# google-research/sparf

Measured on NVIDIA H100. Metric: rays/sec (fwd+bwd, 128 samples/ray), higher is better.
Workload: dtype fp32 in / out; GEMMs on Hopper wgmma with a 3-pass error-compensated split (fp16 halves forward, bf16 halves backward), fp32 accumulation; fp32 CUDA cores for encoding / activations / compositing

## Files before the change

### include/sparf_b200.h

```cpp
#ifndef SPARF_B200_H_
#define SPARF_B200_H_

#include <stddef.h>
#include <stdint.h>

#ifdef __cplusplus
extern "C" {
#endif

#define SPARF_B200_VERSION 100
#define SPARF_MAX_TRUNK 12
#define SPARF_MAX_L 16

enum {
  SPARF_OK = 0,
  SPARF_ERR_INVALID = 1,
  SPARF_ERR_CUDA = 2,
  SPARF_ERR_WORKSPACE = 3,
  SPARF_ERR_UNSUPPORTED = 4
};

enum {
  SPARF_ENGINE_AUTO = 0,
  SPARF_ENGINE_SIMT_FP32 = 1,
// ... 71 lines not shown
                                const float* origins, const float* dirs, const float* t, const float* noise, float* sigma,
                                float* rgb, void* tape, size_t tape_bytes, void* workspace, size_t workspace_bytes,
                                sparf_stream_t stream);
int sparf_mlp_backward_tape_rows(const SparfMLP* mlp, int32_t engine, int32_t R, int32_t S, const int64_t* rows,
                                 const float* origins, const float* dirs, const float* t, const float* sigma,
                                 const float* rgb, const float* d_sigma, const float* d_rgb, const SparfMLPGrad* grad,
                                 float* d_origins, float* d_dirs, void* tape, size_t tape_bytes, void* workspace,
                                 size_t workspace_bytes, sparf_stream_t stream);
int sparf_compact_scatter(int64_t C, const int64_t* K, const int64_t* sample_idx, int32_t width, const float* src,
                          float* dst, sparf_stream_t stream);
int sparf_compact_gather(int64_t C, const int64_t* K, const int64_t* sample_idx, int32_t width, const float* src,
                         float* dst, sparf_stream_t stream);
int sparf_compact_ray_sum(int64_t R, int32_t S, int64_t C, const int64_t* K, const int64_t* sample_idx, int32_t width,
                          const float* src, float* dst, sparf_stream_t stream);

int sparf_mlp_forward_tape_span(const SparfMLP* mlp, int32_t engine, int32_t C, int32_t cap, const int64_t* begin,
                                const int64_t* end, const float* origins, const float* dirs, const float* t,
                                const float* noise, float* sigma, float* rgb, void* tape, size_t tape_bytes,
                                void* workspace, size_t workspace_bytes, sparf_stream_t stream);
int sparf_compact_scatter_span(int64_t C, const int64_t* ends, int32_t w, const int64_t* sample_idx, int32_t width,
                               const float* src, float* dst, sparf_stream_t stream);
int sparf_compact_gather_span(int64_t C, const int64_t* ends, int32_t w, const int64_t* sample_idx, int32_t width,
                              const float* src, float* dst, sparf_stream_t stream);
int sparf_compact_ray_sum_segments(int64_t R, int32_t S, int32_t W, const int64_t* ends, const int64_t* sample_idx,
                                   int32_t width, const float* src, float* dst, sparf_stream_t stream);

size_t sparf_density_workspace_bytes(const SparfMLP* mlp, int64_t M, int32_t backward, int32_t engine);
int sparf_density_forward(const SparfMLP* mlp, int32_t engine, int64_t M, const float* points, float* raw, float* feat,
                          void* workspace, size_t workspace_bytes, sparf_stream_t stream);
int sparf_density_backward(const SparfMLP* mlp, int32_t engine, int64_t M, const float* points, const float* d_raw,
                           const float* d_feat, const SparfMLPGrad* grad, float* d_points, void* workspace,
                           size_t workspace_bytes, sparf_stream_t stream);
int sparf_density_gradient(const SparfMLP* mlp, int32_t engine, int64_t M, const float* points, float* grad_points,
                           void* workspace, size_t workspace_bytes, sparf_stream_t stream);

#define SPARF_MCUBES_MAX_TRIS 5
size_t sparf_mcubes_workspace_bytes(int64_t nx, int64_t ny, int64_t nz);
int sparf_mcubes_count(const float* vol, int64_t nx, int64_t ny, int64_t nz, float iso, int64_t* totals, void* workspace,
                       size_t workspace_bytes, sparf_stream_t stream);
int sparf_mcubes_emit(const float* vol, int64_t nx, int64_t ny, int64_t nz, float iso, float* verts, int64_t* faces,
                      void* workspace, size_t workspace_bytes, sparf_stream_t stream);
int sparf_mcubes_table(int8_t* table);

#define SPARF_MCUBES_BLOCK 8
size_t sparf_mcubes_sparse_workspace_bytes(int32_t res, int64_t n_active, int64_t max_verts);
int sparf_mcubes_sparse_classify(const float* coarse, int32_t res, float iso, int32_t* slots, int64_t* n_active,
                                 void* workspace, size_t workspace_bytes, sparf_stream_t stream);
int sparf_mcubes_sparse_blocks(const int32_t* slots, int32_t res, int64_t* block_ids, sparf_stream_t stream);
int sparf_mcubes_sparse_points(const float* axis, int32_t res, const int64_t* block_ids, int64_t b0, int64_t n_blocks,
                               float* points, sparf_stream_t stream);
int sparf_mcubes_sparse_count(const float* sigma_blocks, int32_t res, const int32_t* slots, const int64_t* block_ids,
                              int64_t n_active, float iso, int64_t* totals, void* workspace, size_t workspace_bytes,
                              sparf_stream_t stream);
int sparf_mcubes_sparse_emit(const float* sigma_blocks, int32_t res, const int32_t* slots, const int64_t* block_ids,
                             int64_t n_active, float iso, int64_t max_verts, int64_t max_faces, float* verts,
                             int64_t* faces, void* workspace, size_t workspace_bytes, sparf_stream_t stream);

int sparf_occupancy_build(const float* sigma, int32_t res, float thres, uint32_t* bits, sparf_stream_t stream);
size_t sparf_occupancy_workspace_bytes(int64_t R, int32_t S);
int sparf_occupancy_count(int64_t R, int32_t S, const float* origins, const float* dirs, const float* t,
                          const uint32_t* bits, int32_t res, float r0, float r1, int64_t* K, void* workspace,
                          size_t workspace_bytes, sparf_stream_t stream);
int sparf_occupancy_emit(int64_t R, int32_t S, const float* origins, const float* dirs, const float* t,
                         const uint32_t* bits, int32_t res, float r0, float r1, int64_t* sample_idx, float* origins_k,
                         float* dirs_k, float* t_k, void* workspace, size_t workspace_bytes, sparf_stream_t stream);

size_t sparf_termination_workspace_bytes(int64_t R, int32_t window);
int sparf_termination_count(int64_t R, int32_t S, int32_t k0, int32_t k1, const float* origins, const float* dirs,
                            const float* t, const uint8_t* alive, const uint32_t* bits, int32_t res, float r0, float r1,
                            int64_t* K, void* workspace, size_t workspace_bytes, sparf_stream_t stream);
int sparf_termination_emit(int64_t R, int32_t S, int32_t k0, int32_t k1, const float* origins, const float* dirs,
                           const float* t, const uint8_t* alive, const uint32_t* bits, int32_t res, float r0, float r1,
                           int64_t* sample_idx, float* origins_k, float* dirs_k, float* t_k, void* workspace,
                           size_t workspace_bytes, sparf_stream_t stream);
int sparf_termination_update(int64_t R, int32_t S, int32_t k0, int32_t k1, const float* sigma, const float* t,
                             const float* dirs, float tau_max, float* tau, uint8_t* alive, sparf_stream_t stream);
int sparf_termination_append(int64_t R, int32_t S, int32_t k0, int32_t k1, const float* origins, const float* dirs,
                             const float* t, const uint8_t* alive, const uint32_t* bits, int32_t res, float r0, float r1,
                             int64_t* ends, int32_t w, int64_t* sample_idx, float* origins_k, float* dirs_k, float* t_k,
                             void* workspace, size_t workspace_bytes, sparf_stream_t stream);

int sparf_contracted_count(int64_t R, int32_t S, int32_t k0, int32_t k1, const float* origins, const float* dirs,
                           const float* t, const uint8_t* alive, const uint32_t* bits, int32_t res, const float* center,
                           float radius, int64_t* K, void* workspace, size_t workspace_bytes, sparf_stream_t stream);
int sparf_contracted_emit(int64_t R, int32_t S, int32_t k0, int32_t k1, const float* origins, const float* dirs,
                          const float* t, const uint8_t* alive, const uint32_t* bits, int32_t res, const float* center,
                          float radius, int64_t* sample_idx, float* origins_k, float* dirs_k, float* t_k,
                          void* workspace, size_t workspace_bytes, sparf_stream_t stream);
int sparf_contracted_append(int64_t R, int32_t S, int32_t k0, int32_t k1, const float* origins, const float* dirs,
                            const float* t, const uint8_t* alive, const uint32_t* bits, int32_t res, const float* center,
                            float radius, int64_t* ends, int32_t w, int64_t* sample_idx, float* origins_k, float* dirs_k,
                            float* t_k, void* workspace, size_t workspace_bytes, sparf_stream_t stream);

size_t sparf_occupancy_sample_workspace_bytes(int32_t res);
int sparf_occupancy_sample(int32_t res, const uint32_t* bits, float r0, float r1, const float* center, float radius,
                           int64_t n_uniform, int64_t n_occupied, const float* u_cell, const float* u_jit, int64_t* cells,
                           float* points, void* workspace, size_t workspace_bytes, sparf_stream_t stream);
int sparf_occupancy_ema(int32_t res, int32_t contracted, int64_t n, const int64_t* cells, const float* sigma, float decay,
                        float thres, float* density, uint32_t* bits, void* workspace, size_t workspace_bytes,
                        sparf_stream_t stream);

int sparf_composite_forward(int32_t R, int32_t S, const float* sigma, const float* rgb, const float* t,
                            const float* dirs, int32_t white_bg, float* rgb_map, float* depth,
                            float* opacity, float* depth_var, float* rgb_var, float* weights,
                            float* all_cumulated, sparf_stream_t stream);
int sparf_composite_backward(int32_t R, int32_t S, const float* sigma, const float* rgb, const float* t,
                             const float* dirs, int32_t white_bg, const float* g_rgb_map,
                             const float* g_depth, const float* g_opacity, const float* g_weights,
                             float* d_sigma, float* d_rgb, float* d_dirs, sparf_stream_t stream);

int sparf_huber2_fwd_bwd(int64_t n, const float* pred, const float* target, float scale, float* loss,
                         float* d_pred, sparf_stream_t stream);

int sparf_posenc_forward(int64_t n, int32_t channels, int32_t L, const float* x, int32_t use_c2f, float c2f_start,
                         float c2f_range, const float* progress, float* out, sparf_stream_t stream);
int sparf_posenc_backward(int64_t n, int32_t channels, int32_t L, const float* x, int32_t use_c2f, float c2f_start,
                          float c2f_range, const float* progress, const float* d_out, float* d_x, sparf_stream_t stream);

int sparf_distortion_fwd_bwd(int32_t R, int32_t S, const float* t, const float* w, float scale, float* loss,
                             float* d_w, float* d_t, sparf_stream_t stream);

int sparf_adam_step(int64_t n, float* param, float* grad, float* exp_avg, float* exp_avg_sq, int64_t* step,
                    double* scratch, double lr0, double gamma, double warmup_steps, double beta1, double beta2,
                    double eps, double max_norm, sparf_stream_t stream);

int sparf_tc_selftest(const float* A, const float* B, int32_t K, void* packed, float* D, sparf_stream_t stream);
int sparf_tc_selftest_tn(const float* G, const float* X, int32_t rows, float* D, sparf_stream_t stream);
int sparf_tc_selftest_images(const float* X, const float* W1, const float* E, const float* W2, int32_t M, float* Y, float* Z,
                             float* db, sparf_stream_t stream);
int sparf_tc_selftest_persistent(const float* X, const float* W1, const float* E, const float* W2, int32_t M, float* Y,
                                 float* Z, float* db, int32_t max_ctas, sparf_stream_t stream);
int sparf_tc_selftest_head(const float* d_rgb, const float* rgb, const float* d_sigma, const float* raw, const float* hid,
                           const float* W9, int32_t M, int32_t HW, int32_t row_passes, int32_t tr_passes, uint16_t* img,
                           float* graw, sparf_stream_t stream);
int sparf_tc_selftest_featgrad(const float* d_raw, const float* d_feat, const float* feat, int32_t M, int32_t W,
                               int32_t row_passes, int32_t tr_passes, uint16_t* img, float* sums, sparf_stream_t stream);
int sparf_tc_selftest_wgrad(const float* G, const float* X, int32_t M, int32_t N, int32_t K, int32_t Kv, int32_t ldx,
                            int32_t div, int32_t passes, int32_t max_ctas, float* dW, uint32_t* bits, sparf_stream_t stream);
int sparf_tc_selftest_wgrad_rows(const float* G, const float* X, int32_t M, int32_t N, int32_t K, int32_t Kv, int32_t ldx,
                                 int32_t div, int32_t passes, int32_t max_ctas, const int64_t* rows, float* dW,
                                 uint32_t* bits, sparf_stream_t stream);
int sparf_tc_selftest_mask_bits(const float* G, const float* W, const float* X, int32_t M, int32_t N, int32_t K,
                                int32_t max_ctas, uint16_t* img, sparf_stream_t stream);
int sparf_tc_selftest_chain(const float* enc, int32_t M, int32_t E3, int32_t nt, int32_t skip, const float* W,
                            const float* bias, int32_t passes, int32_t f16, int32_t max_ctas, int32_t chain,
                            uint32_t outputs, const int64_t* rows, float* H, uint16_t* last, sparf_stream_t stream);
int sparf_tc_selftest_chain_bits(const float* enc, int32_t M, int32_t E3, int32_t nt, int32_t skip, const float* W,
                                 const float* bias, int32_t passes, int32_t f16, int32_t max_ctas, const int64_t* rows,
                                 float* H, uint32_t* bits, sparf_stream_t stream);
int sparf_tc_selftest_dgrad_chain(const float* G, int32_t M, int32_t E3, int32_t nt, int32_t skip, const float* W,
                                  const uint32_t* bits, int32_t dg_passes, int32_t wg_passes, int32_t max_ctas,
                                  int32_t chain, const int64_t* rows, uint16_t* tr, uint16_t* row, float* db,
                                  sparf_stream_t stream);

#ifdef __cplusplus
}
#endif
#endif
```

### sparf_b200/_lib.py

```python
from __future__ import annotations

import ctypes
import os
from ctypes import POINTER, c_char_p, c_float, c_int32, c_int64, c_size_t, c_void_p

from . import build as _build

MAX_TRUNK = 12
MCUBES_MAX_TRIS = 5
MCUBES_BLOCK = 8

ENGINE_AUTO, ENGINE_SIMT_FP32, ENGINE_TC_3X, ENGINE_TC_1X, ENGINE_TC_3X_W1 = 0, 1, 2, 3, 4
ENGINES = {"auto": 0, "simt_fp32": 1, "tc_3x": 2, "tc_1x": 3, "tc_3x_w1": 4}


class SparfMLP(ctypes.Structure):
    _fields_ = [
        ("n_trunk", c_int32), ("width", c_int32), ("head_width", c_int32), ("skip_layer", c_int32),
        ("L_xyz", c_int32), ("L_view", c_int32), ("use_c2f", c_int32),
        ("c2f_start", c_float), ("c2f_range", c_float),
        ("progress", c_void_p),
        ("trunk_w", c_void_p * MAX_TRUNK), ("trunk_b", c_void_p * MAX_TRUNK),
        ("head_w", c_void_p * 2), ("head_b", c_void_p * 2),
    ]


class SparfMLPGrad(ctypes.Structure):
    _fields_ = [
        ("trunk_w", c_void_p * MAX_TRUNK), ("trunk_b", c_void_p * MAX_TRUNK),
        ("head_w", c_void_p * 2), ("head_b", c_void_p * 2),
    ]


_P = c_void_p
_SIGNATURES = {
    "sparf_version": (c_int32, []),
    "sparf_last_error": (c_char_p, []),
    "sparf_launch_count": (ctypes.c_uint64, []),
    "sparf_engine_available": (c_int32, [c_int32]),
    "sparf_raygen_forward": (c_int32, [c_int32, c_int32, c_int32, _P, _P, _P, _P, c_int32, _P, _P, _P]),
    "sparf_raygen_backward": (c_int32, [c_int32, c_int32, c_int32, _P, _P, _P, _P, c_int32, _P, _P, _P, _P, _P]),
    "sparf_sample_depth": (c_int32, [c_int32, c_int32, c_float, c_float, c_int32, _P, _P, _P, _P]),
    "sparf_sample_pdf_merge": (c_int32, [c_int32, c_int32, c_int32, c_float, c_float, _P, _P, _P, _P, _P, _P]),
    "sparf_mlp_workspace_bytes": (c_size_t, [POINTER(SparfMLP), c_int32, c_int32, c_int32, c_int32]),
    "sparf_mlp_forward": (c_int32, [POINTER(SparfMLP), c_int32, c_int32, c_int32, _P, _P, _P, _P, _P, _P, _P, c_size_t, _P]),
    "sparf_mlp_backward": (c_int32, [POINTER(SparfMLP), c_int32, c_int32, c_int32, _P, _P, _P, _P, _P, _P,
                                     POINTER(SparfMLPGrad), _P, _P, _P, c_size_t, _P]),
    "sparf_mlp_tape_bytes": (c_size_t, [POINTER(SparfMLP), c_int32, c_int32, c_int32]),
    "sparf_mlp_forward_tape": (c_int32, [POINTER(SparfMLP), c_int32, c_int32, c_int32, _P, _P, _P, _P, _P, _P, _P, c_size_t,
                                         _P, c_size_t, _P]),
    "sparf_mlp_backward_tape": (c_int32, [POINTER(SparfMLP), c_int32, c_int32, c_int32, _P, _P, _P, _P, _P, _P, _P,
                                          POINTER(SparfMLPGrad), _P, _P, _P, c_size_t, _P, c_size_t, _P]),
    "sparf_mlp_forward_tape_rows": (c_int32, [POINTER(SparfMLP), c_int32, c_int32, c_int32, _P, _P, _P, _P, _P, _P, _P, _P,
                                              c_size_t, _P, c_size_t, _P]),
    "sparf_mlp_backward_tape_rows": (c_int32, [POINTER(SparfMLP), c_int32, c_int32, c_int32, _P, _P, _P, _P, _P, _P, _P, _P,
                                               POINTER(SparfMLPGrad), _P, _P, _P, c_size_t, _P, c_size_t, _P]),
    "sparf_compact_scatter": (c_int32, [c_int64, _P, _P, c_int32, _P, _P, _P]),
    "sparf_compact_gather": (c_int32, [c_int64, _P, _P, c_int32, _P, _P, _P]),
    "sparf_compact_ray_sum": (c_int32, [c_int64, c_int32, c_int64, _P, _P, c_int32, _P, _P, _P]),
    "sparf_mlp_forward_tape_span": (c_int32, [POINTER(SparfMLP), c_int32, c_int32, c_int32, _P, _P, _P, _P, _P, _P, _P, _P,
                                              _P, c_size_t, _P, c_size_t, _P]),
    "sparf_compact_scatter_span": (c_int32, [c_int64, _P, c_int32, _P, c_int32, _P, _P, _P]),
    "sparf_compact_gather_span": (c_int32, [c_int64, _P, c_int32, _P, c_int32, _P, _P, _P]),
    "sparf_compact_ray_sum_segments": (c_int32, [c_int64, c_int32, c_int32, _P, _P, c_int32, _P, _P, _P]),
    "sparf_density_workspace_bytes": (c_size_t, [POINTER(SparfMLP), c_int64, c_int32, c_int32]),
    "sparf_density_forward": (c_int32, [POINTER(SparfMLP), c_int32, c_int64, _P, _P, _P, _P, c_size_t, _P]),
    "sparf_density_backward": (c_int32, [POINTER(SparfMLP), c_int32, c_int64, _P, _P, _P, POINTER(SparfMLPGrad), _P, _P,
                                         c_size_t, _P]),
    "sparf_density_gradient": (c_int32, [POINTER(SparfMLP), c_int32, c_int64, _P, _P, _P, c_size_t, _P]),
    "sparf_mcubes_workspace_bytes": (c_size_t, [c_int64, c_int64, c_int64]),
    "sparf_mcubes_count": (c_int32, [_P, c_int64, c_int64, c_int64, c_float, _P, _P, c_size_t, _P]),
    "sparf_mcubes_emit": (c_int32, [_P, c_int64, c_int64, c_int64, c_float, _P, _P, _P, c_size_t, _P]),
    "sparf_mcubes_table": (c_int32, [_P]),
    "sparf_mcubes_sparse_workspace_bytes": (c_size_t, [c_int32, c_int64, c_int64]),
    "sparf_mcubes_sparse_classify": (c_int32, [_P, c_int32, c_float, _P, _P, _P, c_size_t, _P]),
    "sparf_mcubes_sparse_blocks": (c_int32, [_P, c_int32, _P, _P]),
    "sparf_mcubes_sparse_points": (c_int32, [_P, c_int32, _P, c_int64, c_int64, _P, _P]),
    "sparf_mcubes_sparse_count": (c_int32, [_P, c_int32, _P, _P, c_int64, c_float, _P, _P, c_size_t, _P]),
    "sparf_mcubes_sparse_emit": (c_int32, [_P, c_int32, _P, _P, c_int64, c_float, c_int64, c_int64, _P, _P, _P, c_size_t,
                                           _P]),
    "sparf_occupancy_build": (c_int32, [_P, c_int32, c_float, _P, _P]),
    "sparf_occupancy_workspace_bytes": (c_size_t, [c_int64, c_int32]),
    "sparf_occupancy_count": (c_int32, [c_int64, c_int32, _P, _P, _P, _P, c_int32, c_float, c_float, _P, _P, c_size_t, _P]),
    "sparf_occupancy_emit": (c_int32, [c_int64, c_int32, _P, _P, _P, _P, c_int32, c_float, c_float, _P, _P, _P, _P, _P,
                                       c_size_t, _P]),
    "sparf_termination_workspace_bytes": (c_size_t, [c_int64, c_int32]),
    "sparf_termination_count": (c_int32, [c_int64, c_int32, c_int32, c_int32, _P, _P, _P, _P, _P, c_int32, c_float, c_float,
                                          _P, _P, c_size_t, _P]),
    "sparf_termination_emit": (c_int32, [c_int64, c_int32, c_int32, c_int32, _P, _P, _P, _P, _P, c_int32, c_float, c_float,
                                         _P, _P, _P, _P, _P, c_size_t, _P]),
    "sparf_termination_update": (c_int32, [c_int64, c_int32, c_int32, c_int32, _P, _P, _P, c_float, _P, _P, _P]),
    "sparf_termination_append": (c_int32, [c_int64, c_int32, c_int32, c_int32, _P, _P, _P, _P, _P, c_int32, c_float, c_float,
                                           _P, c_int32, _P, _P, _P, _P, _P, c_size_t, _P]),
    "sparf_contracted_append": (c_int32, [c_int64, c_int32, c_int32, c_int32, _P, _P, _P, _P, _P, c_int32, POINTER(c_float),
                                          c_float, _P, c_int32, _P, _P, _P, _P, _P, c_size_t, _P]),
    "sparf_contracted_count": (c_int32, [c_int64, c_int32, c_int32, c_int32, _P, _P, _P, _P, _P, c_int32, POINTER(c_float),
                                         c_float, _P, _P, c_size_t, _P]),
    "sparf_contracted_emit": (c_int32, [c_int64, c_int32, c_int32, c_int32, _P, _P, _P, _P, _P, c_int32, POINTER(c_float),
                                        c_float, _P, _P, _P, _P, _P, c_size_t, _P]),
    "sparf_occupancy_sample_workspace_bytes": (c_size_t, [c_int32]),
    "sparf_occupancy_sample": (c_int32, [c_int32, _P, c_float, c_float, POINTER(c_float), c_float, c_int64, c_int64, _P, _P,
                                         _P, _P, _P, c_size_t, _P]),
    "sparf_occupancy_ema": (c_int32, [c_int32, c_int32, c_int64, _P, _P, c_float, c_float, _P, _P, _P, c_size_t, _P]),
    "sparf_composite_forward":(c_int32, [c_int32, c_int32, _P, _P, _P, _P, c_int32, _P, _P, _P, _P, _P, _P, _P, _P]),
    "sparf_composite_backward": (c_int32, [c_int32, c_int32, _P, _P, _P, _P, c_int32, _P, _P, _P, _P, _P, _P, _P, _P]),
    "sparf_huber2_fwd_bwd": (c_int32, [c_int64, _P, _P, c_float, _P, _P, _P]),
    "sparf_posenc_forward": (c_int32, [c_int64, c_int32, c_int32, _P, c_int32, c_float, c_float, _P, _P, _P]),
    "sparf_posenc_backward": (c_int32, [c_int64, c_int32, c_int32, _P, c_int32, c_float, c_float, _P, _P, _P, _P]),
    "sparf_distortion_fwd_bwd": (c_int32, [c_int32, c_int32, _P, _P, c_float, _P, _P, _P, _P]),
    "sparf_adam_step": (c_int32, [c_int64, _P, _P, _P, _P, _P, _P] + [ctypes.c_double] * 7 + [_P]),
    "sparf_tc_selftest": (c_int32, [_P, _P, c_int32, _P, _P, _P]),
    "sparf_tc_selftest_tn": (c_int32, [_P, _P, c_int32, _P, _P]),
    "sparf_tc_selftest_images": (c_int32, [_P, _P, _P, _P, c_int32, _P, _P, _P, _P]),
    "sparf_tc_selftest_persistent": (c_int32, [_P, _P, _P, _P, c_int32, _P, _P, _P, c_int32, _P]),
    "sparf_tc_selftest_head": (c_int32, [_P, _P, _P, _P, _P, _P, c_int32, c_int32, c_int32, c_int32, _P, _P, _P]),
    "sparf_tc_selftest_featgrad": (c_int32, [_P, _P, _P, c_int32, c_int32, c_int32, c_int32, _P, _P, _P]),
    "sparf_tc_selftest_wgrad": (c_int32, [_P, _P, c_int32, c_int32, c_int32, c_int32, c_int32, c_int32, c_int32, c_int32,
                                          _P, _P, _P]),
    "sparf_tc_selftest_wgrad_rows": (c_int32, [_P, _P, c_int32, c_int32, c_int32, c_int32, c_int32, c_int32, c_int32,
                                               c_int32, _P, _P, _P, _P]),
    "sparf_tc_selftest_mask_bits": (c_int32, [_P, _P, _P, c_int32, c_int32, c_int32, c_int32, _P, _P]),
    "sparf_tc_selftest_chain": (c_int32, [_P, c_int32, c_int32, c_int32, c_int32, _P, _P, c_int32, c_int32, c_int32, c_int32,
                                          ctypes.c_uint32, _P, _P, _P, _P]),
    "sparf_tc_selftest_chain_bits": (c_int32, [_P, c_int32, c_int32, c_int32, c_int32, _P, _P, c_int32, c_int32, c_int32,
                                               _P, _P, _P, _P]),
    "sparf_tc_selftest_dgrad_chain": (c_int32, [_P, c_int32, c_int32, c_int32, c_int32, _P, _P, c_int32, c_int32, c_int32,
                                                c_int32, _P, _P, _P, _P, _P]),
}

_lib = None


def exported_symbols():
    return list(_SIGNATURES)


def lib():
    global _lib
    if _lib is not None:
        return _lib
    path = _build.LIB_PATH
    override = os.environ.get("SPARF_B200_LIB")
    if override:
        if not os.path.exists(override):
            raise RuntimeError("SPARF_B200_LIB=%s does not exist" % override)
        path = override
    elif not os.path.exists(path) or _build._stale():
        try:
            path = _build.build()
        except Exception as e:
            if not os.path.exists(path):
                raise RuntimeError(
                    "sparf_b200: native library %s is missing and could not be built (%s). "
                    "There is no fallback path." % (path, e))
    L = ctypes.CDLL(path)
    for name, (res, args) in _SIGNATURES.items():
        fn = getattr(L, name)
        fn.restype = res
        fn.argtypes = args
    _lib = L
    return L


def check(rc: int, what: str = ""):
    if rc != 0:
        msg = lib().sparf_last_error()
        raise RuntimeError("sparf_b200 %s failed (code %d): %s" % (what, rc, msg.decode() if msg else "?"))
```

### sparf_b200/csrc/gemm_wgmma.cu

```cuda
#include <cuda_bf16.h>
#include <cudaTypedefs.h>
#include <cuda_fp16.h>

#include <algorithm>
#include <type_traits>

#include "gemm_wgmma.cuh"

namespace sparf {
namespace {

constexpr int TM = 128, TN = 128, TK = 32;
constexpr int TILE_ELEMS = TM * TK;

struct __align__(128) WgSmem {
  uint16_t a[2][TILE_ELEMS];
  uint16_t b[2][TILE_ELEMS];
};

__device__ __forceinline__ int sw_off(int r, int k) { return (((r >> 3) * (TK / 8) + (k >> 3)) << 6) + ((r & 7) << 3) + (k & 7); }

__device__ __forceinline__ uint64_t smem_desc(const void* p) {
  uint32_t a = static_cast<uint32_t>(__cvta_generic_to_shared(p));
  uint64_t d = (uint64_t)((a & 0x3FFFF) >> 4);
// ... 645 lines not shown
      float* d = e.out + (size_t)m * e.ldo + e.col_off + n;
      if (n < e.Kv) atomicAdd(d, acc[i]);
      if (two && n + 1 < e.Kv) atomicAdd(d + 1, acc[i + 1]);
    }
    if (!two) acc[i + 1] = 0.f;
  }
}

template <bool F16, bool F32, int ROWP, int TRP>
__device__ __forceinline__ void epilogue(float (&acc)[64], int bx, int by, const Epi e) {
  const int m0 = by * TM, n0 = bx * TN;
  if (e.pairs) epilogue_values<F32, true>(acc, m0, n0, e);
  else epilogue_values<F32, false>(acc, m0, n0, e);
  const int lane = threadIdx.x & 31, w = threadIdx.x >> 5;
  if (e.colsum) {
    float part[32];
#pragma unroll
    for (int j = 0; j < 16; ++j)
#pragma unroll
      for (int c = 0; c < 2; ++c) part[2 * j + c] = acc[4 * j + c] + acc[4 * j + 2 + c];
    tile_colsum(part, n0, e.N, e.colsum);
  }
  if constexpr (ROWP > 0) {
#pragma unroll
    for (int j = 0; j < 16; ++j) {
      const int kt = (n0 >> 5) + (j >> 2);
      if (kt >= e.row_ks) break;
      uint16_t* t = e.row + ((size_t)by * e.row_ks + kt) * 2 * TILE_ELEMS;
#pragma unroll
      for (int h = 0; h < 2; ++h) {
        uint32_t hi, lo;
        split2<F16>(acc[4 * j + 2 * h], acc[4 * j + 2 * h + 1], hi, lo);
        const int core = (2 * w + h) * (TK / 8) + (j & 3);
        reinterpret_cast<uint32_t*>(t + core * 64)[lane] = hi;
        if (ROWP == 3) reinterpret_cast<uint32_t*>(t + TILE_ELEMS + core * 64)[lane] = lo;
      }
    }
  }
  if constexpr (TRP > 0) {
    const int kt = (m0 >> 5) + (w >> 1);
    if (kt < e.tr_ks) {
      uint16_t* t = e.tr + ((size_t)bx * e.tr_ks + kt) * 2 * TILE_ELEMS;
#pragma unroll
      for (int j = 0; j < 16; ++j)
#pragma unroll
        for (int h = 0; h < 2; ++h) {
          uint32_t hi, lo;
          split2<F16>(acc[4 * j + 2 * h], acc[4 * j + 2 * h + 1], hi, lo);
          const int core = j * (TK / 8) + 2 * (w & 1) + h;
          reinterpret_cast<uint32_t*>(t + core * 64)[lane] = movmatrix_trans(hi);
          if (TRP == 3) reinterpret_cast<uint32_t*>(t + TILE_ELEMS + core * 64)[lane] = movmatrix_trans(lo);
        }
    }
  }
}

template <bool F16, int PASSES, bool F32, int ROWP, int TRP, bool DYN = false, bool SPAN = false>
__global__ void __launch_bounds__(GEMM_THREADS, 1) wg_gemm_kernel(Opnd a, Opnd b, Units w, Epi e, RowCount rc) {
  extern __shared__ __align__(1024) uint8_t smem[];
  if constexpr (DYN) {
    e.M = (int)live_rows<true, SPAN>(e.M, rc);
    if (e.M == 0) return;
    w.tiles = (e.M + TM - 1) / TM * w.rtb;
    if constexpr (SPAN) e.out += row_start<true>(rc) * e.ldo;
  }
  uint64_t* full = reinterpret_cast<uint64_t*>(smem + STAGES * STAGE_BYTES + RED_BYTES);
  uint64_t* empty = full + STAGES;
  if (threadIdx.x == 0) {
    for (int i = 0; i < STAGES; ++i) {
      mbar_init(&full[i], 1);
      mbar_init(&empty[i], CONSUMERS / 32);
    }
    asm volatile("fence.mbarrier_init.release.cluster;\n" ::: "memory");
  }
  __syncthreads();
  if (threadIdx.x >= CONSUMERS) {
    asm volatile("setmaxnreg.dec.sync.aligned.u32 40;\n" ::: "memory");
    if (threadIdx.x == CONSUMERS) produce<PASSES>(a, b, w, full, empty);
    return;
  }
  asm volatile("setmaxnreg.inc.sync.aligned.u32 232;\n" ::: "memory");
  int it = 0;
  for (int u = blockIdx.x; u < w.tiles * w.nsplit; u += gridDim.x) {
    int bx, by, kt0, nk;
    w.get(u, bx, by, kt0, nk);
    float acc[64];
    mma_unit<F16, PASSES>(acc, nk, it, full, empty);
    epilogue<F16, F32, ROWP, TRP>(acc, bx, by, e);
  }
}

struct Staged {
  const float* X;
  int ldx, div, M, K;
  uint32_t* bits;
  int kw;
};

constexpr int STAGED_THREADS = CONSUMERS + 256;
constexpr int STAGED_STAGES = 5;
constexpr int PART_BYTES = TM * TN * 4;
constexpr int STAGED_SMEM = STAGED_STAGES * STAGE_BYTES + PART_BYTES + 3 * STAGED_STAGES * 8;

__device__ __forceinline__ void split8_mul(const float (&v)[8], uint4& hi, uint4& lo) {
  uint16_t h[8], l[8];
#pragma unroll
  for (int e = 0; e < 8; ++e) {
    const __nv_bfloat16 b = __float2bfloat16_rn(v[e]);
    h[e] = __bfloat16_as_ushort(b);
    l[e] = __bfloat16_as_ushort(__float2bfloat16_rn((v[e] - __bfloat162float(b)) * (float)(1 << LO_SHIFT)));
  }
  hi = make_uint4(h[0] | (uint32_t)h[1] << 16, h[2] | (uint32_t)h[3] << 16, h[4] | (uint32_t)h[5] << 16, h[6] | (uint32_t)h[7] << 16);
  lo = make_uint4(l[0] | (uint32_t)l[1] << 16, l[2] | (uint32_t)l[3] << 16, l[4] | (uint32_t)l[5] << 16, l[6] | (uint32_t)l[7] << 16);
}

__device__ __forceinline__ void converter_sync() { asm volatile("bar.sync 2, 128;\n" ::: "memory"); }
__device__ __forceinline__ void fence_proxy_async() { asm volatile("fence.proxy.async.shared::cta;\n" ::: "memory"); }

template <int PASSES, int NST = STAGES>
__device__ __forceinline__ void produce_staged(const Opnd& a, const Staged& x, const CUtensorMap* xmap, const Units& w,
                                               uint64_t* full, uint64_t* empty) {
  extern __shared__ __align__(1024) uint8_t smem[];
  const int lane = threadIdx.x & 31;
  const uint32_t abytes = PASSES == 3 ? 2 * TILE_BYTES : TILE_BYTES;
  int it = 0;
  for (int u = blockIdx.x; u < w.tiles * w.nsplit; u += gridDim.x) {
    int bx, by, kt0, nk;
    w.get(u, bx, by, kt0, nk);
    const int k0 = bx * TM;
    const uint32_t rbytes = 4 * min(TM, x.K - k0);
    for (int j = 0; j < nk; ++j, ++it) {
      const int s = it % NST, m0 = (kt0 + j) * TK;
      mbar_wait(&empty[s], ((it / NST) & 1) ^ 1);
      uint8_t* st = smem + s * STAGE_BYTES;
      if (x.div == 1) {
        if (lane == 0) {
          mbar_expect_tx(&full[s], abytes + TK * TM * 4);
          bulk_g2s(st, a.tile(by, kt0 + j), abytes, &full[s]);
          tensor_g2s(st + 2 * TILE_BYTES, xmap, k0, m0, &full[s]);
        }
        continue;
      }
      if (lane == 0) {
        mbar_expect_tx(&full[s], abytes + min(TK, x.M - m0) * rbytes);
        bulk_g2s(st, a.tile(by, kt0 + j), abytes, &full[s]);
      }
      __syncwarp();
      const int m = m0 + lane;
      if (m < x.M) bulk_g2s(st + 2 * TILE_BYTES + lane * (TM * 4), x.X + (size_t)(m / x.div) * x.ldx + k0, rbytes, &full[s]);
    }
  }
}

template <int PASSES, int NST = STAGES>
__device__ __forceinline__ void convert_staged(const Staged& x, const Units& w, uint64_t* full, uint64_t* conv) {
  extern __shared__ __align__(1024) uint8_t smem[];
  const int t = threadIdx.x - CONSUMERS, lane = t & 31;
  int it = 0;
  for (int u = blockIdx.x; u < w.tiles * w.nsplit; u += gridDim.x) {
    int bx, by, kt0, nk;
    w.get(u, bx, by, kt0, nk);
    const bool kin = bx * TM + t < x.K, bits = x.bits && by == 0;
    const int bword = bx * (TM / 32) + (t >> 5);
    for (int j = 0; j < nk; ++j, ++it) {
      const int s = it % NST, m0 = (kt0 + j) * TK;
      mbar_wait(&full[s], (it / NST) & 1);
      uint8_t* st = smem + s * STAGE_BYTES + 2 * TILE_BYTES;
      const float* src = reinterpret_cast<const float*>(st);
      float v[TK];
      if (kin && m0 + TK <= x.M) {
#pragma unroll
        for (int r = 0; r < TK; ++r) v[r] = src[r * TM + t];
      } else {
#pragma unroll
        for (int r = 0; r < TK; ++r) v[r] = kin && m0 + r < x.M ? src[r * TM + t] : 0.f;
      }
      if (bits) {
        uint32_t word = 0;
#pragma unroll
        for (int r = 0; r < TK; ++r) {
          const uint32_t b = __ballot_sync(0xffffffffu, v[r] > 0.f);
          if (lane == r) word = b;
        }
        if (m0 + lane < x.M && bword < x.kw) x.bits[(size_t)(m0 + lane) * x.kw + bword] = word;
      }
      converter_sync();
      uint16_t* img = reinterpret_cast<uint16_t*>(st);
#pragma unroll
      for (int o = 0; o < TK / 8; ++o) {
        float e8[8];
#pragma unroll
        for (int e = 0; e < 8; ++e) e8[e] = v[8 * o + e];
        uint4 hi, lo;
        split8_mul(e8, hi, lo);
        const int off = sw_off(t, 8 * o);
        *reinterpret_cast<uint4*>(img + off) = hi;
        if (PASSES == 3) *reinterpret_cast<uint4*>(img + TILE_ELEMS + off) = lo;
      }
      fence_proxy_async();
      __syncwarp();
      if (lane == 0) mbar_arrive(&conv[s]);
    }
  }
}

__device__ __forceinline__ int part_off(int r, int c) { return r * TN + (((c >> 3) ^ (r & 7)) << 3) + (c & 7); }

__device__ __forceinline__ void presum_epilogue(const float (&acc)[64], float* part, bool first, bool flush, int bx, int by,
                                                const Epi& e) {
  const int lane = threadIdx.x & 31, w = threadIdx.x >> 5;
#pragma unroll
  for (int i = 0; i < 64; i += 2) {
    float2* p = reinterpret_cast<float2*>(part + part_off(frag_row(i), frag_col(i)));
    if (first) {
      *p = make_float2(acc[i], acc[i + 1]);
    } else {
      const float2 o = *p;
      *p = make_float2(o.x + acc[i], o.y + acc[i + 1]);
    }
  }
  if (!flush) return;
  __syncwarp();
  const int m0 = by * TM, n0 = bx * TN;
  float* out = e.out + e.col_off + n0;
  for (int i = 0; i < 16; ++i) {
    const int r = 16 * w + i, m = m0 + r;
    if (m >= e.M) continue;
#pragma unroll
    for (int q = 0; q < TN / 32; ++q) {
      const int c = 32 * q + lane, n = n0 + c;
      if (n < e.N && n < e.Kv) atomicAdd(out + (size_t)m * e.ldo + c, part[part_off(r, c)]);
    }
  }
  __syncwarp();
}

template <int PASSES, bool DYN = false>
__global__ void __launch_bounds__(STAGED_THREADS, 1) wg_gemm_staged_kernel(Opnd a, Staged x, Units w, Epi e, RowCount rc,
                                                                           int ctas, const __grid_constant__ CUtensorMap xmap) {
  extern __shared__ __align__(1024) uint8_t smem[];
  if constexpr (DYN) {
    x.M = (int)live_rows<true, false>(x.M, rc);
    if (x.M == 0) return;
    w.nk = (x.M + TK - 1) / TK;
    w.nsplit = max(1, min(w.nk, (ctas + w.tiles - 1) / w.tiles * ((w.nk + 1023) / 1024)));
  }
  float* part = reinterpret_cast<float*>(smem + STAGED_STAGES * STAGE_BYTES);
  uint64_t* full = reinterpret_cast<uint64_t*>(smem + STAGED_STAGES * STAGE_BYTES + PART_BYTES);
  uint64_t* empty = full + STAGED_STAGES;
  uint64_t* conv = empty + STAGED_STAGES;
  if (threadIdx.x == 0) {
    for (int i = 0; i < STAGED_STAGES; ++i) {
      mbar_init(&full[i], 1);
      mbar_init(&empty[i], CONSUMERS / 32);
      mbar_init(&conv[i], 4);
    }
    asm volatile("fence.mbarrier_init.release.cluster;\n" ::: "memory");
  }
  __syncthreads();
  if (threadIdx.x >= CONSUMERS + 128) {
    asm volatile("setmaxnreg.dec.sync.aligned.u32 40;\n" ::: "memory");
    if (threadIdx.x < CONSUMERS + 128 + 32) produce_staged<PASSES, STAGED_STAGES>(a, x, &xmap, w, full, empty);
    return;
  }
  if (threadIdx.x >= CONSUMERS) {
    asm volatile("setmaxnreg.dec.sync.aligned.u32 64;\n" ::: "memory");
    convert_staged<PASSES, STAGED_STAGES>(x, w, full, conv);
    return;
  }
  asm volatile("setmaxnreg.inc.sync.aligned.u32 200;\n" ::: "memory");
  const int units = w.tiles * w.nsplit, grid = gridDim.x;
  int it = 0;
  for (int u = blockIdx.x; u < units; u += grid) {
    int bx, by, kt0, nk;
    w.get(u, bx, by, kt0, nk);
    float acc[64];
    mma_unit<false, PASSES, true, STAGED_STAGES>(acc, nk, it, full, empty, conv);
    const int t = u % w.tiles;
    const bool first = u < grid || (u - grid) % w.tiles != t;
    const bool flush = u + grid >= units || (u + grid) % w.tiles != t;
    presum_epilogue(acc, part, first, flush, bx, by, e);
  }
}

constexpr int CH_W = 256;
constexpr int CH_M = 64;
constexpr int CH_KS = CH_W / TK;
constexpr int CH_ENC_KS = 2;
constexpr int CH_HALF = CH_M * TK * 2;
constexpr int CH_STAGES = 4;
constexpr int CH_ENC = CH_KS * 2 * CH_HALF;
constexpr int CH_RING = CH_ENC + CH_ENC_KS * 2 * CH_HALF;
constexpr int CH_BAR = CH_RING + CH_STAGES * STAGE_BYTES;
constexpr int CH_SMEM = CH_BAR + (2 * CH_STAGES + 2) * 8;

struct Chain {
  int M, nl, skip, enc_ks;
  const uint16_t* enc;
  const uint16_t* w[SPARF_MAX_TRUNK];
  const float* bias[SPARF_MAX_TRUNK];
  float* H[SPARF_MAX_TRUNK];
  uint16_t* last;
  uint32_t* bits[SPARF_MAX_TRUNK];
};

__host__ __device__ __forceinline__ int chain_ks(int l, int skip, int enc_ks) {
  return l == 0 ? enc_ks : CH_KS + (l == skip ? enc_ks : 0);
}

template <int PASSES>
__device__ __forceinline__ void chain_produce(const Chain& c, int M, int tiles, uint64_t* full, uint64_t* empty, uint64_t* enc_full,
                                              uint64_t* enc_empty) {
  extern __shared__ __align__(1024) uint8_t smem[];
  constexpr int HB = PASSES == 3 ? 2 : 1;
  int it = 0, n = 0;
  for (int t = blockIdx.x; t < tiles; t += gridDim.x) {
    if (t * CH_M >= M) continue;
    mbar_wait(enc_empty, (n & 1) ^ 1);
    ++n;
    mbar_expect_tx(enc_full, c.enc_ks * HB * CH_HALF);
    for (int kt = 0; kt < c.enc_ks; ++kt)
      for (int h = 0; h < HB; ++h)
        bulk_g2s(smem + CH_ENC + (kt * 2 + h) * CH_HALF,
                 c.enc + (((size_t)(t >> 1) * c.enc_ks + kt) * 2 + h) * TILE_ELEMS + (t & 1) * (CH_M * TK), CH_HALF, enc_full);
    for (int l = 0; l < c.nl; ++l) {
      const int nk = chain_ks(l, c.skip, c.enc_ks);
      for (int kt = 0; kt < nk; ++kt, ++it) {
        const int s = it % CH_STAGES;
        mbar_wait(&empty[s], ((it / CH_STAGES) & 1) ^ 1);
        uint8_t* st = smem + CH_RING + s * STAGE_BYTES;
        mbar_expect_tx(&full[s], 2 * HB * TILE_BYTES);
        for (int g = 0; g < 2; ++g)
          bulk_g2s(st + g * 2 * TILE_BYTES, c.w[l] + ((size_t)g * nk + kt) * 2 * TILE_ELEMS, HB * TILE_BYTES, &full[s]);
      }
    }
  }
}

template <bool F16, int PASSES>
__device__ __forceinline__ void chain_mma(float (&acc)[64], int nk, int na, int& it, uint64_t* full, uint64_t* empty) {
  extern __shared__ __align__(1024) uint8_t smem[];
  const int wg = threadIdx.x >> 7, lane = threadIdx.x & 31;
  float acc_lo[PASSES == 3 ? 64 : 1];
#pragma unroll
  for (int i = 0; i < 64; ++i) acc[i] = 0.f;
#pragma unroll
  for (int i = 0; i < (PASSES == 3 ? 64 : 1); ++i) acc_lo[i] = 0.f;
  for (int j = 0; j < nk; ++j, ++it) {
    const int s = it % CH_STAGES;
    mbar_wait(&full[s], (it / CH_STAGES) & 1);
    const uint8_t* a = j < na ? smem + j * 2 * CH_HALF : smem + CH_ENC + (j - na) * 2 * CH_HALF;
    const uint8_t* b = smem + CH_RING + s * STAGE_BYTES + wg * 2 * TILE_BYTES;
    wgmma_fence();
#pragma unroll
    for (int ks = 0; ks < TK / 16; ++ks) {
      const uint64_t ahi = smem_desc(a + ks * 256), bhi = smem_desc(b + ks * 256);
      if constexpr (PASSES == 3) {
        wgmma_m64n128k16<F16>(acc_lo, smem_desc(a + CH_HALF + ks * 256), bhi);
        wgmma_m64n128k16<F16>(acc_lo, ahi, smem_desc(b + TILE_BYTES + ks * 256));
      }
      wgmma_m64n128k16<F16>(acc, ahi, bhi);
    }
    wgmma_commit();
    wgmma_wait_1();
    if (j > 0 && lane == 0) mbar_arrive(&empty[(it + CH_STAGES - 1) % CH_STAGES]);
  }
  wgmma_wait_all();
  if (lane == 0) mbar_arrive(&empty[(it + CH_STAGES - 1) % CH_STAGES]);
  if constexpr (PASSES == 3) {
#pragma unroll
    for (int i = 0; i < 64; ++i) acc[i] += ldexpf(acc_lo[i], -LO_SHIFT);
  }
}

template <bool F16, int PASSES>
__device__ __forceinline__ void chain_epilogue(float (&acc)[64], const Chain& c, int M, int l, int t) {
  extern __shared__ __align__(1024) uint8_t smem[];
  const int wg = threadIdx.x >> 7, wq = (threadIdx.x >> 5) & 3, lane = threadIdx.x & 31;
  const float* bias = c.bias[l];
#pragma unroll
  for (int i = 0; i < 64; i += 2) {
    const int m = t * CH_M + wq * 16 + (lane >> 2) + ((i >> 1) & 1) * 8, n = wg * TN + (i >> 2) * 8 + (lane & 3) * 2;
    if (m >= M) {
      acc[i] = acc[i + 1] = 0.f;
      continue;
    }
    acc[i] = fmaxf(acc[i] + bias[n], 0.f);
    acc[i + 1] = fmaxf(acc[i + 1] + bias[n + 1], 0.f);
  }
  const bool last = l == c.nl - 1;
  if (last && !c.last) return;
  uint16_t* img = last ? c.last + (size_t)(t >> 1) * CH_KS * 2 * TILE_ELEMS + (t & 1) * (CH_M * TK)
                       : reinterpret_cast<uint16_t*>(smem);
  const int kstride = last ? 2 * TILE_ELEMS : CH_HALF, lo_off = last ? TILE_ELEMS : CH_HALF / 2;
#pragma unroll
  for (int j = 0; j < 16; ++j) {
    uint16_t* kt = img + (size_t)(4 * wg + (j >> 2)) * kstride;
#pragma unroll
    for (int h = 0; h < 2; ++h) {
      uint32_t hi, lo;
      split2<F16>(acc[4 * j + 2 * h], acc[4 * j + 2 * h + 1], hi, lo);
      const int core = (2 * wq + h) * (TK / 8) + (j & 3);
      reinterpret_cast<uint32_t*>(kt + core * 64)[lane] = hi;
      if (PASSES == 3) reinterpret_cast<uint32_t*>(kt + lo_off + core * 64)[lane] = lo;
    }
  }
}

__device__ __forceinline__ void chain_store(const float (&acc)[64], float* H, int M, int t) {
  const int wg = threadIdx.x >> 7, wq = (threadIdx.x >> 5) & 3, lane = threadIdx.x & 31;
#pragma unroll
  for (int i = 0; i < 64; i += 2) {
    const int m = t * CH_M + wq * 16 + (lane >> 2) + ((i >> 1) & 1) * 8, n = wg * TN + (i >> 2) * 8 + (lane & 3) * 2;
    if (m < M) *reinterpret_cast<float2*>(H + (size_t)m * CH_W + n) = make_float2(acc[i], acc[i + 1]);
  }
}

__device__ __forceinline__ void chain_store_bits(const float (&acc)[64], uint32_t* bits, int M, int t) {
  const int wg = threadIdx.x >> 7, wq = (threadIdx.x >> 5) & 3, lane = threadIdx.x & 31;
#pragma unroll
  for (int h = 0; h < 2; ++h) {
    uint32_t mine = 0;
#pragma unroll
    for (int q = 0; q < 4; ++q) {
      uint32_t w = 0;
#pragma unroll
      for (int jj = 0; jj < 4; ++jj) {
        const int i = 4 * (4 * q + jj) + 2 * h, b = 8 * jj + 2 * (lane & 3);
        w |= (uint32_t)(acc[i] > 0.f) << b | (uint32_t)(acc[i + 1] > 0.f) << (b + 1);
      }
      w |= __shfl_xor_sync(0xffffffffu, w, 1);
      w |= __shfl_xor_sync(0xffffffffu, w, 2);
      if ((lane & 3) == q) mine = w;
    }
    const int m = t * CH_M + wq * 16 + (lane >> 2) + 8 * h;
    if (m < M) bits[(size_t)m * (CH_W / 32) + wg * 4 + (lane & 3)] = mine;
  }
}

template <bool F16, int PASSES, bool DYN = false, bool BITS = false, bool SPAN = false>
__global__ void __launch_bounds__(GEMM_THREADS, 1) trunk_chain_kernel(const Chain c, RowCount rc) {
  extern __shared__ __align__(1024) uint8_t smem[];
  const int M = (int)live_rows<DYN, SPAN>(c.M, rc);
  if (DYN && M == 0) return;
  const int tiles = (M + TM - 1) / TM * 2;
  uint64_t* full = reinterpret_cast<uint64_t*>(smem + CH_BAR);
  uint64_t* empty = full + CH_STAGES;
  uint64_t* enc_full = empty + CH_STAGES;
  uint64_t* enc_empty = enc_full + 1;
  if (threadIdx.x == 0) {
    for (int i = 0; i < CH_STAGES; ++i) {
      mbar_init(&full[i], 1);
      mbar_init(&empty[i], CONSUMERS / 32);
    }
    mbar_init(enc_full, 1);
    mbar_init(enc_empty, CONSUMERS / 32);
    asm volatile("fence.mbarrier_init.release.cluster;\n" ::: "memory");
  }
  __syncthreads();
  if (threadIdx.x >= CONSUMERS) {
    asm volatile("setmaxnreg.dec.sync.aligned.u32 40;\n" ::: "memory");
    if (threadIdx.x == CONSUMERS) chain_produce<PASSES>(c, M, tiles, full, empty, enc_full, enc_empty);
    return;
  }
  asm volatile("setmaxnreg.inc.sync.aligned.u32 232;\n" ::: "memory");
  const int enc_last = c.skip > 0 && c.skip < c.nl ? c.skip : 0;
  const long long s0 = row_start<SPAN>(rc);
  int it = 0, n = 0;
  for (int t = blockIdx.x; t < tiles; t += gridDim.x) {
    if (t * CH_M >= M) {
      if (c.last)
        for (int i = 0; i < CH_KS * (PASSES == 3 ? 2 : 1); ++i)
          reinterpret_cast<uint4*>(c.last + ((size_t)(t >> 1) * CH_KS * 2 + (PASSES == 3 ? i : 2 * i)) * TILE_ELEMS +
                                   (t & 1) * (CH_M * TK))[threadIdx.x] = make_uint4(0, 0, 0, 0);
      continue;
    }
    mbar_wait(enc_full, n & 1);
    ++n;
    for (int l = 0; l < c.nl; ++l) {
      float acc[64];
      chain_mma<F16, PASSES>(acc, chain_ks(l, c.skip, c.enc_ks), l == 0 ? 0 : CH_KS, it, full, empty);
      if (l == enc_last && (threadIdx.x & 31) == 0) mbar_arrive(enc_empty);
      consumer_sync();
      chain_epilogue<F16, PASSES>(acc, c, M, l, t);
      if (l + 1 < c.nl) {
        fence_proxy_async();
        consumer_sync();
      }
      if (c.H[l]) chain_store(acc, c.H[l] + s0 * CH_W, M, t);
      if (BITS && c.bits[l]) chain_store_bits(acc, c.bits[l] + s0 * (CH_W / 32), M, t);
    }
  }
}

template <bool F16, int PASSES>
static int launch_chain(const Chain& c, int ctas, RowCount rc, cudaStream_t st) {
  bool bits = false;
  for (int l = 0; l < c.nl; ++l) bits |= c.bits[l] != nullptr;
  auto kernel = bits ? (rc.rows ? trunk_chain_kernel<F16, PASSES, true, true> : trunk_chain_kernel<F16, PASSES, false, true>)
                     : (rc.rows ? trunk_chain_kernel<F16, PASSES, true> : trunk_chain_kernel<F16, PASSES>);
  if (rc.start) {
    if (!bits) {
      set_error("trunk_chain: a row start needs the mask bits (taped forward)");
      return SPARF_ERR_UNSUPPORTED;
    }
    kernel = trunk_chain_kernel<F16, PASSES, true, true, true>;
  }
  SPARF_CHECK_CUDA(cudaFuncSetAttribute(kernel, cudaFuncAttributeMaxDynamicSharedMemorySize, CH_SMEM));
  kernel<<<std::min(2 * ceil_div(c.M, TM), ctas), GEMM_THREADS, CH_SMEM, st>>>(c, rc);
  SPARF_CHECK_LAUNCH("trunk_chain_kernel");
  return SPARF_OK;
}

struct DgChain {
  int M, top, tr_ks;
  const uint16_t* in;
  const uint16_t* w[SPARF_MAX_TRUNK];
  const uint32_t* bits[SPARF_MAX_TRUNK];
  float* db[SPARF_MAX_TRUNK];
  uint16_t* tr[SPARF_MAX_TRUNK];
  uint16_t* row[SPARF_MAX_TRUNK];
};

template <int DP>
__device__ __forceinline__ void dg_produce(const DgChain& c, int M, int tiles, uint64_t* full, uint64_t* empty, uint64_t* act_full,
                                           uint64_t* act_empty) {
  extern __shared__ __align__(1024) uint8_t smem[];
  constexpr int HB = DP == 3 ? 2 : 1;
  int it = 0, n = 0;
  for (int t = blockIdx.x; t < tiles; t += gridDim.x) {
    if (t * CH_M >= M) continue;
    mbar_wait(act_empty, (n & 1) ^ 1);
    ++n;
    mbar_expect_tx(act_full, CH_KS * HB * CH_HALF);
    for (int kt = 0; kt < CH_KS; ++kt)
      for (int h = 0; h < HB; ++h)
        bulk_g2s(smem + (kt * 2 + h) * CH_HALF,
                 c.in + (((size_t)(t >> 1) * CH_KS + kt) * 2 + h) * TILE_ELEMS + (t & 1) * (CH_M * TK), CH_HALF, act_full);
    for (int l = c.top; l >= 1; --l)
      for (int kt = 0; kt < CH_KS; ++kt, ++it) {
        const int s = it % CH_STAGES;
        mbar_wait(&empty[s], ((it / CH_STAGES) & 1) ^ 1);
        uint8_t* st = smem + CH_RING + s * STAGE_BYTES;
        mbar_expect_tx(&full[s], 2 * HB * TILE_BYTES);
        for (int g = 0; g < 2; ++g)
          bulk_g2s(st + g * 2 * TILE_BYTES, c.w[l] + ((size_t)g * CH_KS + kt) * 2 * TILE_ELEMS, HB * TILE_BYTES, &full[s]);
      }
  }
}

__device__ __forceinline__ void dg_mask_words(uint4 (&wd)[2], const uint32_t* bits, int M, int t) {
  const int wg = threadIdx.x >> 7, wq = (threadIdx.x >> 5) & 3, lane = threadIdx.x & 31;
#pragma unroll
  for (int h = 0; h < 2; ++h) {
    const int m = t * CH_M + wq * 16 + (lane >> 2) + 8 * h;
    wd[h] = m < M ? *reinterpret_cast<const uint4*>(bits + (size_t)m * (CH_W / 32) + wg * 4) : make_uint4(0, 0, 0, 0);
  }
}

template <int PASSES>
__device__ __forceinline__ void dg_split(const float (&acc)[64], uint16_t* img, int kstride, int lo_off) {
  const int wg = threadIdx.x >> 7, wq = (threadIdx.x >> 5) & 3, lane = threadIdx.x & 31;
#pragma unroll
  for (int j = 0; j < 16; ++j) {
    uint16_t* kt = img + (size_t)(4 * wg + (j >> 2)) * kstride;
#pragma unroll
    for (int h = 0; h < 2; ++h) {
      uint32_t hi, lo;
      split2<false>(acc[4 * j + 2 * h], acc[4 * j + 2 * h + 1], hi, lo);
      const int core = (2 * wq + h) * (TK / 8) + (j & 3);
      reinterpret_cast<uint32_t*>(kt + core * 64)[lane] = hi;
      if (PASSES == 3) reinterpret_cast<uint32_t*>(kt + lo_off + core * 64)[lane] = lo;
    }
  }
}

template <int DP, int TP>
__device__ __forceinline__ void dg_zero_tile(const DgChain& c, int t) {
  const uint4 z = make_uint4(0, 0, 0, 0);
  for (int l = c.top; l >= 1; --l) {
    if (c.row[l])
      for (int i = 0; i < CH_KS * (DP == 3 ? 2 : 1); ++i)
        reinterpret_cast<uint4*>(c.row[l] + ((size_t)(t >> 1) * CH_KS * 2 + (DP == 3 ? i : 2 * i)) * TILE_ELEMS +
                                 (t & 1) * (CH_M * TK))[threadIdx.x] = z;
    for (int g = 0; g < 2; ++g)
      for (int kt = 2 * t; kt < 2 * t + 2 && kt < c.tr_ks; ++kt)
        for (int h = 0; h < (TP == 3 ? 2 : 1); ++h)
          for (int i = threadIdx.x; i < TILE_ELEMS / 8; i += CONSUMERS)
            reinterpret_cast<uint4*>(c.tr[l] + (((size_t)g * c.tr_ks + kt) * 2 + h) * TILE_ELEMS)[i] = z;
  }
}

template <int DP, int TP, bool DYN = false>
__global__ void __launch_bounds__(GEMM_THREADS, 1) dgrad_chain_kernel(const DgChain c, RowCount rc) {
  extern __shared__ __align__(1024) uint8_t smem[];
  const int M = (int)live_rows<DYN, false>(c.M, rc);
  if (DYN && M == 0) return;
  const int tiles = (M + TM - 1) / TM * 2;
  uint64_t* full = reinterpret_cast<uint64_t*>(smem + CH_BAR);
  uint64_t* empty = full + CH_STAGES;
  uint64_t* act_full = empty + CH_STAGES;
  uint64_t* act_empty = act_full + 1;
  float* red = reinterpret_cast<float*>(smem + CH_ENC);
  if (threadIdx.x == 0) {
    for (int i = 0; i < CH_STAGES; ++i) {
      mbar_init(&full[i], 1);
      mbar_init(&empty[i], CONSUMERS / 32);
    }
    mbar_init(act_full, 1);
    mbar_init(act_empty, CONSUMERS / 32);
    asm volatile("fence.mbarrier_init.release.cluster;\n" ::: "memory");
  }
  __syncthreads();
  if (threadIdx.x >= CONSUMERS) {
    asm volatile("setmaxnreg.dec.sync.aligned.u32 40;\n" ::: "memory");
    if (threadIdx.x == CONSUMERS) dg_produce<DP>(c, M, tiles, full, empty, act_full, act_empty);
    return;
  }
  asm volatile("setmaxnreg.inc.sync.aligned.u32 232;\n" ::: "memory");
  const int wg = threadIdx.x >> 7, wq = (threadIdx.x >> 5) & 3, w = threadIdx.x >> 5, lane = threadIdx.x & 31;
  int it = 0, n = 0;
  for (int t = blockIdx.x; t < tiles; t += gridDim.x) {
    if (t * CH_M >= M) {
      dg_zero_tile<DP, TP>(c, t);
      continue;
    }
    mbar_wait(act_full, n & 1);
    ++n;
    for (int l = c.top; l >= 1; --l) {
      uint4 wd[2];
      dg_mask_words(wd, c.bits[l], M, t);
      float acc[64];
      chain_mma<false, DP>(acc, CH_KS, CH_KS, it, full, empty);
      if (l == 1 && lane == 0) mbar_arrive(act_empty);
      consumer_sync();
      const uint32_t wds[2][4] = {{wd[0].x, wd[0].y, wd[0].z, wd[0].w}, {wd[1].x, wd[1].y, wd[1].z, wd[1].w}};
#pragma unroll
      for (int i = 0; i < 64; i += 2) {
        const int j = i >> 2;
        const uint32_t k = wds[(i >> 1) & 1][j >> 2] >> (8 * (j & 3) + 2 * (lane & 3));
        if (!(k & 1)) acc[i] = 0.f;
        if (!(k & 2)) acc[i + 1] = 0.f;
      }
#pragma unroll
      for (int j = 0; j < 16; ++j)
#pragma unroll
        for (int cc = 0; cc < 2; ++cc) {
          float s = acc[4 * j + cc] + acc[4 * j + 2 + cc];
#pragma unroll
          for (int o = 4; o < 32; o <<= 1) s += __shfl_xor_sync(0xffffffffu, s, o);
          if (lane < 4) red[w * TN + 8 * j + 2 * lane + cc] = s;
        }
      if (l > 1) {
        dg_split<DP>(acc, reinterpret_cast<uint16_t*>(smem), CH_HALF, CH_HALF / 2);
        fence_proxy_async();
      }
      consumer_sync();
      {
        float s = 0.f;
#pragma unroll
        for (int i = 0; i < 4; ++i) s += red[(4 * wg + i) * TN + (threadIdx.x & (TN - 1))];
        atomicAdd(c.db[l] + threadIdx.x, s);
      }
      const int kt = 2 * t + (wq >> 1);
      if (kt < c.tr_ks) {
        uint16_t* tp = c.tr[l] + ((size_t)wg * c.tr_ks + kt) * 2 * TILE_ELEMS;
#pragma unroll
        for (int j = 0; j < 16; ++j)
#pragma unroll
          for (int h = 0; h < 2; ++h) {
            uint32_t hi, lo;
            split2<false>(acc[4 * j + 2 * h], acc[4 * j + 2 * h + 1], hi, lo);
            const int core = j * (TK / 8) + 2 * (wq & 1) + h;
            reinterpret_cast<uint32_t*>(tp + core * 64)[lane] = movmatrix_trans(hi);
            if (TP == 3) reinterpret_cast<uint32_t*>(tp + TILE_ELEMS + core * 64)[lane] = movmatrix_trans(lo);
          }
      }
      if (c.row[l])
        dg_split<DP>(acc, c.row[l] + (size_t)(t >> 1) * CH_KS * 2 * TILE_ELEMS + (t & 1) * (CH_M * TK), 2 * TILE_ELEMS, TILE_ELEMS);
    }
  }
}

template <int DP, int TP>
static int launch_dgrad_chain(const DgChain& c, int ctas, RowCount rc, cudaStream_t st) {
  auto kernel = rc.rows ? dgrad_chain_kernel<DP, TP, true> : dgrad_chain_kernel<DP, TP>;
  SPARF_CHECK_CUDA(cudaFuncSetAttribute(kernel, cudaFuncAttributeMaxDynamicSharedMemorySize, CH_SMEM));
  kernel<<<std::min(2 * ceil_div(c.M, TM), ctas), GEMM_THREADS, CH_SMEM, st>>>(c, rc);
  SPARF_CHECK_LAUNCH("dgrad_chain_kernel");
  return SPARF_OK;
}

template <bool F16, int PASSES, bool KFAST, class F, bool DYN = false>
static int launch_pack(F f, int rtiles, int ksteps, uint16_t* img, cudaStream_t st, RowCount rc = {nullptr, 0}) {
  pack_kernel<F16, PASSES, KFAST, F, DYN><<<dim3(ksteps, rtiles), 256, 0, st>>>(f, ksteps, img, rc);
  SPARF_CHECK_LAUNCH("pack_kernel");
  return SPARF_OK;
}

template <bool F16, int PASSES, bool F32, int ROWP, int TRP>
static int launch_gemm(const Opnd& a, const Opnd& b, const Units& w, int ctas, const Epi& e, RowCount rc, cudaStream_t st) {
  auto kernel = rc.rows ? wg_gemm_kernel<F16, PASSES, F32, ROWP, TRP, true> : wg_gemm_kernel<F16, PASSES, F32, ROWP, TRP>;
  if (rc.start) {
    if constexpr (F32) {
      kernel = wg_gemm_kernel<F16, PASSES, F32, ROWP, TRP, true, true>;
    } else {
      set_error("a GEMM without an fp32 output takes no row start");
      return SPARF_ERR_UNSUPPORTED;
    }
  }
  SPARF_CHECK_CUDA(cudaFuncSetAttribute(kernel, cudaFuncAttributeMaxDynamicSharedMemorySize, GEMM_SMEM));
  kernel<<<std::min(w.tiles * w.nsplit, ctas), GEMM_THREADS, GEMM_SMEM, st>>>(a, b, w, e, rc);
  SPARF_CHECK_LAUNCH("wg_gemm_kernel");
  return SPARF_OK;
}

static int gemm_ctas(const TcPrec& p) { return p.max_ctas > 0 ? std::min(p.max_ctas, num_sms()) : num_sms(); }

static Units gemm_units(int rta, int rtb, int ksteps, bool split_k, int ctas) {
  Units w{rtb, rta * rtb, 1, ksteps};
  if (split_k) w.nsplit = std::max(1, std::min(ksteps, ceil_div(ctas, w.tiles) * ceil_div(ksteps, 1024)));
  return w;
}

template <bool F16, int PASSES, bool BK, class FB>
static int run(const TcPrec& p, const Opnd& a, int a_rows, FB fb, int b_rows, int ksteps, bool split_k, const Epi& e,
               int row_passes, int tr_passes, cudaStream_t st) {
  const int rta = ceil_div(a_rows, TM), rtb = ceil_div(b_rows, TM);
  SPARF_REQUIRE(p.pack_b && (size_t)rtb * ksteps * 2 * TILE_ELEMS <= p.pack_elems,
                "tc gemm: B operand image needs %zu 16-bit elements, have %zu", (size_t)rtb * ksteps * 2 * TILE_ELEMS,
                p.pack_elems);
  SPARF_TRY((launch_pack<F16, PASSES, BK>(fb, rtb, ksteps, p.pack_b, st)));
  const Opnd b{p.pack_b, nullptr, ksteps, 0};
  const int ctas = gemm_ctas(p);
  const Units w = gemm_units(rta, rtb, ksteps, split_k, ctas);
  const bool f32 = e.out != nullptr;
  const RowCount rc = p.rows;
  SPARF_REQUIRE(!rc.rows || !split_k, "tc gemm: a device row count needs the staged weight-gradient GEMM");
  if (f32 && !row_passes && !tr_passes) return launch_gemm<F16, PASSES, true, 0, 0>(a, b, w, ctas, e, rc, st);
  if (f32 && row_passes == PASSES && !tr_passes) return launch_gemm<F16, PASSES, true, PASSES, 0>(a, b, w, ctas, e, rc, st);
  if (!f32 && row_passes == PASSES && tr_passes == 3) return launch_gemm<F16, PASSES, false, PASSES, 3>(a, b, w, ctas, e, rc, st);
  if (!f32 && row_passes == PASSES && tr_passes == 1) return launch_gemm<F16, PASSES, false, PASSES, 1>(a, b, w, ctas, e, rc, st);
  SPARF_REQUIRE(false, "tc gemm: no kernel for fp32 output %d, row image %d passes, transposed image %d passes", (int)f32,
                row_passes, tr_passes);
}

static int staged_tensor_map(const Staged& x, CUtensorMap* map) {
  static PFN_cuTensorMapEncodeTiled_v12000 encode = nullptr;
  if (!encode) {
    void* fn = nullptr;
    cudaDriverEntryPointQueryResult q;
    SPARF_CHECK_CUDA(cudaGetDriverEntryPoint("cuTensorMapEncodeTiled", &fn, cudaEnableDefault, &q));
    SPARF_REQUIRE(fn && q == cudaDriverEntryPointSuccess, "tc_gemm_tn: the driver has no cuTensorMapEncodeTiled");
    encode = reinterpret_cast<PFN_cuTensorMapEncodeTiled_v12000>(fn);
  }
  const cuuint64_t dims[2] = {(cuuint64_t)x.K, (cuuint64_t)x.M}, pitch[1] = {(cuuint64_t)x.ldx * 4};
  const cuuint32_t box[2] = {TM, TK}, step[2] = {1, 1};
  const CUresult r = encode(map, CU_TENSOR_MAP_DATA_TYPE_FLOAT32, 2, const_cast<float*>(x.X), dims, pitch, box, step,
                            CU_TENSOR_MAP_INTERLEAVE_NONE, CU_TENSOR_MAP_SWIZZLE_NONE, CU_TENSOR_MAP_L2_PROMOTION_L2_256B,
                            CU_TENSOR_MAP_FLOAT_OOB_FILL_NONE);
  SPARF_REQUIRE(r == CUDA_SUCCESS, "tc_gemm_tn: cuTensorMapEncodeTiled failed (%d)", (int)r);
  return SPARF_OK;
}

template <int PASSES>
static int run_staged(const TcPrec& p, const Opnd& gt, int N, const Staged& x, int ksteps, const Epi& e, cudaStream_t st) {
  CUtensorMap xmap{};
  if (x.div == 1 && x.M > 0) SPARF_TRY(staged_tensor_map(x, &xmap));
  const int ctas = gemm_ctas(p);
  const Units w = gemm_units(ceil_div(N, TM), ceil_div(x.K, TM), ksteps, true, ctas);
  auto kernel = p.rows.rows ? wg_gemm_staged_kernel<PASSES, true> : wg_gemm_staged_kernel<PASSES>;
  SPARF_CHECK_CUDA(cudaFuncSetAttribute(kernel, cudaFuncAttributeMaxDynamicSharedMemorySize, STAGED_SMEM));
  kernel<<<std::min(w.tiles * w.nsplit, ctas), STAGED_THREADS, STAGED_SMEM, st>>>(gt, x, w, e, p.rows, ctas, xmap);
  SPARF_CHECK_LAUNCH("wg_gemm_staged_kernel");
  return SPARF_OK;
}

static Opnd opnd(const TcImage& x, const TcImage& y = TcImage{}) { return Opnd{x.p, y.p, x.ks, y.ks}; }

static int set_images(Epi& e, const TcOut& o, int M, int N) {
  SPARF_REQUIRE(!e.accumulate || (!o.row_passes && !o.tr_passes), "tc gemm: images of an accumulated output");
  SPARF_REQUIRE(!o.row_passes || (o.row.p && o.row.ks == ceil_div(N, TK)), "tc gemm: row image needs %d k-steps",
                ceil_div(N, TK));
  SPARF_REQUIRE(!o.tr_passes || (o.tr.p && o.tr.ks == ceil_div(M, TK)), "tc gemm: transposed image needs %d k-steps",
                ceil_div(M, TK));
  e.row = o.row.p; e.row_ks = o.row.ks;
  e.tr = o.tr.p; e.tr_ks = o.tr.ks;
  return SPARF_OK;
}

}

#define SPARF_WG_RUN(BK, ...)                                                                   \
  (p.f16 ? (p.passes == 3 ? run<true, 3, BK>(__VA_ARGS__) : run<true, 1, BK>(__VA_ARGS__))       \
         : (p.passes == 3 ? run<false, 3, BK>(__VA_ARGS__) : run<false, 1, BK>(__VA_ARGS__)))
#define SPARF_WG_PACK(KFAST, ...)                                                                                 \
  (p.f16 ? (p.passes == 3 ? launch_pack<true, 3, KFAST>(__VA_ARGS__) : launch_pack<true, 1, KFAST>(__VA_ARGS__)) \
         : (p.passes == 3 ? launch_pack<false, 3, KFAST>(__VA_ARGS__) : launch_pack<false, 1, KFAST>(__VA_ARGS__)))

size_t tc_image_elems(int rows, int cols) { return (size_t)ceil_div(rows, TM) * ceil_div(cols, TK) * 2 * TILE_ELEMS; }

size_t tc_pack_elems(int rows, int ksteps_rows, int cols) {
  return (size_t)ceil_div(std::max(rows, cols), TM) * ksteps_rows * 2 * TILE_ELEMS;
}

int tc_pack_rows(TcPrec p, int M, int K, const float* X, int ldx, int div, TcImage img, cudaStream_t st) {
  SPARF_REQUIRE((p.passes == 1 || p.passes == 3) && img.p && img.ks == ceil_div(K, TK), "tc_pack_rows: passes=%d ks=%d K=%d",
                p.passes, img.ks, K);
  if (p.rows.rows) {
    const Rows f{X, ldx, K, div, M};
    return p.f16 ? (p.passes == 3 ? launch_pack<true, 3, true, Rows, true>(f, ceil_div(M, TM), img.ks, img.p, st, p.rows)
                                  : launch_pack<true, 1, true, Rows, true>(f, ceil_div(M, TM), img.ks, img.p, st, p.rows))
                 : (p.passes == 3 ? launch_pack<false, 3, true, Rows, true>(f, ceil_div(M, TM), img.ks, img.p, st, p.rows)
                                  : launch_pack<false, 1, true, Rows, true>(f, ceil_div(M, TM), img.ks, img.p, st, p.rows));
  }
  return SPARF_WG_PACK(true, Rows{X, ldx, K, div, M}, ceil_div(M, TM), img.ks, img.p, st);
}

int tc_pack_cols(TcPrec p, int M, int N, const float* X, int ldx, TcImage img, cudaStream_t st) {
  SPARF_REQUIRE((p.passes == 1 || p.passes == 3) && img.p && img.ks == ceil_div(M, TK), "tc_pack_cols: passes=%d ks=%d M=%d",
                p.passes, img.ks, M);
  return SPARF_WG_PACK(false, Cols{X, ldx, M, N}, ceil_div(N, TM), img.ks, img.p, st);
}

int tc_gemm_nt(TcPrec p, int act, int M, int N, TcImage a1, int K1v, TcImage a2, int K2v, const float* W, int ldw, int wcol2,
               const float* bias, float* Y, int ldy, const TcOut& out, cudaStream_t st) {
  SPARF_REQUIRE((p.passes == 1 || p.passes == 3) && (act == 0 || act == 1) && Y, "tc_gemm_nt: passes=%d act=%d", p.passes, act);
  const int ks = a1.ks + (a2.p ? a2.ks : 0);
  Epi e{};
  e.kind = 0; e.M = M; e.N = N; e.act = act; e.bias = bias; e.out = Y; e.ldo = ldy;
  e.pairs = N % 2 == 0 && pair_aligned(Y, ldy);
  SPARF_TRY(set_images(e, out, M, N));
  return SPARF_WG_RUN(true, p, opnd(a1, a2.p ? a2 : TcImage{}), M, NtB{W, ldw, wcol2, K1v, K2v, N, a1.ks}, N, ks, false, e,
                      out.row_passes, out.tr_passes, st);
}

bool tc_chain_supported(int W, int E3p, int nt, int skip) {
  return W == CH_W && E3p <= CH_ENC_KS * TK && nt >= 3 && nt <= SPARF_MAX_TRUNK && skip != 0 && skip < nt;
}

int tc_chain_ksteps(int l, int skip, int E3p) { return chain_ks(l, skip, ceil_div(E3p, TK)); }

int tc_pack_nt(TcPrec p, int N, int ks1, int K1v, int ks2, int K2v, const float* W, int ldw, int wcol2, TcImage img,
               cudaStream_t st) {
  SPARF_REQUIRE((p.passes == 1 || p.passes == 3) && img.p && img.ks == ks1 + ks2, "tc_pack_nt: passes=%d ks=%d, %d + %d k-steps",
                p.passes, img.ks, ks1, ks2);
  return SPARF_WG_PACK(true, NtB{W, ldw, wcol2, K1v, K2v, N, ks1}, ceil_div(N, TM), img.ks, img.p, st);
}

int tc_pack_nn(TcPrec p, int Kout, int N, int Kv, const float* W, int ldw, int wcol, TcImage img, cudaStream_t st) {
  SPARF_REQUIRE((p.passes == 1 || p.passes == 3) && img.p && img.ks == ceil_div(N, TK), "tc_pack_nn: passes=%d ks=%d N=%d",
                p.passes, img.ks, N);
  return SPARF_WG_PACK(false, NnB{W, ldw, wcol, Kv, N}, ceil_div(Kout, TM), img.ks, img.p, st);
}

int tc_dgrad_chain(TcPrec dg, TcPrec wg, int M, int W, int top, TcImage in, const TcImage* wimg, const uint32_t* const* bits,
                   float* const* db, const TcImage* tr, const TcImage* row, cudaStream_t st) {
  SPARF_REQUIRE(!dg.f16 && !wg.f16 && M >= 1 && W == CH_W && top >= 1 && top < SPARF_MAX_TRUNK && in.p && in.ks == CH_KS,
                "tc_dgrad_chain: bf16 images, M=%d W=%d top=%d, input row image of %d k-steps", M, W, top, CH_KS);
  DgChain c{};
  c.M = M; c.top = top; c.tr_ks = ceil_div(M, TK); c.in = in.p;
  for (int l = 1; l <= top; ++l) {
    SPARF_REQUIRE(wimg[l].p && wimg[l].ks == CH_KS && bits[l] && !(reinterpret_cast<uintptr_t>(bits[l]) & 15) && db[l] &&
                      tr[l].p && tr[l].ks == c.tr_ks && (!row[l].p || row[l].ks == CH_KS),
                  "tc_dgrad_chain: layer %d: weight image of %d k-steps, 16-byte aligned mask bits, column sums, transposed "
                  "image of %d k-steps, row image of %d",
                  l, CH_KS, c.tr_ks, CH_KS);
    c.w[l] = wimg[l].p; c.bits[l] = bits[l]; c.db[l] = db[l]; c.tr[l] = tr[l].p; c.row[l] = row[l].p;
  }
  const int ctas = gemm_ctas(dg);
  if (dg.passes == 3 && wg.passes == 3) return launch_dgrad_chain<3, 3>(c, ctas, dg.rows, st);
  if (dg.passes == 3 && wg.passes == 1) return launch_dgrad_chain<3, 1>(c, ctas, dg.rows, st);
  if (dg.passes == 1 && wg.passes == 1) return launch_dgrad_chain<1, 1>(c, ctas, dg.rows, st);
  SPARF_REQUIRE(false, "tc_dgrad_chain: no kernel for %d-pass row and %d-pass transposed images", dg.passes, wg.passes);
}

int tc_trunk_chain(TcPrec p, int M, int W, int nt, int skip, TcImage enc, const TcImage* wimg, const float* const* bias,
                   float* const* H, uint32_t* const* bits, const TcOut& last, cudaStream_t st) {
  SPARF_REQUIRE((p.passes == 1 || p.passes == 3) && M >= 1 && enc.p && tc_chain_supported(W, enc.ks * TK, nt, skip),
                "tc_trunk_chain: passes=%d M=%d W=%d nt=%d skip=%d encoding k-steps %d", p.passes, M, W, nt, skip, enc.ks);
  Chain c{};
  c.M = M; c.skip = skip; c.enc_ks = enc.ks; c.enc = enc.p;
  c.nl = H[nt - 1] ? nt : nt - 1;
  SPARF_REQUIRE(H[c.nl - 1], "tc_trunk_chain: no output asked for");
  for (int l = 0; l < c.nl; ++l) {
    SPARF_REQUIRE(wimg[l].p && wimg[l].ks == chain_ks(l, skip, enc.ks) && bias[l] && !(reinterpret_cast<uintptr_t>(H[l]) & 7),
                  "tc_trunk_chain: layer %d: weight image of %d k-steps, bias, 8-byte aligned output", l,
                  chain_ks(l, skip, enc.ks));
    c.w[l] = wimg[l].p; c.bias[l] = bias[l]; c.H[l] = H[l];
    c.bits[l] = bits ? bits[l] : nullptr;
  }
  if (last.row_passes) {
    SPARF_REQUIRE(c.nl == nt && last.row_passes == p.passes && !last.tr_passes && last.row.p && last.row.ks == CH_KS,
                  "tc_trunk_chain: the last layer's row image takes the chain's passes and %d k-steps", CH_KS);
    c.last = last.row.p;
  }
  const int ctas = gemm_ctas(p);
  return p.f16 ? (p.passes == 3 ? launch_chain<true, 3>(c, ctas, p.rows, st) : launch_chain<true, 1>(c, ctas, p.rows, st))
               : (p.passes == 3 ? launch_chain<false, 3>(c, ctas, p.rows, st) : launch_chain<false, 1>(c, ctas, p.rows, st));
}

int tc_gemm_nn(TcPrec p, int M, int N, int Kout, int Kv, TcImage g, const float* W, int ldw, int wcol, const float* mask_src,
               int ldmask, const uint32_t* mask_bits, const float* r1_vec, const float* r1_row, float* D, int ldd,
               int accumulate, const TcOut& out, float* db, float* r1_wgrad, cudaStream_t st) {
  SPARF_REQUIRE((p.passes == 1 || p.passes == 3) && g.ks == ceil_div(N, TK), "tc_gemm_nn: passes=%d ks=%d N=%d", p.passes,
                g.ks, N);
  SPARF_REQUIRE(!r1_wgrad || (mask_src && r1_vec && !D), "tc_gemm_nn: r1_wgrad needs the mask source, r1_vec, no fp32 D");
  SPARF_REQUIRE(!mask_src || !mask_bits, "tc_gemm_nn: an fp32 mask or a bit mask, not both");
  SPARF_REQUIRE(!mask_bits || !D, "tc_gemm_nn: a bit mask needs image outputs only (no fp32 D)");
  Epi e{};
  e.kind = 1; e.M = M; e.N = Kout; e.out = D; e.ldo = ldd; e.Kv = Kv; e.mask = mask_src; e.ldmask = ldmask;
  if (mask_bits) {
    e.mask_bits = mask_bits;
    e.ldbits = ceil_div(Kout, 32);
  }
  e.r1_vec = r1_vec; e.r1_row = r1_row; e.accumulate = accumulate; e.colsum = db; e.r1_wgrad = r1_wgrad;
  e.pairs = Kout % 2 == 0 && pair_aligned(D, ldd) && pair_aligned(mask_src, ldmask);
  SPARF_REQUIRE(!db || !accumulate, "tc_gemm_nn: column sums of an accumulated output");
  SPARF_TRY(set_images(e, out, M, Kout));
  return SPARF_WG_RUN(false, p, opnd(g), M, NnB{W, ldw, wcol, Kv, N}, Kout, g.ks, false, e, out.row_passes, out.tr_passes, st);
}

int tc_gemm_tn(TcPrec p, int M, int N, int K, int Kv, TcImage gt, const float* X, int ldx, int div, float* dW, int ldw,
               int wcol, uint32_t* bits, cudaStream_t st) {
  SPARF_REQUIRE((p.passes == 1 || p.passes == 3) && gt.ks == ceil_div(M, TK), "tc_gemm_tn: passes=%d ks=%d", p.passes, gt.ks);
  Epi e{};
  e.kind = 2; e.M = N; e.N = K; e.out = dW; e.ldo = ldw; e.col_off = wcol; e.Kv = Kv;
  if (!(reinterpret_cast<uintptr_t>(X) & 15) && ldx % 4 == 0 && K % 4 == 0) {
    SPARF_REQUIRE(!p.f16, "tc_gemm_tn: bf16 halves only");
    const Staged x{X, ldx, div, M, K, bits, ceil_div(K, 32)};
    return p.passes == 3 ? run_staged<3>(p, opnd(gt), N, x, gt.ks, e, st) : run_staged<1>(p, opnd(gt), N, x, gt.ks, e, st);
  }
  SPARF_REQUIRE(!p.rows.rows, "tc_gemm_tn: a device row count needs X 16-byte aligned with ldx and K multiples of 4");
  return SPARF_WG_RUN(false, p, opnd(gt), N, TnB{X, ldx, div, M, K, bits, ceil_div(K, 32)}, K, gt.ks, true, e, 0, 0, st);
}

template <int ROWP, int TRP>
static int launch_head_bwd(const HeadBwd& h, RowCount rc, cudaStream_t st) {
  auto kernel = rc.rows ? head_bwd_kernel<ROWP, TRP, true> : head_bwd_kernel<ROWP, TRP>;
  SPARF_CHECK_CUDA(cudaFuncSetAttribute(kernel, cudaFuncAttributeMaxDynamicSharedMemorySize, HEAD_SMEM));
  kernel<<<ceil_div(h.M, TM), 256, HEAD_SMEM, st>>>(h, rc);
  SPARF_CHECK_LAUNCH("head_bwd_kernel");
  return SPARF_OK;
}

int tc_head_backward(TcPrec dg, TcPrec wg, int M, int HW, const float* d_rgb, const float* rgb, const float* d_sigma,
                     const float* raw, const float* hid, const float* W9, float* graw, TcImage row, TcImage tr, float* dW9,
                     float* db9, float* db_hid, float* db_raw, cudaStream_t st) {
  SPARF_REQUIRE(!dg.f16 && !wg.f16 && (dg.passes == 1 || dg.passes == 3) && (wg.passes == 1 || wg.passes == 3),
                "tc_head_backward: bf16 1- or 3-pass images only");
  SPARF_REQUIRE(M >= 1 && HW % 4 == 0 && !(reinterpret_cast<uintptr_t>(hid) & 15), "tc_head_backward: M=%d HW=%d", M, HW);
  SPARF_REQUIRE(row.p && row.ks == ceil_div(HW, TK) && tr.p && tr.ks == ceil_div(M, TK),
                "tc_head_backward: images need %d and %d k-steps", ceil_div(HW, TK), ceil_div(M, TK));
  const HeadBwd h{M, HW, d_rgb, rgb, d_sigma, raw, hid, W9, graw, row.p, tr.p, row.ks, tr.ks, dW9, db9, db_hid, db_raw};
  if (dg.passes == 3 && wg.passes == 3) return launch_head_bwd<3, 3>(h, dg.rows, st);
  if (dg.passes == 3 && wg.passes == 1) return launch_head_bwd<3, 1>(h, dg.rows, st);
  if (dg.passes == 1 && wg.passes == 1) return launch_head_bwd<1, 1>(h, dg.rows, st);
  SPARF_REQUIRE(false, "tc_head_backward: no kernel for %d-pass row and %d-pass transposed images", dg.passes, wg.passes);
}

template <int ROWP, int TRP>
static int launch_feat_bwd(const FeatBwd& f, cudaStream_t st) {
  auto kernel = feat_bwd_kernel<ROWP, TRP>;
  SPARF_CHECK_CUDA(cudaFuncSetAttribute(kernel, cudaFuncAttributeMaxDynamicSharedMemorySize, FEAT_SMEM));
  kernel<<<ceil_div(f.M, TM), 256, FEAT_SMEM, st>>>(f);
  SPARF_CHECK_LAUNCH("feat_bwd_kernel");
  return SPARF_OK;
}

int tc_feat_backward(TcPrec dg, TcPrec wg, int M, int W, const float* d_raw, const float* d_feat, const float* feat,
                     TcImage row, TcImage tr, float* db_raw, float* db_feat, cudaStream_t st) {
  SPARF_REQUIRE(!dg.f16 && !wg.f16 && (dg.passes == 1 || dg.passes == 3) && (wg.passes == 1 || wg.passes == 3),
                "tc_feat_backward: bf16 1- or 3-pass images only");
  SPARF_REQUIRE(M >= 1 && W % 4 == 0 && (!d_feat || (feat && !(reinterpret_cast<uintptr_t>(feat) & 15))),
                "tc_feat_backward: M=%d W=%d", M, W);
  SPARF_REQUIRE(row.p && row.ks == ceil_div(W, TK) && tr.p && tr.ks == ceil_div(M, TK),
                "tc_feat_backward: images need %d and %d k-steps", ceil_div(W, TK), ceil_div(M, TK));
  const FeatBwd f{M, W, d_raw, d_feat, feat, row.p, tr.p, row.ks, tr.ks, db_raw, db_feat,
                  !(reinterpret_cast<uintptr_t>(d_feat) & 15)};
  if (dg.passes == 3 && wg.passes == 3) return launch_feat_bwd<3, 3>(f, st);
  if (dg.passes == 3 && wg.passes == 1) return launch_feat_bwd<3, 1>(f, st);
  if (dg.passes == 1 && wg.passes == 1) return launch_feat_bwd<1, 1>(f, st);
  SPARF_REQUIRE(false, "tc_feat_backward: no kernel for %d-pass row and %d-pass transposed images", dg.passes, wg.passes);
}

}

using namespace sparf;

static int alloc_images(size_t elems, cudaStream_t st, TcPrec& p) {
  SPARF_CHECK_CUDA(cudaMallocAsync(reinterpret_cast<void**>(&p.pack_a), elems * 2, st));
  SPARF_CHECK_CUDA(cudaMallocAsync(reinterpret_cast<void**>(&p.pack_b), elems * 2, st));
  p.pack_elems = elems;
  return SPARF_OK;
}

static void free_images(TcPrec& p, cudaStream_t st) {
  cudaFreeAsync(p.pack_a, st);
  cudaFreeAsync(p.pack_b, st);
}

extern "C" int sparf_tc_selftest(const float* A, const float* B, int32_t K, void* packed, float* D, sparf_stream_t stream) {
  (void)packed;
  SPARF_REQUIRE(K % 64 == 0 && K >= 64 && K <= 256, "tc_selftest: K=%d", K);
  cudaStream_t st = (cudaStream_t)stream;
  TcPrec p{false, 1};
  SPARF_TRY(alloc_images(tc_pack_elems(128, K / 32, 128), st, p));
  const TcImage a{p.pack_a, K / 32};
  int rc = tc_pack_rows(p, 128, K, A, K, 1, a, st);
  if (!rc) rc = tc_gemm_nt(p, 0, 128, 128, a, K, TcImage{}, 0, B, K, 0, nullptr, D, 128, TcOut{}, st);
  free_images(p, st);
  return rc;
}

extern "C" int sparf_tc_selftest_tn(const float* G, const float* X, int32_t rows, float* D, sparf_stream_t stream) {
  SPARF_REQUIRE(rows == 64 || rows == 128, "tc_selftest_tn: rows=%d", rows);
  cudaStream_t st = (cudaStream_t)stream;
  SPARF_CHECK_CUDA(cudaMemsetAsync(D, 0, 128 * 128 * sizeof(float), st));
  TcPrec p{false, 1};
  SPARF_TRY(alloc_images(tc_pack_elems(128, rows / 32, 128), st, p));
  const TcImage gt{p.pack_a, rows / 32};
  int rc = tc_pack_cols(p, rows, 128, G, 128, gt, st);
  if (!rc) rc = tc_gemm_tn(p, rows, 128, 128, 128, gt, X, 128, 1, D, 128, 0, nullptr, st);
  free_images(p, st);
  return rc;
}

static int selftest_images(const float* X, const float* W1, const float* E, const float* W2, int M, float* Y, float* Z,
                           float* db, int max_ctas, cudaStream_t st) {
  SPARF_REQUIRE(M >= 1 && M <= 1024, "tc_selftest_images: M=%d", M);
  const int N = 128, K = 96, KE = 40;
  TcPrec q{false, 3};
  q.max_ctas = max_ctas;
  const TcImage x{nullptr, N / TK}, d{nullptr, K / TK}, e{nullptr, ceil_div(KE, TK)}, dt{nullptr, ceil_div(M, TK)};
  const size_t nx = tc_image_elems(M, N), nd = tc_image_elems(M, K), ne = tc_image_elems(M, KE), ndt = tc_image_elems(K, M);
  SPARF_TRY(alloc_images(nx + nd + ne + ndt + tc_pack_elems(std::max(M, N), ceil_div(K + KE, TK), 0), st, q));
  TcImage xi = x, di = d, ei = e, dti = dt;
  xi.p = q.pack_a; di.p = xi.p + nx; ei.p = di.p + nd; dti.p = ei.p + ne;
  SPARF_CHECK_CUDA(cudaMemsetAsync(q.pack_a, 0xFF, (nx + nd + ne + ndt) * 2, st));
  SPARF_CHECK_CUDA(cudaMemsetAsync(db, 0, K * sizeof(float), st));
  SPARF_CHECK_CUDA(cudaMemsetAsync(Z, 0, K * N * sizeof(float), st));
  TcOut o;
  o.row = di; o.row_passes = 3;
  o.tr = dti; o.tr_passes = 3;
  int rc = tc_pack_rows(q, M, N, X, N, 1, xi, st);
  if (!rc)
    rc = tc_gemm_nn(q, M, N, K, K, xi, W1, K, 0, nullptr, 0, nullptr, nullptr, nullptr, nullptr, 0, 0, o, db, nullptr, st);
  if (!rc) rc = tc_pack_rows(q, M, KE, E, KE, 1, ei, st);
  if (!rc) rc = tc_gemm_nt(q, 0, M, 128, di, K, ei, KE, W2, K + KE, K, nullptr, Y, 128, TcOut{}, st);
  if (!rc) rc = tc_gemm_tn(q, M, K, N, N, dti, X, N, 1, Z, N, 0, nullptr, st);
  free_images(q, st);
  return rc;
}

extern "C" int sparf_tc_selftest_images(const float* X, const float* W1, const float* E, const float* W2, int32_t M, float* Y,
                                        float* Z, float* db, sparf_stream_t stream) {
  return selftest_images(X, W1, E, W2, M, Y, Z, db, 0, (cudaStream_t)stream);
}

static int selftest_wgrad(const float* G, const float* X, int M, int N, int K, int Kv, int ldx, int div, int passes,
                          int max_ctas, const int64_t* rows, float* dW, uint32_t* bits, cudaStream_t st) {
  SPARF_REQUIRE(M >= 1 && M <= (1 << 20) && N >= 1 && N <= 512 && K >= 1 && K <= 512 && Kv >= 0 && Kv <= K && ldx >= K &&
                    div >= 1 && (passes == 1 || passes == 3),
                "tc_selftest_wgrad: M=%d N=%d K=%d Kv=%d ldx=%d div=%d passes=%d", M, N, K, Kv, ldx, div, passes);
  SPARF_REQUIRE(G && X && dW, "tc_selftest_wgrad: NULL tensor");
  SPARF_CHECK_CUDA(cudaMemsetAsync(dW, 0, (size_t)N * K * sizeof(float), st));
  TcPrec p{false, passes};
  p.max_ctas = max_ctas;
  SPARF_TRY(alloc_images(std::max(tc_image_elems(N, M), tc_pack_elems(K, ceil_div(M, TK), 0)), st, p));
  const TcImage gt{p.pack_a, ceil_div(M, TK)};
  int rc = tc_pack_cols(p, M, N, G, N, gt, st);
  p.rows = RowCount{rows, 0};
  if (!rc) rc = tc_gemm_tn(p, M, N, K, Kv, gt, X, ldx, div, dW, K, 0, bits, st);
  free_images(p, st);
  return rc;
}

extern "C" int sparf_tc_selftest_wgrad(const float* G, const float* X, int32_t M, int32_t N, int32_t K, int32_t Kv, int32_t ldx,
                                       int32_t div, int32_t passes, int32_t max_ctas, float* dW, uint32_t* bits,
                                       sparf_stream_t stream) {
  return selftest_wgrad(G, X, M, N, K, Kv, ldx, div, passes, max_ctas, nullptr, dW, bits, (cudaStream_t)stream);
}

extern "C" int sparf_tc_selftest_wgrad_rows(const float* G, const float* X, int32_t M, int32_t N, int32_t K, int32_t Kv,
                                            int32_t ldx, int32_t div, int32_t passes, int32_t max_ctas, const int64_t* rows,
                                            float* dW, uint32_t* bits, sparf_stream_t stream) {
  SPARF_REQUIRE(rows, "tc_selftest_wgrad_rows: NULL row count");
  return selftest_wgrad(G, X, M, N, K, Kv, ldx, div, passes, max_ctas, rows, dW, bits, (cudaStream_t)stream);
}

extern "C" int sparf_tc_selftest_mask_bits(const float* G, const float* W, const float* X, int32_t M, int32_t N, int32_t K,
                                           int32_t max_ctas, uint16_t* img, sparf_stream_t stream) {
  SPARF_REQUIRE(M >= 1 && M <= (1 << 20) && N >= 1 && N <= 512 && K >= 2 && K <= 512 && K % 2 == 0,
                "tc_selftest_mask_bits: M=%d N=%d K=%d", M, N, K);
  SPARF_REQUIRE(G && W && X && img, "tc_selftest_mask_bits: NULL tensor");
  cudaStream_t st = (cudaStream_t)stream;
  TcPrec p{false, 3};
  p.max_ctas = max_ctas;
  const size_t ng = tc_image_elems(M, N), ngt = tc_image_elems(N, M);
  const size_t nrow = tc_image_elems(M, K), ntr = tc_image_elems(K, M);
  SPARF_TRY(alloc_images(ng + ngt + tc_pack_elems(K, ceil_div(M, TK) + ceil_div(N, TK), 0), st, p));
  uint32_t* bits = nullptr;
  float* dW = nullptr;
  const size_t nbits = (size_t)M * ceil_div(K, 32);
  SPARF_CHECK_CUDA(cudaMallocAsync(reinterpret_cast<void**>(&bits), nbits * 4 + (size_t)N * K * sizeof(float), st));
  dW = reinterpret_cast<float*>(bits + nbits);
  SPARF_CHECK_CUDA(cudaMemsetAsync(dW, 0, (size_t)N * K * sizeof(float), st));
  SPARF_CHECK_CUDA(cudaMemsetAsync(img, 0xFF, 2 * (nrow + ntr) * sizeof(uint16_t), st));
  const TcImage g{p.pack_a, ceil_div(N, TK)}, gt{p.pack_a + ng, ceil_div(M, TK)};
  TcOut o[2];
  for (int i = 0; i < 2; ++i) {
    o[i].row = TcImage{img + i * (nrow + ntr), ceil_div(K, TK)};
    o[i].tr = TcImage{img + i * (nrow + ntr) + nrow, ceil_div(M, TK)};
    o[i].row_passes = o[i].tr_passes = 3;
  }
  int rc = tc_pack_rows(p, M, N, G, N, 1, g, st);
  if (!rc) rc = tc_pack_cols(p, M, N, G, N, gt, st);
  if (!rc) rc = tc_gemm_tn(p, M, N, K, K, gt, X, K, 1, dW, K, 0, bits, st);
  if (!rc)
    rc = tc_gemm_nn(p, M, N, K, K, g, W, K, 0, X, K, nullptr, nullptr, nullptr, nullptr, 0, 0, o[0], nullptr, nullptr, st);
  if (!rc)
    rc = tc_gemm_nn(p, M, N, K, K, g, W, K, 0, nullptr, 0, bits, nullptr, nullptr, nullptr, 0, 0, o[1], nullptr, nullptr, st);
  cudaFreeAsync(bits, st);
  free_images(p, st);
  return rc;
}

extern "C" int sparf_tc_selftest_persistent(const float* X, const float* W1, const float* E, const float* W2, int32_t M,
                                            float* Y, float* Z, float* db, int32_t max_ctas, sparf_stream_t stream) {
  return selftest_images(X, W1, E, W2, M, Y, Z, db, max_ctas, (cudaStream_t)stream);
}

static int selftest_chain(const float* enc, int M, int E3, int nt, int skip, const float* W, const float* bias, int passes,
                          int f16, int max_ctas, int chain, uint32_t outputs, const int64_t* rows, float* H, uint16_t* last,
                          uint32_t* bits, cudaStream_t st) {
  SPARF_REQUIRE(enc && W && bias && H && M >= 1 && M <= (1 << 20) && E3 >= 1 && (passes == 1 || passes == 3),
                "tc_selftest_chain: M=%d E3=%d passes=%d", M, E3, passes);
  const int E3p = ceil_div(E3, TK) * TK, eks = E3p / TK;
  SPARF_REQUIRE(tc_chain_supported(CH_W, E3p, nt, skip) && (outputs >> (nt - 2) & 1), "tc_selftest_chain: nt=%d skip=%d", nt, skip);
  SPARF_REQUIRE(!bits || chain, "tc_selftest_chain: mask bits come from the chain only");
  TcPrec p{f16 != 0, passes};
  p.max_ctas = max_ctas;
  p.rows = RowCount{rows, 0};
  const bool feat = outputs >> (nt - 1) & 1;
  size_t wel = 0;
  for (int l = 0; l < nt; ++l) wel += tc_image_elems(CH_W, chain_ks(l, skip, eks) * TK);
  const size_t ne = tc_image_elems(M, E3p), nh = tc_image_elems(M, CH_W);
  SPARF_TRY(alloc_images(std::max(ne + 2 * nh, wel), st, p));
  float* scratch = nullptr;
  SPARF_CHECK_CUDA(cudaMallocAsync(reinterpret_cast<void**>(&scratch), (size_t)M * CH_W * sizeof(float), st));
  const TcImage ei{p.pack_a, eks}, himg[2] = {{p.pack_a + ne, CH_KS}, {p.pack_a + ne + nh, CH_KS}};
  TcOut lo;
  if (feat && last) {
    lo.row = TcImage{last, CH_KS};
    lo.row_passes = passes;
  }
  int rc = tc_pack_rows(p, M, E3p, enc, E3p, 1, ei, st);
  const float* Wl[SPARF_MAX_TRUNK];
  const float* bl[SPARF_MAX_TRUNK];
  float* Hl[SPARF_MAX_TRUNK];
  uint32_t* bl_bits[SPARF_MAX_TRUNK] = {};
  TcImage wimg[SPARF_MAX_TRUNK];
  size_t wo = 0, io = 0;
  for (int l = 0; l < nt; ++l) {
    Wl[l] = W + wo;
    bl[l] = bias + (size_t)l * CH_W;
    Hl[l] = outputs >> l & 1 ? H + (size_t)l * M * CH_W : nullptr;
    if (bits && l < nt - 2) bl_bits[l] = bits + (size_t)l * M * (CH_W / 32);
    wimg[l] = TcImage{p.pack_b + io, chain_ks(l, skip, eks)};
    wo += (size_t)CH_W * ((l == 0 ? E3 : CH_W) + (l == skip ? E3 : 0));
    io += tc_image_elems(CH_W, wimg[l].ks * TK);
  }
  if (chain) {
    for (int l = 0; l < nt && !rc; ++l)
      rc = tc_pack_nt(p, CH_W, l == 0 ? eks : CH_KS, l == 0 ? E3 : CH_W, l == skip ? eks : 0, E3, Wl[l],
                      (l == 0 ? E3 : CH_W) + (l == skip ? E3 : 0), CH_W, wimg[l], st);
    if (!rc) rc = tc_trunk_chain(p, M, CH_W, nt, skip, ei, wimg, bl, Hl, bl_bits, lo, st);
  } else {
    for (int l = 0; l < (feat ? nt : nt - 1) && !rc; ++l) {
      TcOut o;
      if (l < nt - 1) {
        o.row = himg[l & 1];
        o.row_passes = passes;
      } else {
        o = lo;
      }
      rc = tc_gemm_nt(p, 1, M, CH_W, l == 0 ? ei : himg[(l - 1) & 1], l == 0 ? E3 : CH_W, l == skip ? ei : TcImage{}, E3, Wl[l],
                      (l == 0 ? E3 : CH_W) + (l == skip ? E3 : 0), CH_W, bl[l], Hl[l] ? Hl[l] : scratch, CH_W, o, st);
    }
  }
  cudaFreeAsync(scratch, st);
  free_images(p, st);
  return rc;
}

extern "C" int sparf_tc_selftest_chain(const float* enc, int32_t M, int32_t E3, int32_t nt, int32_t skip, const float* W,
                                       const float* bias, int32_t passes, int32_t f16, int32_t max_ctas, int32_t chain,
                                       uint32_t outputs, const int64_t* rows, float* H, uint16_t* last,
                                       sparf_stream_t stream) {
  return selftest_chain(enc, M, E3, nt, skip, W, bias, passes, f16, max_ctas, chain, outputs, rows, H, last, nullptr,
                        (cudaStream_t)stream);
}

extern "C" int sparf_tc_selftest_chain_bits(const float* enc, int32_t M, int32_t E3, int32_t nt, int32_t skip, const float* W,
                                            const float* bias, int32_t passes, int32_t f16, int32_t max_ctas,
                                            const int64_t* rows, float* H, uint32_t* bits, sparf_stream_t stream) {
  SPARF_REQUIRE(bits && nt >= 3 && nt <= SPARF_MAX_TRUNK, "tc_selftest_chain_bits: nt=%d, bits", nt);
  return selftest_chain(enc, M, E3, nt, skip, W, bias, passes, f16, max_ctas, 1, (1u << nt) - 1, rows, H, nullptr, bits,
                        (cudaStream_t)stream);
}

extern "C" int sparf_tc_selftest_dgrad_chain(const float* G, int32_t M, int32_t E3, int32_t nt, int32_t skip, const float* W,
                                             const uint32_t* bits, int32_t dg_passes, int32_t wg_passes, int32_t max_ctas,
                                             int32_t chain, const int64_t* rows, uint16_t* tr, uint16_t* row, float* db,
                                             sparf_stream_t stream) {
  SPARF_REQUIRE(G && W && bits && tr && db && M >= 1 && M <= (1 << 20) && E3 >= 1 && nt >= 3 && nt <= SPARF_MAX_TRUNK &&
                    skip > 0 && skip < nt && (!row || skip <= nt - 3),
                "tc_selftest_dgrad_chain: M=%d E3=%d nt=%d skip=%d", M, E3, nt, skip);
  cudaStream_t st = (cudaStream_t)stream;
  TcPrec dg{false, dg_passes}, wg{false, wg_passes};
  dg.max_ctas = wg.max_ctas = max_ctas;
  dg.rows = wg.rows = RowCount{rows, 0};
  const int top = nt - 2;
  const size_t nh = tc_image_elems(M, CH_W), ntr = tc_image_elems(CH_W, M), nw = tc_image_elems(CH_W, CH_W);
  SPARF_TRY(alloc_images(std::max(3 * nh, (top + 1) * nw), st, dg));
  SPARF_CHECK_CUDA(cudaMemsetAsync(db, 0, (size_t)top * CH_W * sizeof(float), st));
  const TcImage gin{dg.pack_a, CH_KS}, scratch[2] = {{dg.pack_a + nh, CH_KS}, {dg.pack_a + 2 * nh, CH_KS}};
  const float* Wl[SPARF_MAX_TRUNK];
  int ldw[SPARF_MAX_TRUNK];
  size_t wo = 0;
  for (int l = 0; l < nt; ++l) {
    Wl[l] = W + wo;
    ldw[l] = (l == 0 ? E3 : CH_W) + (l == skip ? E3 : 0);
    wo += (size_t)CH_W * ldw[l];
  }
  TcImage trl[SPARF_MAX_TRUNK], rowl[SPARF_MAX_TRUNK], wimg[SPARF_MAX_TRUNK];
  const uint32_t* bl[SPARF_MAX_TRUNK] = {};
  float* dbl[SPARF_MAX_TRUNK] = {};
  for (int l = 1; l <= top; ++l) {
    trl[l] = TcImage{tr + (size_t)(l - 1) * ntr, ceil_div(M, TK)};
    if (row && (l == 1 || l - 1 == skip)) rowl[l] = TcImage{row + (l == 1 ? 0 : nh), CH_KS};
    bl[l] = bits + (size_t)(l - 1) * M * (CH_W / 32);
    dbl[l] = db + (size_t)(l - 1) * CH_W;
    wimg[l] = TcImage{dg.pack_b + (size_t)l * nw, CH_KS};
  }
  int rc = tc_pack_rows(dg, M, CH_W, G, CH_W, 1, gin, st);
  if (chain) {
    for (int l = 1; l <= top && !rc; ++l) rc = tc_pack_nn(dg, CH_W, CH_W, CH_W, Wl[l], ldw[l], 0, wimg[l], st);
    if (!rc) rc = tc_dgrad_chain(dg, wg, M, CH_W, top, gin, wimg, bl, dbl, trl, rowl, st);
  } else {
    TcImage g = gin;
    for (int l = top; l >= 1 && !rc; --l) {
      TcOut o;
      o.row = rowl[l].p ? rowl[l] : scratch[l & 1];
      o.tr = trl[l];
      o.row_passes = dg_passes;
      o.tr_passes = wg_passes;
      rc = tc_gemm_nn(dg, M, CH_W, CH_W, CH_W, g, Wl[l], ldw[l], 0, nullptr, 0, bl[l], nullptr, nullptr, nullptr, 0, 0, o,
                      dbl[l], nullptr, st);
      g = o.row;
    }
  }
  free_images(dg, st);
  return rc;
}
```

### sparf_b200/csrc/gemm_wgmma.cuh

```cuda
#pragma once
#include "common.cuh"

namespace sparf {

struct TcPrec {
  bool f16;
  int passes;
  uint16_t* pack_a = nullptr;
  uint16_t* pack_b = nullptr;
  size_t pack_elems = 0;
  int max_ctas = 0;
  RowCount rows{nullptr, 0};
};

struct TcImage {
  uint16_t* p = nullptr;
  int ks = 0;
};

struct TcOut {
  TcImage row, tr;
  int row_passes = 0, tr_passes = 0;
};

size_t tc_image_elems(int rows, int cols);
size_t tc_pack_elems(int rows, int ksteps, int cols);

int tc_pack_rows(TcPrec p, int M, int K, const float* X, int ldx, int div, TcImage img, cudaStream_t st);
int tc_pack_cols(TcPrec p, int M, int N, const float* X, int ldx, TcImage img, cudaStream_t st);

int tc_gemm_nt(TcPrec p, int act, int M, int N, TcImage a1, int K1v, TcImage a2, int K2v, const float* W, int ldw, int wcol2,
               const float* bias, float* Y, int ldy, const TcOut& out, cudaStream_t st);
bool tc_chain_supported(int W, int E3p, int nt, int skip);
int tc_chain_ksteps(int l, int skip, int E3p);
int tc_pack_nt(TcPrec p, int N, int ks1, int K1v, int ks2, int K2v, const float* W, int ldw, int wcol2, TcImage img,
               cudaStream_t st);
int tc_trunk_chain(TcPrec p, int M, int W, int nt, int skip, TcImage enc, const TcImage* wimg, const float* const* bias,
                   float* const* H, uint32_t* const* bits, const TcOut& last, cudaStream_t st);
int tc_pack_nn(TcPrec p, int Kout, int N, int Kv, const float* W, int ldw, int wcol, TcImage img, cudaStream_t st);
int tc_dgrad_chain(TcPrec dg, TcPrec wg, int M, int W, int top, TcImage in, const TcImage* wimg, const uint32_t* const* bits,
                   float* const* db, const TcImage* tr, const TcImage* row, cudaStream_t st);
int tc_gemm_nn(TcPrec p, int M, int N, int Kout, int Kv, TcImage g, const float* W, int ldw, int wcol, const float* mask_src,
               int ldmask, const uint32_t* mask_bits, const float* r1_vec, const float* r1_row, float* D, int ldd,
               int accumulate, const TcOut& out, float* db, float* r1_wgrad, cudaStream_t st);
int tc_gemm_tn(TcPrec p, int M, int N, int K, int Kv, TcImage gt, const float* X, int ldx, int div, float* dW, int ldw,
               int wcol, uint32_t* bits, cudaStream_t st);

int tc_head_backward(TcPrec dg, TcPrec wg, int M, int HW, const float* d_rgb, const float* rgb, const float* d_sigma,
                     const float* raw, const float* hid, const float* W9, float* graw, TcImage row, TcImage tr, float* dW9,
                     float* db9, float* db_hid, float* db_raw, cudaStream_t st);

int tc_feat_backward(TcPrec dg, TcPrec wg, int M, int W, const float* d_raw, const float* d_feat, const float* feat,
                     TcImage row, TcImage tr, float* db_raw, float* db_feat, cudaStream_t st);

}
```

### sparf_b200/csrc/mlp.cu

```cuda
#include <algorithm>

#include "common.cuh"
#include "gemm_wgmma.cuh"

namespace sparf {

__global__ void c2f_weights_kernel(C2F c, int L_xyz, int L_view, float* __restrict__ wts ) {
  int j = threadIdx.x;
  if (j < 16) wts[j] = j < L_xyz ? band_weight(c, L_xyz, j) : 0.f;
  else if (j < 32) wts[j] = (j - 16) < L_view ? band_weight(c, L_view, j - 16) : 0.f;
}

template <bool DYN = false>
__global__ void encode_xyz_kernel(long long total, int S, int L, int E3p, const float* __restrict__ origins,
                                  const float* __restrict__ dirs, const float* __restrict__ t,
                                  const float* __restrict__ wts, float* __restrict__ enc, RowCount rc) {
  long long idx = (long long)blockIdx.x * blockDim.x + threadIdx.x;
  if (idx >= (DYN ? live_rows<DYN>(total / E3p, rc) * E3p : total)) return;
  if constexpr (DYN) {
    const long long s0 = row_start<true>(rc);
    origins += s0 * 3;
    if (dirs) dirs += s0 * 3;
    t += s0;
    enc += s0 * E3p;
// ... 372 lines not shown
__global__ void ray_reduce_kernel(int nrays, int S, int C, const float* __restrict__ in, float* __restrict__ out,
                                  RowCount rc) {
  int idx = blockIdx.x * blockDim.x + threadIdx.x;
  if (idx >= (int)live_rows<DYN, false>(nrays, rc) * C) return;
  int c = idx % C, r = idx / C;
  float acc = 0.f;
  for (int k = 0; k < S; ++k) acc += in[((size_t)r * S + k) * C + c];
  out[idx] = acc;
}

template <bool DYN = false>
__global__ void posenc_bwd_kernel(int nrays, int S, int L, int E3p, const float* __restrict__ enc,
                                  const float* __restrict__ Genc, const float* __restrict__ t,
                                  float* __restrict__ d_o, float* __restrict__ d_d, RowCount rc) {
  const int lane = threadIdx.x & 31;
  int r = blockIdx.x * (blockDim.x >> 5) + (threadIdx.x >> 5);
  if (r >= (int)live_rows<DYN, false>(nrays, rc)) return;
  float so[3] = {0.f, 0.f, 0.f}, sd[3] = {0.f, 0.f, 0.f};
  for (int k = lane; k < S; k += 32) {
    size_t m = (size_t)r * S + k;
    const float* e = enc + m * E3p;
    const float* g = Genc + m * E3p;
    float tk = t ? t[m] : 0.f;
#pragma unroll
    for (int c = 0; c < 3; ++c) {
      float gx = g[c];
      for (int j = 0; j < L; ++j) {
        float f = band_freq(j);
        int is = 3 + c * 2 * L + j, ic = is + L;
        gx += f * (g[is] * e[ic] - g[ic] * e[is]);
      }
      so[c] += gx;
      sd[c] += tk * gx;
    }
  }
#pragma unroll
  for (int c = 0; c < 3; ++c) {
#pragma unroll
    for (int s = 16; s > 0; s >>= 1) {
      so[c] += __shfl_xor_sync(0xffffffffu, so[c], s);
      sd[c] += __shfl_xor_sync(0xffffffffu, sd[c], s);
    }
  }
  if (lane == 0) {
#pragma unroll
    for (int c = 0; c < 3; ++c) {
      if (d_o) d_o[r * 3 + c] += so[c];
      if (d_d) d_d[r * 3 + c] += sd[c];
    }
  }
}

template <bool DYN = false>
__global__ void direnc_bwd_kernel(int nrays, int L, int Evp, const float* __restrict__ denc,
                                  const float* __restrict__ Gdenc, const float* __restrict__ dirs,
                                  float* __restrict__ d_d, RowCount rc) {
  int r = blockIdx.x * blockDim.x + threadIdx.x;
  if (r >= (int)live_rows<DYN, false>(nrays, rc)) return;
  const float* e = denc + (size_t)r * Evp;
  const float* g = Gdenc + (size_t)r * Evp;
  float gu[3];
#pragma unroll
  for (int c = 0; c < 3; ++c) {
    float gx = g[c];
    for (int j = 0; j < L; ++j) {
      float f = band_freq(j);
      int is = 3 + c * 2 * L + j, ic = is + L;
      gx += f * (g[is] * e[ic] - g[ic] * e[is]);
    }
    gu[c] = gx;
  }
  float dx = dirs[r * 3], dy = dirs[r * 3 + 1], dz = dirs[r * 3 + 2];
  float len = fmaxf(sqrtf(dx * dx + dy * dy + dz * dz), 1e-12f);
  float ux = dx / len, uy = dy / len, uz = dz / len;
  float dot = gu[0] * ux + gu[1] * uy + gu[2] * uz;
  d_d[r * 3] += (gu[0] - ux * dot) / len;
  d_d[r * 3 + 1] += (gu[1] - uy * dot) / len;
  d_d[r * 3 + 2] += (gu[2] - uz * dot) / len;
}

static inline int pad8(int x) { return (x + 7) / 8 * 8; }

struct MlpDims {
  int E3, E3p, Ev, Evp, W, HW, nt, skip;
};

static MlpDims mlp_dims(const SparfMLP* mlp) {
  MlpDims d;
  d.E3 = 3 + 6 * mlp->L_xyz;
  d.Ev = 3 + 6 * mlp->L_view;
  d.E3p = pad8(d.E3);
  d.Evp = pad8(d.Ev);
  d.W = mlp->width;
  d.HW = mlp->head_width;
  d.nt = mlp->n_trunk;
  d.skip = mlp->skip_layer;
  return d;
}

static int validate_trunk(const SparfMLP* mlp) {
  SPARF_REQUIRE(mlp != nullptr, "mlp is NULL");
  SPARF_REQUIRE(mlp->n_trunk >= 2 && mlp->n_trunk <= SPARF_MAX_TRUNK, "n_trunk=%d unsupported", mlp->n_trunk);
  SPARF_REQUIRE(mlp->width % 8 == 0 && mlp->width >= 8, "width=%d must be a multiple of 8", mlp->width);
  SPARF_REQUIRE(mlp->L_xyz >= 1 && mlp->L_xyz <= SPARF_MAX_L && mlp->L_view >= 1 && mlp->L_view <= SPARF_MAX_L,
                "L_xyz=%d / L_view=%d unsupported", mlp->L_xyz, mlp->L_view);
  SPARF_REQUIRE(mlp->skip_layer < mlp->n_trunk && mlp->skip_layer != 0, "skip_layer=%d unsupported", mlp->skip_layer);
  SPARF_REQUIRE(!mlp->use_c2f || mlp->progress, "use_c2f needs the progress pointer");
  for (int i = 0; i < mlp->n_trunk; ++i)
    SPARF_REQUIRE(mlp->trunk_w[i] && mlp->trunk_b[i], "trunk layer %d has NULL tensors", i);
  return SPARF_OK;
}

static int validate_mlp(const SparfMLP* mlp) {
  SPARF_TRY(validate_trunk(mlp));
  SPARF_REQUIRE(mlp->head_width % 8 == 0 && mlp->head_width >= 8, "head_width=%d must be a multiple of 8", mlp->head_width);
  SPARF_REQUIRE(mlp->head_w[0] && mlp->head_b[0] && mlp->head_w[1] && mlp->head_b[1], "head has NULL tensors");
  return SPARF_OK;
}

enum class Pass { kForward, kTapedForward, kRecomputeBackward, kTapedBackward, kGradient };

static int chunk_rows(Pass pass) {
  switch (pass) {
    case Pass::kForward: return 65536;
    case Pass::kRecomputeBackward:
    case Pass::kGradient: return 32768;
    default: return 131072;
  }
}

static int chunk_rays(int S, Pass pass) { return std::max(1, chunk_rows(pass) / S); }

struct Carver {
  char* p;
  size_t used;
  float* take(size_t nfloats) {
    size_t bytes = align_up(nfloats * sizeof(float), 256);
    float* r = reinterpret_cast<float*>(p + used);
    used += bytes;
    return r;
  }
  TcImage image(int rows, int cols) {
    return TcImage{reinterpret_cast<uint16_t*>(take((tc_image_elems(rows, cols) + 1) / 2)), ceil_div(cols, 32)};
  }
};

struct Tape {
  float *enc, *denc, *hid, *raw;
  float* H[SPARF_MAX_TRUNK];
  uint32_t* bits[SPARF_MAX_TRUNK];
};

static bool trunk_chained(const MlpDims& d, bool tc) { return tc && tc_chain_supported(d.W, d.E3p, d.nt, d.skip); }

static size_t tape_layout(const MlpDims& d, bool tc, int R, int S, char* base, Tape* tp) {
  const size_t M = (size_t)R * S;
  Carver cv{base, 0};
  Tape t{};
  t.enc = cv.take(M * d.E3p);
  t.denc = cv.take((size_t)R * d.Evp);
  t.hid = cv.take(M * d.HW);
  t.raw = cv.take(M);
  for (int l = 0; l < d.nt; ++l) t.H[l] = cv.take(M * d.W);
  for (int l = 0; trunk_chained(d, tc) && l < d.nt - 2; ++l) t.bits[l] = reinterpret_cast<uint32_t*>(cv.take(M * (d.W / 32)));
  if (tp) *tp = t;
  return cv.used + 256;
}

constexpr size_t kMaxTapeBytes = (size_t)16 << 30;

static Tape tape_chunk(const Tape& t, const MlpDims& d, int r0, int S) {
  const size_t m0 = (size_t)r0 * S;
  Tape c{};
  c.enc = t.enc + m0 * d.E3p;
  c.denc = t.denc + (size_t)r0 * d.Evp;
  c.hid = t.hid + m0 * d.HW;
  c.raw = t.raw + m0;
  for (int l = 0; l < d.nt; ++l) {
    c.H[l] = t.H[l] + m0 * d.W;
    c.bits[l] = t.bits[l] ? t.bits[l] + m0 * (d.W / 32) : nullptr;
  }
  return c;
}

struct Ws {
  float *wts, *rgbv, *G0, *G1, *Genc, *Ghid, *gpre, *graw, *Gdtmp, *Gdenc;
  float *ones, *colsum_sink;
  Tape act;
  TcImage encimg, dencimg, Himg[2], Grow[2], Gtr[SPARF_MAX_TRUNK - 1], ghid_row, ghid_tr;
  TcImage wimg[SPARF_MAX_TRUNK];
  TcImage nnimg[SPARF_MAX_TRUNK];
  uint32_t* mask_bits;
  uint16_t* pack_b;
  size_t pack_elems;
};

static size_t carve(const MlpDims& d, bool tc, int nrc, int S, Pass pass, bool head, char* base, Ws* out) {
  const size_t Mc = (size_t)nrc * S;
  const bool grad_only = pass == Pass::kGradient;
  const bool fwd_here = pass == Pass::kForward || pass == Pass::kRecomputeBackward || grad_only;
  const bool bwd = pass == Pass::kRecomputeBackward || pass == Pass::kTapedBackward || grad_only;
  const bool chain = trunk_chained(d, tc);
  Carver cv{base, 0};
  Ws w{};
  w.wts = cv.take(32);
  if (fwd_here) {
    w.act.enc = cv.take(Mc * d.E3p);
    if (head) {
      w.act.denc = cv.take((size_t)nrc * d.Evp);
      w.act.hid = cv.take(Mc * d.HW);
      w.act.raw = cv.take(Mc);
      w.rgbv = cv.take(Mc * 3);
    }
    const int nH = pass == Pass::kForward ? 2 : grad_only ? d.nt - 1 : d.nt;
    if (chain && pass == Pass::kForward) {
      for (int l = d.nt - 2; l < d.nt; ++l) w.act.H[l] = cv.take(Mc * d.W);
    } else {
      for (int l = 0; l < nH; ++l) w.act.H[l] = cv.take(Mc * d.W);
      for (int l = nH; l < d.nt; ++l) w.act.H[l] = w.act.H[l & 1];
    }
    if (grad_only) w.act.H[d.nt - 1] = nullptr;
    for (int l = 0; chain && bwd && l < d.nt - 2; ++l) w.act.bits[l] = reinterpret_cast<uint32_t*>(cv.take(Mc * (d.W / 32)));
  }
  if (bwd && !tc) {
    w.G0 = cv.take(Mc * d.W);
    w.G1 = cv.take(Mc * d.W);
  }
  if (bwd) {
    w.Genc = cv.take(Mc * d.E3p);
    if (grad_only) w.ones = cv.take(Mc);
    if (!tc && head) {
      w.Ghid = cv.take(Mc * d.HW);
      w.gpre = cv.take(Mc * 4);
    }
    if (head) {
      w.graw = cv.take(Mc);
      w.Gdtmp = cv.take(Mc * d.Evp);
      w.Gdenc = cv.take((size_t)nrc * d.Evp);
    }
  }
  if (tc && pass != Pass::kTapedBackward) {
    w.encimg = cv.image((int)Mc, d.E3p);
    if (head) w.dencimg = cv.image((int)Mc, d.Evp);
    if (chain) {
      if (head) w.Himg[(d.nt - 1) & 1] = cv.image((int)Mc, d.W);
      for (int l = 0; l < d.nt; ++l) w.wimg[l] = cv.image(d.W, tc_chain_ksteps(l, d.skip, d.E3p) * 32);
    } else {
      for (TcImage& h : w.Himg) h = cv.image((int)Mc, d.W);
    }
  }
  if (tc && bwd) {
    for (TcImage& g : w.Grow) g = cv.image((int)Mc, d.W);
    const int ntr = chain ? d.nt - 1 : 2;
    for (int i = 0; i < (grad_only ? 1 : ntr); ++i) w.Gtr[i] = cv.image(d.W, (int)Mc);
    for (int i = 1; grad_only && i < ntr; ++i) w.Gtr[i] = w.Gtr[0];
    for (int l = 1; chain && l <= d.nt - 2; ++l) w.nnimg[l] = cv.image(d.W, d.W);
    if (head) {
      w.ghid_row = cv.image((int)Mc, d.HW);
      w.ghid_tr = cv.image(d.HW, (int)Mc);
    }
    if (grad_only) w.colsum_sink = cv.take(d.W);
    else w.mask_bits = reinterpret_cast<uint32_t*>(cv.take(Mc * ceil_div(d.W, 32)));
  }
  if (tc) {
    const int HW = head ? d.HW : 0, Evp = head ? d.Evp : 0;
    const int wmax = std::max(std::max(d.W, HW), std::max(d.E3p, Evp));
    w.pack_elems = tc_pack_elems(wmax, ceil_div(wmax, 32) + ceil_div(std::max(d.E3p, Evp), 32), 0);
    w.pack_b = reinterpret_cast<uint16_t*>(cv.take((w.pack_elems + 1) / 2));
  }
  if (out) *out = w;
  return cv.used + 256;
}

static size_t workspace_need(const MlpDims& d, bool tc, long long R, int S, Pass pass, bool head) {
  auto bytes = [&](Pass p) {
    return carve(d, tc, (int)std::min<long long>(R, chunk_rays(S, p)), S, p, head, nullptr, nullptr);
  };
  return head && pass == Pass::kForward ? std::max(bytes(Pass::kForward), bytes(Pass::kTapedForward)) : bytes(pass);
}

struct Call {
  MlpDims d;
  bool tc;
  int nrc;
  Ws w;
  EnginePrec ep;
  Tape tape;
  RowCount rc{nullptr, 0};

  void at(long long m0) {
    if (!rc.rows) return;
    rc.m0 = m0;
    for (TcPrec* p : {&ep.fwd, &ep.dgrad, &ep.wgrad}) p->rows = rc;
  }
};

static int begin_call(const char* who, const SparfMLP* mlp, int engine, long long R, int S, Pass pass, bool head, void* tape,
                      size_t tape_bytes, void* workspace, size_t workspace_bytes, Call* c, long long tape_R = -1) {
  const int e = resolve_engine(engine);
  if (e < 0) {
    set_error("%s: engine %d not available in this build", who, engine);
    return SPARF_ERR_UNSUPPORTED;
  }
  SPARF_TRY(head ? validate_mlp(mlp) : validate_trunk(mlp));
  c->d = mlp_dims(mlp);
  c->tc = is_tc(e);
  if (tape_R < 0) tape_R = R;
  if (tape) {
    SPARF_REQUIRE(tape_bytes >= tape_layout(c->d, c->tc, (int)tape_R, S, nullptr, nullptr), "%s: tape %zu bytes too small",
                  who, tape_bytes);
    tape_layout(c->d, c->tc, (int)tape_R, S, reinterpret_cast<char*>(align_up(reinterpret_cast<size_t>(tape), 256)),
                &c->tape);
  }
  const size_t need = workspace_need(c->d, c->tc, R, S, pass, head);
  if (workspace_bytes < need) {
    set_error("%s: workspace %zu < %zu bytes", who, workspace_bytes, need);
    return SPARF_ERR_WORKSPACE;
  }
  c->nrc = (int)std::min<long long>(R, chunk_rays(S, pass));
  carve(c->d, c->tc, c->nrc, S, pass, head, reinterpret_cast<char*>(workspace), &c->w);
  c->ep = engine_prec(e);
  for (TcPrec* p : {&c->ep.fwd, &c->ep.dgrad, &c->ep.wgrad}) {
    p->pack_b = c->w.pack_b;
    p->pack_elems = c->w.pack_elems;
  }
  return SPARF_OK;
}

static inline int trunk_in_main(const MlpDims& d, int l) { return l == 0 ? d.E3p : d.W; }
static inline int trunk_in_main_valid(const MlpDims& d, int l) { return l == 0 ? d.E3 : d.W; }
static inline int trunk_ldw(const MlpDims& d, int l) {
  return (l == 0 ? d.E3 : d.W) + (l == d.skip ? d.E3 : 0);
}

static int chunk_encode_xyz(const SparfMLP* mlp, const Call& c, long long Mc, int S, const float* origins,
                            const float* dirs, const float* t, float* enc, cudaStream_t st) {
  const MlpDims& d = c.d;
  C2F c2f{mlp->use_c2f, mlp->c2f_start, mlp->c2f_range, mlp->progress};
  c2f_weights_kernel<<<1, 32, 0, st>>>(c2f, mlp->L_xyz, mlp->L_view, c.w.wts);
  SPARF_CHECK_LAUNCH("c2f_weights_kernel");
  if (c.rc.rows)
    encode_xyz_kernel<true><<<ceil_div(Mc * d.E3p, 256), 256, 0, st>>>(Mc * d.E3p, S, mlp->L_xyz, d.E3p, origins, dirs, t,
                                                                       c.w.wts, enc, c.rc);
  else
    encode_xyz_kernel<<<ceil_div(Mc * d.E3p, 256), 256, 0, st>>>(Mc * d.E3p, S, mlp->L_xyz, d.E3p, origins, dirs, t, c.w.wts,
                                                                 enc, c.rc);
  SPARF_CHECK_LAUNCH("encode_xyz_kernel");
  if (c.tc) SPARF_TRY(tc_pack_rows(c.ep.fwd, (int)Mc, d.E3p, enc, d.E3p, 1, c.w.encimg, st));
  return SPARF_OK;
}

static int chunk_trunk(const SparfMLP* mlp, const Call& c, long long Mc, const float* enc, float* const* H,
                       uint32_t* const* bits, const float* noise, float* raw, float* sigma, bool last_image, cudaStream_t st) {
  const MlpDims& d = c.d;
  const Ws& w = c.w;
  const float* in = enc;
  const bool chained = trunk_chained(d, c.tc);
  if (chained) {
    const float* bias[SPARF_MAX_TRUNK];
    for (int l = 0; l < d.nt; ++l) {
      const bool last = l == d.nt - 1;
      bias[l] = mlp->trunk_b[l] + (last ? 1 : 0);
      if (last && !H[l]) break;
      const int ldw = trunk_ldw(d, l);
      SPARF_TRY(tc_pack_nt(c.ep.fwd, d.W, ceil_div(trunk_in_main(d, l), 32), trunk_in_main_valid(d, l),
                           l == d.skip ? w.encimg.ks : 0, d.E3, mlp->trunk_w[l] + (last ? ldw : 0), ldw, d.W, w.wimg[l], st));
    }
    TcOut o;
    if (last_image) {
      o.row = w.Himg[(d.nt - 1) & 1];
      o.row_passes = c.ep.fwd.passes;
    }
    SPARF_TRY(tc_trunk_chain(c.ep.fwd, (int)Mc, d.W, d.nt, d.skip, w.encimg, w.wimg, bias, H, bits, o, st));
  }
  for (int l = 0; l < d.nt; ++l) {
    const bool last = l == d.nt - 1;
    const int ldw = trunk_ldw(d, l);
    const float* Wl = mlp->trunk_w[l] + (last ? ldw : 0);
    const float* bl = mlp->trunk_b[l] + (last ? 1 : 0);
    const bool sk = l == d.skip;
    if (chained) {
    } else if (c.tc && H[l]) {
      TcOut o;
      if (!last || last_image) {
        o.row = w.Himg[l & 1];
        o.row_passes = c.ep.fwd.passes;
      }
      SPARF_TRY(tc_gemm_nt(c.ep.fwd, 1, (int)Mc, d.W, l == 0 ? w.encimg : w.Himg[(l - 1) & 1], trunk_in_main_valid(d, l),
                           sk ? w.encimg : TcImage{}, d.E3, Wl, ldw, d.W, bl, H[l], d.W, o, st));
    } else if (H[l]) {
      SPARF_TRY(gemm_nt((int)Mc, d.W, in, trunk_in_main(d, l), trunk_in_main(d, l), trunk_in_main_valid(d, l),
                        sk ? enc : nullptr, d.E3p, d.E3p, d.E3, 1, Wl, ldw, d.W, bl, H[l], d.W, st));
    }
    if (last && (raw || sigma)) {
      if (c.rc.rows)
        rowdot_kernel<0, true><<<ceil_div(Mc, 8), 256, 0, st>>>(Mc, d.W, in, d.W, mlp->trunk_w[l], ldw, mlp->trunk_b[l], noise,
                                                                raw, sigma, c.rc);
      else
        rowdot_kernel<0><<<ceil_div(Mc, 8), 256, 0, st>>>(Mc, d.W, in, d.W, mlp->trunk_w[l], ldw, mlp->trunk_b[l], noise, raw,
                                                         sigma, c.rc);
      SPARF_CHECK_LAUNCH("rowdot_kernel<0>");
    }
    in = H[l];
  }
  return SPARF_OK;
}

static int chunk_forward(const SparfMLP* mlp, const Call& c, int nr, int S, const float* origins, const float* dirs,
                         const float* t, const float* noise, const Tape& v, float* sigma, float* rgb, cudaStream_t st) {
  const MlpDims& d = c.d;
  const long long Mc = (long long)nr * S;
  SPARF_TRY(chunk_encode_xyz(mlp, c, Mc, S, origins, dirs, t, v.enc, st));
  if (c.rc.rows)
    encode_dir_kernel<true><<<ceil_div((long long)nr * d.Evp, 256), 256, 0, st>>>(nr * d.Evp, mlp->L_view, d.Evp, dirs,
                                                                                  c.w.wts + 16, v.denc, c.rc);
  else
    encode_dir_kernel<<<ceil_div((long long)nr * d.Evp, 256), 256, 0, st>>>(nr * d.Evp, mlp->L_view, d.Evp, dirs, c.w.wts + 16,
                                                                            v.denc, c.rc);
  SPARF_CHECK_LAUNCH("encode_dir_kernel");
  if (c.tc) SPARF_TRY(tc_pack_rows(c.ep.fwd, (int)Mc, d.Evp, v.denc, d.Evp, S, c.w.dencimg, st));
  SPARF_TRY(chunk_trunk(mlp, c, Mc, v.enc, v.H, v.bits, noise, v.raw, sigma, true, st));
  if (c.tc)
    SPARF_TRY(tc_gemm_nt(c.ep.fwd, 1, (int)Mc, d.HW, c.w.Himg[(d.nt - 1) & 1], d.W, c.w.dencimg, d.Ev, mlp->head_w[0],
                         d.W + d.Ev, d.W, mlp->head_b[0], v.hid, d.HW, TcOut{}, st));
  else
    SPARF_TRY(gemm_nt((int)Mc, d.HW, v.H[d.nt - 1], d.W, d.W, d.W, v.denc, d.Evp, d.Evp, d.Ev, S, mlp->head_w[0], d.W + d.Ev,
                      d.W, mlp->head_b[0], v.hid, d.HW, st));
  if (c.rc.rows)
    rowdot_kernel<1, true><<<ceil_div(Mc, 8), 256, 0, st>>>(Mc, d.HW, v.hid, d.HW, mlp->head_w[1], d.HW, mlp->head_b[1], nullptr,
                                                            nullptr, rgb, c.rc);
  else
    rowdot_kernel<1><<<ceil_div(Mc, 8), 256, 0, st>>>(Mc, d.HW, v.hid, d.HW, mlp->head_w[1], d.HW, mlp->head_b[1], nullptr,
                                                     nullptr, rgb, c.rc);
  SPARF_CHECK_LAUNCH("rowdot_kernel<1>");
  return SPARF_OK;
}

static int rows_call(const char* who, Call* c, int S, const int64_t* rows, const int64_t* start = nullptr) {
  if (!rows) return SPARF_OK;
  if (!c->tc) {
    set_error("%s: a device row count needs a tensor-core engine (tc_3x, tc_1x or tc_3x_w1)", who);
    return SPARF_ERR_UNSUPPORTED;
  }
  SPARF_REQUIRE(S == 1, "%s: a device row count needs S = 1 (one-sample rays), got S = %d", who, S);
  c->rc.rows = rows;
  c->rc.start = start;
  return SPARF_OK;
}

static int mlp_forward(const SparfMLP* mlp, int engine, int R, int S, const float* origins, const float* dirs, const float* t,
                       const float* noise, float* sigma, float* rgb, void* tape, size_t tape_bytes, void* workspace,
                       size_t workspace_bytes, cudaStream_t st, const int64_t* rows = nullptr,
                       const int64_t* start = nullptr, long long tape_R = -1) {
  Call c;
  const char* who = start ? "mlp_forward_tape_span" : rows ? "mlp_forward_tape_rows" : tape ? "mlp_forward_tape" : "mlp_forward";
  SPARF_TRY(begin_call(who, mlp, engine, R, S, tape ? Pass::kTapedForward : Pass::kForward, true, tape, tape_bytes, workspace,
                       workspace_bytes, &c, tape_R));
  SPARF_TRY(rows_call(who, &c, S, rows, start));
  Tape v = c.w.act;
  v.raw = nullptr;
  for (int r0 = 0; r0 < R; r0 += c.nrc) {
    const int nr = std::min(c.nrc, R - r0);
    c.at(r0);
    const size_t m0 = (size_t)r0 * S;
    SPARF_TRY(chunk_forward(mlp, c, nr, S, origins + (size_t)r0 * 3, dirs + (size_t)r0 * 3, t + m0, noise ? noise + m0 : nullptr,
                            tape ? tape_chunk(c.tape, c.d, r0, S) : v, sigma + m0, rgb + m0 * 3, st));
  }
  return SPARF_OK;
}

constexpr int kSimtSlab = 2048;

static TcImage grad_tr(const Ws& w, int i, long long Mc) { return TcImage{w.Gtr[i].p, ceil_div(Mc, 32)}; }
static TcOut grad_images(const Call& c, int i, long long Mc) {
  TcOut o;
  o.row = c.w.Grow[i];
  o.tr = grad_tr(c.w, i, Mc);
  o.row_passes = c.ep.dgrad.passes;
  o.tr_passes = c.ep.wgrad.passes;
  return o;
}

static int head_backward_simt(const SparfMLP* mlp, const Call& c, long long Mc, int S, const float* d_rgb, const float* rgbv,
                              const float* d_sigma, const Tape& v, const SparfMLPGrad* grad, bool dir_grad, cudaStream_t st) {
  const MlpDims& d = c.d;
  const Ws& w = c.w;
  const int ldw8 = d.W + d.Ev;
  const float* feat = v.H[d.nt - 1];
  head_grad_kernel<<<ceil_div(Mc, 256), 256, 0, st>>>(Mc, d_rgb, rgbv, d_sigma, v.raw, w.gpre, w.graw);
  SPARF_CHECK_LAUNCH("head_grad_kernel");
  narrow_wgrad_kernel<3><<<ceil_div(Mc, 512), 128, 0, st>>>(Mc, d.HW, 512, w.gpre, 4, v.hid, d.HW, grad->head_w[1], d.HW,
                                                             grad->head_b[1]);
  SPARF_CHECK_LAUNCH("narrow_wgrad_kernel<3>");
  narrow_dgrad_kernel<<<ceil_div(Mc * d.HW, 256), 256, 0, st>>>(Mc * d.HW, d.HW, w.gpre, mlp->head_w[1], d.HW, v.hid, w.Ghid);
  SPARF_CHECK_LAUNCH("narrow_dgrad_kernel");
  SPARF_TRY(gemm_tn((int)Mc, d.HW, d.W, d.W, kSimtSlab, w.Ghid, d.HW, feat, d.W, 1, grad->head_w[0], ldw8, 0, st));
  SPARF_TRY(gemm_tn((int)Mc, d.HW, d.Evp, d.Ev, kSimtSlab, w.Ghid, d.HW, v.denc, d.Evp, S, grad->head_w[0], ldw8, d.W, st));
  colsum_kernel<<<dim3(ceil_div(d.HW, 32), ceil_div(Mc, 1024)), 256, 0, st>>>(Mc, d.HW, 1024, w.Ghid, d.HW, grad->head_b[0]);
  SPARF_CHECK_LAUNCH("colsum_kernel(head)");
  SPARF_TRY(gemm_nn((int)Mc, d.HW, d.W, d.W, w.Ghid, d.HW, mlp->head_w[0], ldw8, 0, feat, d.W, nullptr, nullptr, w.G0, d.W, 0, st));
  if (dir_grad)
    SPARF_TRY(gemm_nn((int)Mc, d.HW, d.Evp, d.Ev, w.Ghid, d.HW, mlp->head_w[0], ldw8, d.W, nullptr, 0, nullptr, nullptr, w.Gdtmp,
                      d.Evp, 0, st));
  return SPARF_OK;
}

static int head_backward_tc(const SparfMLP* mlp, const Call& c, long long Mc, int S, const float* d_rgb, const float* rgbv,
                            const float* d_sigma, const Tape& v, const SparfMLPGrad* grad, bool dir_grad, cudaStream_t st) {
  const MlpDims& d = c.d;
  const Ws& w = c.w;
  const EnginePrec& ep = c.ep;
  const int ldw8 = d.W + d.Ev;
  const float* feat = v.H[d.nt - 1];
  const TcImage ghid_t{w.ghid_tr.p, ceil_div(Mc, 32)}, ghid = w.ghid_row;
  SPARF_TRY(tc_head_backward(ep.dgrad, ep.wgrad, (int)Mc, d.HW, d_rgb, rgbv, d_sigma, v.raw, v.hid, mlp->head_w[1], w.graw, ghid,
                             ghid_t, grad->head_w[1], grad->head_b[1], grad->head_b[0], grad->trunk_b[d.nt - 1], st));
  SPARF_TRY(tc_gemm_tn(ep.wgrad, (int)Mc, d.HW, d.W, d.W, ghid_t, feat, d.W, 1, grad->head_w[0], ldw8, 0, w.mask_bits, st));
  SPARF_TRY(tc_gemm_tn(ep.wgrad, (int)Mc, d.HW, d.Evp, d.Ev, ghid_t, v.denc, d.Evp, S, grad->head_w[0], ldw8, d.W, nullptr, st));
  SPARF_TRY(tc_gemm_nn(ep.dgrad, (int)Mc, d.HW, d.W, d.W, ghid, mlp->head_w[0], ldw8, 0, nullptr, 0, w.mask_bits, nullptr,
                       nullptr, nullptr, 0, 0, grad_images(c, 0, Mc), grad->trunk_b[d.nt - 1] + 1, nullptr, st));
  if (dir_grad)
    SPARF_TRY(tc_gemm_nn(ep.dgrad, (int)Mc, d.HW, d.Evp, d.Ev, ghid, mlp->head_w[0], ldw8, d.W, nullptr, 0, nullptr, nullptr,
                         nullptr, w.Gdtmp, d.Evp, 0, TcOut{}, nullptr, nullptr, st));
  return SPARF_OK;
}

static int trunk_backward_simt(const SparfMLP* mlp, const Call& c, long long Mc, const float* enc, float* const* H,
                               const float* graw, const SparfMLPGrad* grad, bool enc_grad, cudaStream_t st) {
  const MlpDims& d = c.d;
  float* G = c.w.G0;
  float* Gn = c.w.G1;
  bool genc_written = false;
  for (int l = d.nt - 1; l >= 0; --l) {
    const bool last = l == d.nt - 1;
    const bool r1 = last && graw;
    const int ldw = trunk_ldw(d, l);
    const float* in = l == 0 ? enc : H[l - 1];
    const int Kin = trunk_in_main(d, l), Kinv = trunk_in_main_valid(d, l);
    const int rowoff = last ? 1 : 0;
    const float* Wl = mlp->trunk_w[l] + (size_t)rowoff * ldw;
    if (grad) {
      float* dWl = grad->trunk_w[l] + (size_t)rowoff * ldw;
      SPARF_TRY(gemm_tn((int)Mc, d.W, Kin, Kinv, kSimtSlab, G, d.W, in, Kin, 1, dWl, ldw, 0, st));
      if (l == d.skip) SPARF_TRY(gemm_tn((int)Mc, d.W, d.E3p, d.E3, kSimtSlab, G, d.W, enc, d.E3p, 1, dWl, ldw, d.W, st));
      colsum_kernel<<<dim3(ceil_div(d.W, 32), ceil_div(Mc, 1024)), 256, 0, st>>>(Mc, d.W, 1024, G, d.W, grad->trunk_b[l] + rowoff);
      SPARF_CHECK_LAUNCH("colsum_kernel(trunk)");
      if (r1) {
        narrow_wgrad_kernel<1><<<ceil_div(Mc, 512), 128, 0, st>>>(Mc, d.W, 512, graw, 1, in, d.W, grad->trunk_w[l], ldw,
                                                                   grad->trunk_b[l]);
        SPARF_CHECK_LAUNCH("narrow_wgrad_kernel<1>");
      }
    }
    if (l > 0)
      SPARF_TRY(gemm_nn((int)Mc, d.W, d.W, d.W, G, d.W, Wl, ldw, 0, in, d.W, r1 ? graw : nullptr, r1 ? mlp->trunk_w[l] : nullptr,
                        Gn, d.W, 0, st));
    if (enc_grad && (l == d.skip || l == 0)) {
      SPARF_TRY(gemm_nn((int)Mc, d.W, d.E3p, d.E3, G, d.W, Wl, ldw, l == 0 ? 0 : d.W, nullptr, 0, nullptr, nullptr, c.w.Genc,
                        d.E3p, genc_written ? 1 : 0, st));
      genc_written = true;
    }
    std::swap(G, Gn);
  }
  return SPARF_OK;
}

static int grad_tr_buf(const MlpDims& d, bool chained, int l) { return chained ? (l ? d.nt - 1 - l : 0) : (d.nt - 1 - l) & 1; }
static int grad_row(const MlpDims& d, bool chained, int l) {
  return chained ? (l == 0 || l == d.nt - 1 ? 0 : 1) : (d.nt - 1 - l) & 1;
}

static int chunk_dgrad_chain(const SparfMLP* mlp, const Call& c, long long Mc, uint32_t* const* bits, const SparfMLPGrad* grad,
                             bool enc_grad, cudaStream_t st) {
  const MlpDims& d = c.d;
  const int top = d.nt - 2;
  const uint32_t* mask[SPARF_MAX_TRUNK] = {};
  float* db[SPARF_MAX_TRUNK] = {};
  TcImage tr[SPARF_MAX_TRUNK], row[SPARF_MAX_TRUNK];
  for (int l = top; l >= 1; --l) {
    SPARF_TRY(tc_pack_nn(c.ep.dgrad, d.W, d.W, d.W, mlp->trunk_w[l], trunk_ldw(d, l), 0, c.w.nnimg[l], st));
    mask[l] = bits[l - 1];
    db[l] = grad ? grad->trunk_b[l - 1] : c.w.colsum_sink;
    tr[l] = grad_tr(c.w, grad_tr_buf(d, true, l - 1), Mc);
    if (enc_grad && (l - 1 == 0 || l - 1 == d.skip)) row[l] = c.w.Grow[grad_row(d, true, l - 1)];
  }
  return tc_dgrad_chain(c.ep.dgrad, c.ep.wgrad, (int)Mc, d.W, top, c.w.Grow[grad_row(d, true, top)], c.w.nnimg, mask, db, tr,
                        row, st);
}

static int trunk_backward_tc(const SparfMLP* mlp, const Call& c, long long Mc, const float* enc, float* const* H,
                             uint32_t* const* bits, const float* graw, const SparfMLPGrad* grad, bool enc_grad, cudaStream_t st) {
  const MlpDims& d = c.d;
  const EnginePrec& ep = c.ep;
  const bool chained = trunk_chained(d, true);
  bool genc_written = false;
  for (int l = d.nt - 1; l >= 0; --l) {
    const bool last = l == d.nt - 1;
    const bool r1 = last && graw;
    const int ldw = trunk_ldw(d, l);
    const float* in = l == 0 ? enc : H[l - 1];
    const int Kin = trunk_in_main(d, l), Kinv = trunk_in_main_valid(d, l);
    const int rowoff = last ? 1 : 0;
    const float* Wl = mlp->trunk_w[l] + (size_t)rowoff * ldw;
    const int gi = (d.nt - 1 - l) & 1;
    const bool nn = l > 0 && (!chained || last);
    uint32_t* wbits = grad && nn && !r1 ? c.w.mask_bits : nullptr;
    if (grad) {
      float* dWl = grad->trunk_w[l] + (size_t)rowoff * ldw;
      const TcImage gt = grad_tr(c.w, grad_tr_buf(d, chained, l), Mc);
      SPARF_TRY(tc_gemm_tn(ep.wgrad, (int)Mc, d.W, Kin, Kinv, gt, in, Kin, 1, dWl, ldw, 0, wbits, st));
      if (l == d.skip) SPARF_TRY(tc_gemm_tn(ep.wgrad, (int)Mc, d.W, d.E3p, d.E3, gt, enc, d.E3p, 1, dWl, ldw, d.W, nullptr, st));
    }
    if (nn)
      SPARF_TRY(tc_gemm_nn(ep.dgrad, (int)Mc, d.W, d.W, d.W, c.w.Grow[gi], Wl, ldw, 0, wbits ? nullptr : in, d.W, wbits,
                           r1 ? graw : nullptr, r1 ? mlp->trunk_w[l] : nullptr, nullptr, 0, 0, grad_images(c, gi ^ 1, Mc),
                           grad ? grad->trunk_b[l - 1] : nullptr, grad && r1 ? grad->trunk_w[l] : nullptr, st));
    if (enc_grad && (l == d.skip || l == 0)) {
      SPARF_TRY(tc_gemm_nn(ep.dgrad, (int)Mc, d.W, d.E3p, d.E3, c.w.Grow[grad_row(d, chained, l)], Wl, ldw, l == 0 ? 0 : d.W,
                           nullptr, 0, nullptr, nullptr, nullptr, c.w.Genc, d.E3p, genc_written ? 1 : 0, TcOut{}, nullptr,
                           nullptr, st));
      genc_written = true;
    }
    if (chained && last) SPARF_TRY(chunk_dgrad_chain(mlp, c, Mc, bits, grad, enc_grad, st));
  }
  return SPARF_OK;
}

static int mlp_backward(const SparfMLP* mlp, int engine, int R, int S, const float* origins, const float* dirs, const float* t,
                        const float* noise, const float* rgb_fwd, void* tape, size_t tape_bytes, const float* d_sigma,
                        const float* d_rgb, const SparfMLPGrad* grad, float* d_origins, float* d_dirs, void* workspace,
                        size_t workspace_bytes, cudaStream_t st, const int64_t* rows = nullptr) {
  Call c;
  const char* who = rows ? "mlp_backward_tape_rows" : tape ? "mlp_backward_tape" : "mlp_backward";
  SPARF_TRY(begin_call(who, mlp, engine, R, S, tape ? Pass::kTapedBackward : Pass::kRecomputeBackward, true, tape, tape_bytes,
                       workspace, workspace_bytes, &c));
  SPARF_TRY(rows_call(who, &c, S, rows));
  const MlpDims& d = c.d;
  const Ws& w = c.w;
  const bool need_rays = d_origins != nullptr || d_dirs != nullptr;
  for (int r0 = 0; r0 < R; r0 += c.nrc) {
    const int nr = std::min(c.nrc, R - r0);
    c.at(r0);
    const long long Mc = (long long)nr * S;
    const size_t m0 = (size_t)r0 * S;
    const float* d_c = dirs + (size_t)r0 * 3;
    const Tape v = tape ? tape_chunk(c.tape, d, r0, S) : w.act;
    const float* rgbv = tape ? rgb_fwd + m0 * 3 : w.rgbv;
    if (!tape)
      SPARF_TRY(chunk_forward(mlp, c, nr, S, origins + (size_t)r0 * 3, d_c, t + m0, noise ? noise + m0 : nullptr, v, nullptr,
                              w.rgbv, st));
    SPARF_TRY(c.tc ? head_backward_tc(mlp, c, Mc, S, d_rgb + m0 * 3, rgbv, d_sigma + m0, v, grad, d_dirs != nullptr, st)
                   : head_backward_simt(mlp, c, Mc, S, d_rgb + m0 * 3, rgbv, d_sigma + m0, v, grad, d_dirs != nullptr, st));
    if (d_dirs) {
      if (c.rc.rows) {
        ray_reduce_kernel<true><<<ceil_div((long long)nr * d.Evp, 256), 256, 0, st>>>(nr, S, d.Evp, w.Gdtmp, w.Gdenc, c.rc);
        SPARF_CHECK_LAUNCH("ray_reduce_kernel");
        direnc_bwd_kernel<true><<<ceil_div(nr, 128), 128, 0, st>>>(nr, mlp->L_view, d.Evp, v.denc, w.Gdenc, d_c,
                                                                   d_dirs + (size_t)r0 * 3, c.rc);
      } else {
        ray_reduce_kernel<<<ceil_div((long long)nr * d.Evp, 256), 256, 0, st>>>(nr, S, d.Evp, w.Gdtmp, w.Gdenc, c.rc);
        SPARF_CHECK_LAUNCH("ray_reduce_kernel");
        direnc_bwd_kernel<<<ceil_div(nr, 128), 128, 0, st>>>(nr, mlp->L_view, d.Evp, v.denc, w.Gdenc, d_c, d_dirs + (size_t)r0 * 3,
                                                             c.rc);
      }
      SPARF_CHECK_LAUNCH("direnc_bwd_kernel");
    }
    SPARF_TRY(c.tc ? trunk_backward_tc(mlp, c, Mc, v.enc, v.H, v.bits, w.graw, grad, need_rays, st)
                   : trunk_backward_simt(mlp, c, Mc, v.enc, v.H, w.graw, grad, need_rays, st));
    if (need_rays) {
      float* d_o = d_origins ? d_origins + (size_t)r0 * 3 : nullptr;
      float* d_d = d_dirs ? d_dirs + (size_t)r0 * 3 : nullptr;
      if (c.rc.rows)
        posenc_bwd_kernel<true><<<ceil_div(nr, 4), 128, 0, st>>>(nr, S, mlp->L_xyz, d.E3p, v.enc, w.Genc, t + m0, d_o, d_d, c.rc);
      else
        posenc_bwd_kernel<<<ceil_div(nr, 4), 128, 0, st>>>(nr, S, mlp->L_xyz, d.E3p, v.enc, w.Genc, t + m0, d_o, d_d, c.rc);
      SPARF_CHECK_LAUNCH("posenc_bwd_kernel");
    }
  }
  return SPARF_OK;
}

static int selftest_featgrad(const float* d_raw, const float* d_feat, const float* feat, int M, int W, TcPrec dg, TcPrec wg,
                             uint16_t* img, float* sums, float* scratch, cudaStream_t st) {
  const size_t nrow = tc_image_elems(M, W), ntr = tc_image_elems(W, M);
  const TcImage row{img, ceil_div(W, 32)}, tr{img + nrow, ceil_div(M, 32)};
  const TcImage row_ref{img + nrow + ntr, row.ks}, tr_ref{img + 2 * nrow + ntr, tr.ks};
  float* ref = sums + W + 1;
  SPARF_CHECK_CUDA(cudaMemsetAsync(img, 0xFF, 2 * (nrow + ntr) * sizeof(uint16_t), st));
  SPARF_CHECK_CUDA(cudaMemsetAsync(sums, 0, 2 * (W + 1) * sizeof(float), st));
  SPARF_TRY(tc_feat_backward(dg, wg, M, W, d_raw, d_feat, feat, row, tr, sums, sums + 1, st));
  relu_mask_kernel<<<ceil_div((long long)M * W, 256), 256, 0, st>>>((long long)M * W, feat, d_feat, scratch);
  SPARF_CHECK_LAUNCH("relu_mask_kernel");
  colsum_kernel<<<dim3(ceil_div(W, 32), ceil_div(M, 1024)), 256, 0, st>>>(M, W, 1024, scratch, W, ref + 1);
  SPARF_CHECK_LAUNCH("colsum_kernel");
  colsum_kernel<<<dim3(1, ceil_div(M, 1024)), 256, 0, st>>>(M, 1, 1024, d_raw, 1, ref);
  SPARF_CHECK_LAUNCH("colsum_kernel");
  SPARF_TRY(tc_pack_rows(dg, M, W, scratch, W, 1, row_ref, st));
  return tc_pack_cols(wg, M, W, scratch, W, tr_ref, st);
}

static int selftest_head(const float* d_rgb, const float* rgb, const float* d_sigma, const float* raw, const float* hid,
                         const float* W9, int M, int HW, TcPrec dg, TcPrec wg, uint16_t* img, float* graw, float* scratch,
                         cudaStream_t st) {
  const size_t nrow = tc_image_elems(M, HW), ntr = tc_image_elems(HW, M);
  const TcImage row{img, ceil_div(HW, 32)}, tr{img + nrow, ceil_div(M, 32)};
  const TcImage row_ref{img + nrow + ntr, row.ks}, tr_ref{img + 2 * nrow + ntr, tr.ks};
  float *Ghid = scratch, *gpre = Ghid + (size_t)M * HW, *sums = gpre + (size_t)M * 4;
  SPARF_CHECK_CUDA(cudaMemsetAsync(img, 0xFF, 2 * (nrow + ntr) * sizeof(uint16_t), st));
  SPARF_CHECK_CUDA(cudaMemsetAsync(sums, 0, (4 * HW + 4) * sizeof(float), st));
  SPARF_TRY(tc_head_backward(dg, wg, M, HW, d_rgb, rgb, d_sigma, raw, hid, W9, graw, row, tr, sums, sums + 3 * HW,
                             sums + 3 * HW + 3, sums + 4 * HW + 3, st));
  head_grad_kernel<<<ceil_div(M, 256), 256, 0, st>>>(M, d_rgb, rgb, d_sigma, raw, gpre, graw + M);
  SPARF_CHECK_LAUNCH("head_grad_kernel");
  narrow_dgrad_kernel<<<ceil_div((long long)M * HW, 256), 256, 0, st>>>((long long)M * HW, HW, gpre, W9, HW, hid, Ghid);
  SPARF_CHECK_LAUNCH("narrow_dgrad_kernel");
  SPARF_TRY(tc_pack_rows(dg, M, HW, Ghid, HW, 1, row_ref, st));
  return tc_pack_cols(wg, M, HW, Ghid, HW, tr_ref, st);
}

}

using namespace sparf;

extern "C" size_t sparf_mlp_workspace_bytes(const SparfMLP* mlp, int32_t R, int32_t S, int32_t backward, int32_t engine) {
  if (!mlp || R <= 0 || S <= 0) return 0;
  const int e = resolve_engine(engine);
  if (e < 0 || backward < 0 || backward > 2) return 0;
  const Pass pass = backward == 0 ? Pass::kForward : backward == 1 ? Pass::kRecomputeBackward : Pass::kTapedBackward;
  return workspace_need(mlp_dims(mlp), is_tc(e), R, S, pass, true);
}

extern "C" int sparf_mlp_forward(const SparfMLP* mlp, int32_t engine, int32_t R, int32_t S, const float* origins,
                                 const float* dirs, const float* t, const float* noise, float* sigma, float* rgb,
                                 void* workspace, size_t workspace_bytes, sparf_stream_t stream) {
  SPARF_REQUIRE(mlp && R >= 0 && S > 0, "mlp_forward: bad arguments");
  SPARF_REQUIRE(origins && dirs && t && sigma && rgb, "mlp_forward: NULL tensor");
  if (R == 0) return SPARF_OK;
  return mlp_forward(mlp, engine, R, S, origins, dirs, t, noise, sigma, rgb, nullptr, 0, workspace, workspace_bytes,
                     (cudaStream_t)stream);
}

extern "C" int sparf_mlp_backward(const SparfMLP* mlp, int32_t engine, int32_t R, int32_t S, const float* origins,
                                  const float* dirs, const float* t, const float* noise, const float* d_sigma,
                                  const float* d_rgb, const SparfMLPGrad* grad, float* d_origins, float* d_dirs,
                                  void* workspace, size_t workspace_bytes, sparf_stream_t stream) {
  SPARF_REQUIRE(mlp && R >= 0 && S > 0, "mlp_backward: bad arguments");
  SPARF_REQUIRE(origins && dirs && t && d_sigma && d_rgb && grad, "mlp_backward: NULL tensor");
  if (R == 0) return SPARF_OK;
  return mlp_backward(mlp, engine, R, S, origins, dirs, t, noise, nullptr, nullptr, 0, d_sigma, d_rgb, grad, d_origins, d_dirs,
                      workspace, workspace_bytes, (cudaStream_t)stream);
}

extern "C" size_t sparf_mlp_tape_bytes(const SparfMLP* mlp, int32_t engine, int32_t R, int32_t S) {
  if (!mlp || R <= 0 || S <= 0 || resolve_engine(engine) < 0 || validate_mlp(mlp)) return 0;
  const size_t n = tape_layout(mlp_dims(mlp), is_tc(resolve_engine(engine)), R, S, nullptr, nullptr);
  return n <= kMaxTapeBytes ? n : 0;
}

extern "C" int sparf_mlp_forward_tape(const SparfMLP* mlp, int32_t engine, int32_t R, int32_t S, const float* origins,
                                      const float* dirs, const float* t, const float* noise, float* sigma, float* rgb,
                                      void* tape, size_t tape_bytes, void* workspace, size_t workspace_bytes,
                                      sparf_stream_t stream) {
  SPARF_REQUIRE(mlp && R > 0 && S > 0 && origins && dirs && t && sigma && rgb && tape, "mlp_forward_tape: bad arguments");
  return mlp_forward(mlp, engine, R, S, origins, dirs, t, noise, sigma, rgb, tape, tape_bytes, workspace, workspace_bytes,
                     (cudaStream_t)stream);
}

extern "C" int sparf_mlp_backward_tape(const SparfMLP* mlp, int32_t engine, int32_t R, int32_t S, const float* origins,
                                       const float* dirs, const float* t, const float* sigma, const float* rgb,
                                       const float* d_sigma, const float* d_rgb, const SparfMLPGrad* grad,
                                       float* d_origins, float* d_dirs, void* tape, size_t tape_bytes, void* workspace,
                                       size_t workspace_bytes, sparf_stream_t stream) {
  SPARF_REQUIRE(mlp && R > 0 && S > 0 && origins && dirs && t && sigma && rgb && d_sigma && d_rgb && grad && tape,
                "mlp_backward_tape: bad arguments");
  return mlp_backward(mlp, engine, R, S, origins, dirs, t, nullptr, rgb, tape, tape_bytes, d_sigma, d_rgb, grad, d_origins,
                      d_dirs, workspace, workspace_bytes, (cudaStream_t)stream);
}

extern "C" int sparf_mlp_forward_tape_rows(const SparfMLP* mlp, int32_t engine, int32_t R, int32_t S, const int64_t* rows,
                                           const float* origins, const float* dirs, const float* t, const float* noise,
                                           float* sigma, float* rgb, void* tape, size_t tape_bytes, void* workspace,
                                           size_t workspace_bytes, sparf_stream_t stream) {
  SPARF_REQUIRE(mlp && R > 0 && S > 0 && rows && origins && dirs && t && sigma && rgb && tape,
                "mlp_forward_tape_rows: bad arguments");
  return mlp_forward(mlp, engine, R, S, origins, dirs, t, noise, sigma, rgb, tape, tape_bytes, workspace, workspace_bytes,
                     (cudaStream_t)stream, rows);
}

extern "C" int sparf_mlp_forward_tape_span(const SparfMLP* mlp, int32_t engine, int32_t C, int32_t cap, const int64_t* begin,
                                           const int64_t* end, const float* origins, const float* dirs, const float* t,
                                           const float* noise, float* sigma, float* rgb, void* tape, size_t tape_bytes,
                                           void* workspace, size_t workspace_bytes, sparf_stream_t stream) {
  SPARF_REQUIRE(mlp && C > 0 && cap > 0 && cap <= C && begin && end && origins && dirs && t && sigma && rgb && tape,
                "mlp_forward_tape_span: bad arguments");
  return mlp_forward(mlp, engine, cap, 1, origins, dirs, t, noise, sigma, rgb, tape, tape_bytes, workspace, workspace_bytes,
                     (cudaStream_t)stream, end, begin, C);
}

extern "C" int sparf_mlp_backward_tape_rows(const SparfMLP* mlp, int32_t engine, int32_t R, int32_t S, const int64_t* rows,
                                            const float* origins, const float* dirs, const float* t, const float* sigma,
                                            const float* rgb, const float* d_sigma, const float* d_rgb,
                                            const SparfMLPGrad* grad, float* d_origins, float* d_dirs, void* tape,
                                            size_t tape_bytes, void* workspace, size_t workspace_bytes,
                                            sparf_stream_t stream) {
  SPARF_REQUIRE(mlp && R > 0 && S > 0 && rows && origins && dirs && t && sigma && rgb && d_sigma && d_rgb && grad && tape,
                "mlp_backward_tape_rows: bad arguments");
  return mlp_backward(mlp, engine, R, S, origins, dirs, t, nullptr, rgb, tape, tape_bytes, d_sigma, d_rgb, grad, d_origins,
                      d_dirs, workspace, workspace_bytes, (cudaStream_t)stream, rows);
}

extern "C" size_t sparf_density_workspace_bytes(const SparfMLP* mlp, int64_t M, int32_t backward, int32_t engine) {
  if (!mlp || M <= 0) return 0;
  const int e = resolve_engine(engine);
  if (e < 0 || backward < 0 || backward > 2) return 0;
  const Pass pass = backward == 0 ? Pass::kForward : backward == 1 ? Pass::kRecomputeBackward : Pass::kGradient;
  return workspace_need(mlp_dims(mlp), is_tc(e), M, 1, pass, false);
}

extern "C" int sparf_density_forward(const SparfMLP* mlp, int32_t engine, int64_t M, const float* points, float* raw,
                                     float* feat, void* workspace, size_t workspace_bytes, sparf_stream_t stream) {
  SPARF_REQUIRE(mlp && M >= 0, "density_forward: bad arguments");
  if (M == 0) return SPARF_OK;
  SPARF_REQUIRE(points && raw, "density_forward: NULL tensor");
  Call c;
  SPARF_TRY(begin_call("density_forward", mlp, engine, M, 1, Pass::kForward, false, nullptr, 0, workspace, workspace_bytes, &c));
  const cudaStream_t st = (cudaStream_t)stream;
  const MlpDims& d = c.d;
  Tape v = c.w.act;
  for (long long p0 = 0; p0 < M; p0 += c.nrc) {
    const int n = (int)std::min<long long>(c.nrc, M - p0);
    v.H[d.nt - 1] = feat ? feat + (size_t)p0 * d.W : nullptr;
    SPARF_TRY(chunk_encode_xyz(mlp, c, n, 1, points + (size_t)p0 * 3, nullptr, nullptr, v.enc, st));
    SPARF_TRY(chunk_trunk(mlp, c, n, v.enc, v.H, nullptr, nullptr, raw + p0, nullptr, false, st));
  }
  return SPARF_OK;
}

extern "C" int sparf_density_backward(const SparfMLP* mlp, int32_t engine, int64_t M, const float* points, const float* d_raw,
                                      const float* d_feat, const SparfMLPGrad* grad, float* d_points, void* workspace,
                                      size_t workspace_bytes, sparf_stream_t stream) {
  SPARF_REQUIRE(mlp && M >= 0, "density_backward: bad arguments");
  if (M == 0) return SPARF_OK;
  SPARF_REQUIRE(points && grad, "density_backward: NULL tensor");
  Call c;
  SPARF_TRY(begin_call("density_backward", mlp, engine, M, 1, Pass::kRecomputeBackward, false, nullptr, 0, workspace,
                       workspace_bytes, &c));
  const cudaStream_t st = (cudaStream_t)stream;
  const MlpDims& d = c.d;
  float* db = grad->trunk_b[d.nt - 1];
  Tape v = c.w.act;
  if (!d_feat) v.H[d.nt - 1] = nullptr;
  for (long long p0 = 0; p0 < M; p0 += c.nrc) {
    const int n = (int)std::min<long long>(c.nrc, M - p0);
    const float* dr = d_raw ? d_raw + p0 : nullptr;
    const float* df = d_feat ? d_feat + (size_t)p0 * d.W : nullptr;
    SPARF_TRY(chunk_encode_xyz(mlp, c, n, 1, points + (size_t)p0 * 3, nullptr, nullptr, v.enc, st));
    SPARF_TRY(chunk_trunk(mlp, c, n, v.enc, v.H, v.bits, nullptr, nullptr, nullptr, false, st));
    if (c.tc) {
      SPARF_TRY(tc_feat_backward(c.ep.dgrad, c.ep.wgrad, n, d.W, dr, df, v.H[d.nt - 1], c.w.Grow[0], grad_tr(c.w, 0, n), db,
                                 db + 1, st));
    } else if (df) {
      relu_mask_kernel<<<ceil_div((long long)n * d.W, 256), 256, 0, st>>>((long long)n * d.W, v.H[d.nt - 1], df, c.w.G0);
      SPARF_CHECK_LAUNCH("relu_mask_kernel");
    } else {
      SPARF_CHECK_CUDA(cudaMemsetAsync(c.w.G0, 0, (size_t)n * d.W * sizeof(float), st));
    }
    SPARF_TRY(c.tc ? trunk_backward_tc(mlp, c, n, v.enc, v.H, v.bits, dr, grad, d_points != nullptr, st)
                   : trunk_backward_simt(mlp, c, n, v.enc, v.H, dr, grad, d_points != nullptr, st));
    if (d_points) {
      posenc_bwd_kernel<<<ceil_div(n, 4), 128, 0, st>>>(n, 1, mlp->L_xyz, d.E3p, v.enc, c.w.Genc, nullptr,
                                                       d_points + (size_t)p0 * 3, nullptr, c.rc);
      SPARF_CHECK_LAUNCH("posenc_bwd_kernel");
    }
  }
  return SPARF_OK;
}

extern "C" int sparf_density_gradient(const SparfMLP* mlp, int32_t engine, int64_t M, const float* points, float* grad_points,
                                      void* workspace, size_t workspace_bytes, sparf_stream_t stream) {
  SPARF_REQUIRE(mlp && M >= 0, "density_gradient: bad arguments");
  if (M == 0) return SPARF_OK;
  SPARF_REQUIRE(points && grad_points, "density_gradient: NULL tensor");
  Call c;
  SPARF_TRY(begin_call("density_gradient", mlp, engine, M, 1, Pass::kGradient, false, nullptr, 0, workspace, workspace_bytes,
                       &c));
  const cudaStream_t st = (cudaStream_t)stream;
  const MlpDims& d = c.d;
  const Tape& v = c.w.act;
  fill_kernel<<<ceil_div(c.nrc, 256), 256, 0, st>>>(c.nrc, 1.f, c.w.ones);
  SPARF_CHECK_LAUNCH("fill_kernel");
  for (long long p0 = 0; p0 < M; p0 += c.nrc) {
    const int n = (int)std::min<long long>(c.nrc, M - p0);
    float* gp = grad_points + (size_t)p0 * 3;
    SPARF_CHECK_CUDA(cudaMemsetAsync(gp, 0, (size_t)n * 3 * sizeof(float), st));
    SPARF_TRY(chunk_encode_xyz(mlp, c, n, 1, points + (size_t)p0 * 3, nullptr, nullptr, v.enc, st));
    SPARF_TRY(chunk_trunk(mlp, c, n, v.enc, v.H, v.bits, nullptr, nullptr, nullptr, false, st));
    if (c.tc)
      SPARF_CHECK_CUDA(cudaMemsetAsync(c.w.Grow[0].p, 0, tc_image_elems(n, d.W) * sizeof(uint16_t), st));
    else
      SPARF_CHECK_CUDA(cudaMemsetAsync(c.w.G0, 0, (size_t)n * d.W * sizeof(float), st));
    SPARF_TRY(c.tc ? trunk_backward_tc(mlp, c, n, v.enc, v.H, v.bits, c.w.ones, nullptr, true, st)
                   : trunk_backward_simt(mlp, c, n, v.enc, v.H, c.w.ones, nullptr, true, st));
    posenc_bwd_kernel<<<ceil_div(n, 4), 128, 0, st>>>(n, 1, mlp->L_xyz, d.E3p, v.enc, c.w.Genc, nullptr, gp, nullptr, c.rc);
    SPARF_CHECK_LAUNCH("posenc_bwd_kernel");
  }
  return SPARF_OK;
}

extern "C" int sparf_tc_selftest_head(const float* d_rgb, const float* rgb, const float* d_sigma, const float* raw,
                                      const float* hid, const float* W9, int32_t M, int32_t HW, int32_t row_passes,
                                      int32_t tr_passes, uint16_t* img, float* graw, sparf_stream_t stream) {
  SPARF_REQUIRE(M >= 1 && M <= (1 << 20) && HW >= 8 && HW <= 512 && HW % 8 == 0, "tc_selftest_head: M=%d HW=%d", M, HW);
  cudaStream_t st = (cudaStream_t)stream;
  float* scratch = nullptr;
  SPARF_CHECK_CUDA(cudaMallocAsync(reinterpret_cast<void**>(&scratch), ((size_t)M * (HW + 4) + 4 * HW + 4) * sizeof(float), st));
  const int rc = selftest_head(d_rgb, rgb, d_sigma, raw, hid, W9, M, HW, TcPrec{false, row_passes}, TcPrec{false, tr_passes},
                               img, graw, scratch, st);
  cudaFreeAsync(scratch, st);
  return rc;
}

extern "C" int sparf_tc_selftest_featgrad(const float* d_raw, const float* d_feat, const float* feat, int32_t M, int32_t W,
                                          int32_t row_passes, int32_t tr_passes, uint16_t* img, float* sums,
                                          sparf_stream_t stream) {
  SPARF_REQUIRE(M >= 1 && M <= (1 << 20) && W >= 8 && W <= 512 && W % 8 == 0, "tc_selftest_featgrad: M=%d W=%d", M, W);
  SPARF_REQUIRE(d_raw && d_feat && feat && img && sums, "tc_selftest_featgrad: NULL tensor");
  cudaStream_t st = (cudaStream_t)stream;
  float* scratch = nullptr;
  SPARF_CHECK_CUDA(cudaMallocAsync(reinterpret_cast<void**>(&scratch), (size_t)M * W * sizeof(float), st));
  const int rc = selftest_featgrad(d_raw, d_feat, feat, M, W, TcPrec{false, row_passes}, TcPrec{false, tr_passes}, img, sums,
                                   scratch, st);
  cudaFreeAsync(scratch, st);
  return rc;
}
```

Before: 246,500.

## Chain head feature dgrad into the trunk dgrad chain kernel with rank-1 sigma term

Extends the persistent dgrad chain kernel to start at the head's hidden-gradient layer, so the feature dgrad GEMM through head_w[0] and the last trunk layer run inside the chained kernel instead of a separate GEMM. The sigma contribution of the last trunk layer is applied as a rank-1 update in the epilogue, and its weight-gradient row is accumulated in the staged wgrad converter warps. Extra producer warps build the ReLU mask bits from H on the fly. This removes a full-size intermediate gradient image round trip and a kernel launch, at the cost of more complex warp specialisation, atomics and new selftest paths.

Result: faster. 258,900, median of 6 (+5.0%).

```diff
diff --git a/include/sparf_b200.h b/include/sparf_b200.h
--- a/include/sparf_b200.h
+++ b/include/sparf_b200.h
@@ -247,6 +247,14 @@
                                   const uint32_t* bits, int32_t dg_passes, int32_t wg_passes, int32_t max_ctas,
                                   int32_t chain, const int64_t* rows, uint16_t* tr, uint16_t* row, float* db,
                                   sparf_stream_t stream);
+int sparf_tc_selftest_wgrad_r1(const float* G, const float* X, int32_t M, int32_t N, int32_t K, int32_t ldx, int32_t passes,
+                               int32_t max_ctas, const int64_t* rows, const float* r1_vec, float* dW, float* r1_out,
+                               sparf_stream_t stream);
+int sparf_tc_selftest_dgrad_chain_head(const float* Ghid, int32_t M, int32_t HW, int32_t E3, int32_t nt, int32_t skip,
+                                       const float* Wh, const float* W, const float* wr1, const uint32_t* fbits,
+                                       const float* H, const float* graw, const uint32_t* bits, int32_t dg_passes,
+                                       int32_t wg_passes, int32_t max_ctas, int32_t chain, const int64_t* rows, uint16_t* tr,
+                                       uint16_t* row, float* db, sparf_stream_t stream);
 
 #ifdef __cplusplus
 }
diff --git a/sparf_b200/_lib.py b/sparf_b200/_lib.py
--- a/sparf_b200/_lib.py
+++ b/sparf_b200/_lib.py
@@ -126,6 +126,10 @@
                                                _P, _P, _P, _P]),
     "sparf_tc_selftest_dgrad_chain": (c_int32, [_P, c_int32, c_int32, c_int32, c_int32, _P, _P, c_int32, c_int32, c_int32,
                                                 c_int32, _P, _P, _P, _P, _P]),
+    "sparf_tc_selftest_wgrad_r1": (c_int32, [_P, _P, c_int32, c_int32, c_int32, c_int32, c_int32, c_int32, _P, _P, _P, _P,
+                                             _P]),
+    "sparf_tc_selftest_dgrad_chain_head": (c_int32, [_P, c_int32, c_int32, c_int32, c_int32, c_int32, _P, _P, _P, _P, _P, _P,
+                                                     _P, c_int32, c_int32, c_int32, c_int32, _P, _P, _P, _P, _P]),
 }
 
 _lib = None
diff --git a/sparf_b200/csrc/gemm_wgmma.cu b/sparf_b200/csrc/gemm_wgmma.cu
--- a/sparf_b200/csrc/gemm_wgmma.cu
+++ b/sparf_b200/csrc/gemm_wgmma.cu
@@ -821,8 +821,9 @@
   }
 }
 
-template <int PASSES, int NST = STAGES>
-__device__ __forceinline__ void convert_staged(const Staged& x, const Units& w, uint64_t* full, uint64_t* conv) {
+template <int PASSES, int NST = STAGES, bool R1 = false>
+__device__ __forceinline__ void convert_staged(const Staged& x, const Units& w, uint64_t* full, uint64_t* conv,
+                                               const float* r1_vec = nullptr, float* r1_out = nullptr) {
   extern __shared__ __align__(1024) uint8_t smem[];
   const int t = threadIdx.x - CONSUMERS, lane = t & 31;
   int it = 0;
@@ -831,8 +832,10 @@
     w.get(u, bx, by, kt0, nk);
     const bool kin = bx * TM + t < x.K, bits = x.bits && by == 0;
     const int bword = bx * (TM / 32) + (t >> 5);
+    float r1 = 0.f;
     for (int j = 0; j < nk; ++j, ++it) {
       const int s = it % NST, m0 = (kt0 + j) * TK;
+      const float g = R1 && by == 0 && m0 + lane < x.M ? r1_vec[m0 + lane] : 0.f;
       mbar_wait(&full[s], (it / NST) & 1);
       uint8_t* st = smem + s * STAGE_BYTES + 2 * TILE_BYTES;
       const float* src = reinterpret_cast<const float*>(st);
@@ -852,6 +855,10 @@
           if (lane == r) word = b;
         }
         if (m0 + lane < x.M && bword < x.kw) x.bits[(size_t)(m0 + lane) * x.kw + bword] = word;
+      }
+      if (R1 && by == 0) {
+#pragma unroll
+        for (int r = 0; r < TK; ++r) r1 = fmaf(__shfl_sync(0xffffffffu, g, r), v[r], r1);
       }
       converter_sync();
       uint16_t* img = reinterpret_cast<uint16_t*>(st);
@@ -870,6 +877,7 @@
       __syncwarp();
       if (lane == 0) mbar_arrive(&conv[s]);
     }
+    if (R1 && by == 0 && kin && nk > 0) atomicAdd(r1_out + bx * TM + t, r1);
   }
 }
 
@@ -904,9 +912,10 @@
   __syncwarp();
 }
 
-template <int PASSES, bool DYN = false>
+template <int PASSES, bool DYN = false, bool R1 = false>
 __global__ void __launch_bounds__(STAGED_THREADS, 1) wg_gemm_staged_kernel(Opnd a, Staged x, Units w, Epi e, RowCount rc,
-                                                                           int ctas, const __grid_constant__ CUtensorMap xmap) {
+                                                                           int ctas, const __grid_constant__ CUtensorMap xmap,
+                                                                           const float* r1_vec, float* r1_out) {
   extern __shared__ __align__(1024) uint8_t smem[];
   if constexpr (DYN) {
     x.M = (int)live_rows<true, false>(x.M, rc);
@@ -934,7 +943,7 @@
   }
   if (threadIdx.x >= CONSUMERS) {
     asm volatile("setmaxnreg.dec.sync.aligned.u32 64;\n" ::: "memory");
-    convert_staged<PASSES, STAGED_STAGES>(x, w, full, conv);
+    convert_staged<PASSES, STAGED_STAGES, R1>(x, w, full, conv, r1_vec, r1_out);
     return;
   }
   asm volatile("setmaxnreg.inc.sync.aligned.u32 200;\n" ::: "memory");
@@ -1189,32 +1198,75 @@
   float* db[SPARF_MAX_TRUNK];
   uint16_t* tr[SPARF_MAX_TRUNK];
   uint16_t* row[SPARF_MAX_TRUNK];
+  int in_ks;
+  const uint16_t* hw;
+  const uint32_t* hbits;
+  float* hdb;
+  uint16_t* htr;
+  const float *hmask, *r1_vec, *r1_row;
 };
 
-template <int DP>
+template <int DP, bool HEAD = false>
 __device__ __forceinline__ void dg_produce(const DgChain& c, int M, int tiles, uint64_t* full, uint64_t* empty, uint64_t* act_full,
                                            uint64_t* act_empty) {
   extern __shared__ __align__(1024) uint8_t smem[];
   constexpr int HB = DP == 3 ? 2 : 1;
+  const int iks = HEAD ? c.in_ks : CH_KS;
   int it = 0, n = 0;
   for (int t = blockIdx.x; t < tiles; t += gridDim.x) {
     if (t * CH_M >= M) continue;
     mbar_wait(act_empty, (n & 1) ^ 1);
     ++n;
-    mbar_expect_tx(act_full, CH_KS * HB * CH_HALF);
-    for (int kt = 0; kt < CH_KS; ++kt)
+    mbar_expect_tx(act_full, iks * HB * CH_HALF);
+    for (int kt = 0; kt < iks; ++kt)
       for (int h = 0; h < HB; ++h)
         bulk_g2s(smem + (kt * 2 + h) * CH_HALF,
-                 c.in + (((size_t)(t >> 1) * CH_KS + kt) * 2 + h) * TILE_ELEMS + (t & 1) * (CH_M * TK), CH_HALF, act_full);
-    for (int l = c.top; l >= 1; --l)
-      for (int kt = 0; kt < CH_KS; ++kt, ++it) {
+                 c.in + (((size_t)(t >> 1) * iks + kt) * 2 + h) * TILE_ELEMS + (t & 1) * (CH_M * TK), CH_HALF, act_full);
+    for (int l = c.top + HEAD; l >= 1; --l) {
+      const bool hl = HEAD && l > c.top;
+      const int nk = hl ? iks : CH_KS;
+      const uint16_t* wl = hl ? c.hw : c.w[l];
+      for (int kt = 0; kt < nk; ++kt, ++it) {
         const int s = it % CH_STAGES;
         mbar_wait(&empty[s], ((it / CH_STAGES) & 1) ^ 1);
         uint8_t* st = smem + CH_RING + s * STAGE_BYTES;
         mbar_expect_tx(&full[s], 2 * HB * TILE_BYTES);
         for (int g = 0; g < 2; ++g)
-          bulk_g2s(st + g * 2 * TILE_BYTES, c.w[l] + ((size_t)g * CH_KS + kt) * 2 * TILE_ELEMS, HB * TILE_BYTES, &full[s]);
-      }
+          bulk_g2s(st + g * 2 * TILE_BYTES, wl + ((size_t)g * nk + kt) * 2 * TILE_ELEMS, HB * TILE_BYTES, &full[s]);
+      }
+    }
+  }
+}
+
+constexpr int DG_HB = 8 * TN * 4, DG_HB_BAR = DG_HB + CH_M * (CH_W / 32) * 4;
+
+__device__ __forceinline__ void dg_head_bits(const DgChain& c, int M, int tiles, uint64_t* hb_full, uint64_t* hb_empty) {
+  extern __shared__ __align__(1024) uint8_t smem[];
+  uint32_t* hb = reinterpret_cast<uint32_t*>(smem + CH_ENC + DG_HB);
+  const int wid = (threadIdx.x >> 5) - (CONSUMERS / 32 + 1), lane = threadIdx.x & 31;
+  int n = 0;
+  for (int t = blockIdx.x; t < tiles; t += gridDim.x) {
+    if (t * CH_M >= M) continue;
+    if (wid == 0 && lane == 0)
+      asm volatile("cp.async.bulk.prefetch.L2.global [%0], %1;\n" ::"l"(c.hmask + (size_t)t * CH_M * CH_W),
+                   "r"(min(CH_M, M - t * CH_M) * CH_W * 4) : "memory");
+    mbar_wait(hb_empty, (n & 1) ^ 1);
+    ++n;
+    for (int r = wid; r < CH_M; r += 3) {
+      const int m = t * CH_M + r;
+      float v[CH_W / 32];
+#pragma unroll
+      for (int q = 0; q < CH_W / 32; ++q) v[q] = m < M ? c.hmask[(size_t)m * CH_W + 32 * q + lane] : 0.f;
+      uint32_t word = 0;
+#pragma unroll
+      for (int q = 0; q < CH_W / 32; ++q) {
+        const uint32_t b = __ballot_sync(0xffffffffu, v[q] > 0.f);
+        if (lane == q) word = b;
+      }
+      if (lane < CH_W / 32) hb[r * (CH_W / 32) + lane] = word;
+    }
+    __syncwarp();
+    if (lane == 0) mbar_arrive(hb_full);
   }
 }
 
@@ -1244,23 +1296,26 @@
   }
 }
 
-template <int DP, int TP>
+template <int DP, int TP, bool HEAD = false>
 __device__ __forceinline__ void dg_zero_tile(const DgChain& c, int t) {
   const uint4 z = make_uint4(0, 0, 0, 0);
-  for (int l = c.top; l >= 1; --l) {
-    if (c.row[l])
+  for (int l = c.top + HEAD; l >= 1; --l) {
+    const bool hl = HEAD && l > c.top;
+    uint16_t* row = hl ? nullptr : c.row[l];
+    uint16_t* tr = hl ? c.htr : c.tr[l];
+    if (row)
       for (int i = 0; i < CH_KS * (DP == 3 ? 2 : 1); ++i)
-        reinterpret_cast<uint4*>(c.row[l] + ((size_t)(t >> 1) * CH_KS * 2 + (DP == 3 ? i : 2 * i)) * TILE_ELEMS +
+        reinterpret_cast<uint4*>(row + ((size_t)(t >> 1) * CH_KS * 2 + (DP == 3 ? i : 2 * i)) * TILE_ELEMS +
                                  (t & 1) * (CH_M * TK))[threadIdx.x] = z;
     for (int g = 0; g < 2; ++g)
       for (int kt = 2 * t; kt < 2 * t + 2 && kt < c.tr_ks; ++kt)
         for (int h = 0; h < (TP == 3 ? 2 : 1); ++h)
           for (int i = threadIdx.x; i < TILE_ELEMS / 8; i += CONSUMERS)
-            reinterpret_cast<uint4*>(c.tr[l] + (((size_t)g * c.tr_ks + kt) * 2 + h) * TILE_ELEMS)[i] = z;
-  }
-}
-
-template <int DP, int TP, bool DYN = false>
+            reinterpret_cast<uint4*>(tr + (((size_t)g * c.tr_ks + kt) * 2 + h) * TILE_ELEMS)[i] = z;
+  }
+}
+
+template <int DP, int TP, bool DYN = false, bool HEAD = false>
 __global__ void __launch_bounds__(GEMM_THREADS, 1) dgrad_chain_kernel(const DgChain c, RowCount rc) {
   extern __shared__ __align__(1024) uint8_t smem[];
   const int M = (int)live_rows<DYN, false>(c.M, rc);
@@ -1271,6 +1326,8 @@
   uint64_t* act_full = empty + CH_STAGES;
   uint64_t* act_empty = act_full + 1;
   float* red = reinterpret_cast<float*>(smem + CH_ENC);
+  uint64_t* hb_full = reinterpret_cast<uint64_t*>(smem + CH_ENC + DG_HB_BAR);
+  uint64_t* hb_empty = hb_full + 1;
   if (threadIdx.x == 0) {
     for (int i = 0; i < CH_STAGES; ++i) {
       mbar_init(&full[i], 1);
@@ -1278,31 +1335,59 @@
     }
     mbar_init(act_full, 1);
     mbar_init(act_empty, CONSUMERS / 32);
+    if constexpr (HEAD) {
+      mbar_init(hb_full, 3);
+      mbar_init(hb_empty, CONSUMERS / 32);
+    }
     asm volatile("fence.mbarrier_init.release.cluster;\n" ::: "memory");
   }
   __syncthreads();
   if (threadIdx.x >= CONSUMERS) {
     asm volatile("setmaxnreg.dec.sync.aligned.u32 40;\n" ::: "memory");
-    if (threadIdx.x == CONSUMERS) dg_produce<DP>(c, M, tiles, full, empty, act_full, act_empty);
+    if (threadIdx.x == CONSUMERS) dg_produce<DP, HEAD>(c, M, tiles, full, empty, act_full, act_empty);
+    if (HEAD && threadIdx.x >= CONSUMERS + 32) dg_head_bits(c, M, tiles, hb_full, hb_empty);
     return;
   }
   asm volatile("setmaxnreg.inc.sync.aligned.u32 232;\n" ::: "memory");
   const int wg = threadIdx.x >> 7, wq = (threadIdx.x >> 5) & 3, w = threadIdx.x >> 5, lane = threadIdx.x & 31;
-  int it = 0, n = 0;
+  int it = 0, n = 0, nb = 0;
   for (int t = blockIdx.x; t < tiles; t += gridDim.x) {
     if (t * CH_M >= M) {
-      dg_zero_tile<DP, TP>(c, t);
+      dg_zero_tile<DP, TP, HEAD>(c, t);
       continue;
     }
     mbar_wait(act_full, n & 1);
     ++n;
-    for (int l = c.top; l >= 1; --l) {
+    for (int l = c.top + HEAD; l >= 1; --l) {
+      const bool hl = HEAD && l > c.top, r1l = HEAD && l == c.top;
       uint4 wd[2];
-      dg_mask_words(wd, c.bits[l], M, t);
+      if (r1l) {
+        mbar_wait(hb_full, nb & 1);
+        ++nb;
+        const uint32_t* hb = reinterpret_cast<const uint32_t*>(smem + CH_ENC + DG_HB);
+#pragma unroll
+        for (int h = 0; h < 2; ++h)
+          wd[h] = *reinterpret_cast<const uint4*>(hb + (wq * 16 + (lane >> 2) + 8 * h) * (CH_W / 32) + wg * 4);
+        __syncwarp();
+        if (lane == 0) mbar_arrive(hb_empty);
+      } else {
+        dg_mask_words(wd, hl ? c.hbits : c.bits[l], M, t);
+      }
       float acc[64];
-      chain_mma<false, DP>(acc, CH_KS, CH_KS, it, full, empty);
+      chain_mma<false, DP>(acc, hl ? c.in_ks : CH_KS, hl ? c.in_ks : CH_KS, it, full, empty);
       if (l == 1 && lane == 0) mbar_arrive(act_empty);
       consumer_sync();
+      if (r1l) {
+#pragma unroll
+        for (int i = 0; i < 64; i += 2) {
+          const int m = t * CH_M + wq * 16 + (lane >> 2) + ((i >> 1) & 1) * 8, n = wg * TN + (i >> 2) * 8 + (lane & 3) * 2;
+          if (m < M) {
+            const float g = c.r1_vec[m];
+            acc[i] = fmaf(g, c.r1_row[n], acc[i]);
+            acc[i + 1] = fmaf(g, c.r1_row[n + 1], acc[i + 1]);
+          }
+        }
+      }
       const uint32_t wds[2][4] = {{wd[0].x, wd[0].y, wd[0].z, wd[0].w}, {wd[1].x, wd[1].y, wd[1].z, wd[1].w}};
 #pragma unroll
       for (int i = 0; i < 64; i += 2) {
@@ -1329,11 +1414,11 @@
         float s = 0.f;
 #pragma unroll
         for (int i = 0; i < 4; ++i) s += red[(4 * wg + i) * TN + (threadIdx.x & (TN - 1))];
-        atomicAdd(c.db[l] + threadIdx.x, s);
+        atomicAdd((hl ? c.hdb : c.db[l]) + threadIdx.x, s);
       }
       const int kt = 2 * t + (wq >> 1);
       if (kt < c.tr_ks) {
-        uint16_t* tp = c.tr[l] + ((size_t)wg * c.tr_ks + kt) * 2 * TILE_ELEMS;
+        uint16_t* tp = (hl ? c.htr : c.tr[l]) + ((size_t)wg * c.tr_ks + kt) * 2 * TILE_ELEMS;
 #pragma unroll
         for (int j = 0; j < 16; ++j)
 #pragma unroll
@@ -1345,7 +1430,7 @@
             if (TP == 3) reinterpret_cast<uint32_t*>(tp + TILE_ELEMS + core * 64)[lane] = movmatrix_trans(lo);
           }
       }
-      if (c.row[l])
+      if (!hl && c.row[l])
         dg_split<DP>(acc, c.row[l] + (size_t)(t >> 1) * CH_KS * 2 * TILE_ELEMS + (t & 1) * (CH_M * TK), 2 * TILE_ELEMS, TILE_ELEMS);
     }
   }
@@ -1353,7 +1438,8 @@
 
 template <int DP, int TP>
 static int launch_dgrad_chain(const DgChain& c, int ctas, RowCount rc, cudaStream_t st) {
-  auto kernel = rc.rows ? dgrad_chain_kernel<DP, TP, true> : dgrad_chain_kernel<DP, TP>;
+  auto kernel = c.hw ? (rc.rows ? dgrad_chain_kernel<DP, TP, true, true> : dgrad_chain_kernel<DP, TP, false, true>)
+                     : (rc.rows ? dgrad_chain_kernel<DP, TP, true> : dgrad_chain_kernel<DP, TP>);
   SPARF_CHECK_CUDA(cudaFuncSetAttribute(kernel, cudaFuncAttributeMaxDynamicSharedMemorySize, CH_SMEM));
   kernel<<<std::min(2 * ceil_div(c.M, TM), ctas), GEMM_THREADS, CH_SMEM, st>>>(c, rc);
   SPARF_CHECK_LAUNCH("dgrad_chain_kernel");
@@ -1433,14 +1519,17 @@
 }
 
 template <int PASSES>
-static int run_staged(const TcPrec& p, const Opnd& gt, int N, const Staged& x, int ksteps, const Epi& e, cudaStream_t st) {
+static int run_staged(const TcPrec& p, const Opnd& gt, int N, const Staged& x, int ksteps, const Epi& e, const float* r1_vec,
+                      float* r1_out, cudaStream_t st) {
   CUtensorMap xmap{};
   if (x.div == 1 && x.M > 0) SPARF_TRY(staged_tensor_map(x, &xmap));
   const int ctas = gemm_ctas(p);
   const Units w = gemm_units(ceil_div(N, TM), ceil_div(x.K, TM), ksteps, true, ctas);
-  auto kernel = p.rows.rows ? wg_gemm_staged_kernel<PASSES, true> : wg_gemm_staged_kernel<PASSES>;
+  auto kernel = r1_out ? (p.rows.rows ? wg_gemm_staged_kernel<PASSES, true, true> : wg_gemm_staged_kernel<PASSES, false, true>)
+                       : (p.rows.rows ? wg_gemm_staged_kernel<PASSES, true> : wg_gemm_staged_kernel<PASSES>);
   SPARF_CHECK_CUDA(cudaFuncSetAttribute(kernel, cudaFuncAttributeMaxDynamicSharedMemorySize, STAGED_SMEM));
-  kernel<<<std::min(w.tiles * w.nsplit, ctas), STAGED_THREADS, STAGED_SMEM, st>>>(gt, x, w, e, p.rows, ctas, xmap);
+  kernel<<<std::min(w.tiles * w.nsplit, ctas), STAGED_THREADS, STAGED_SMEM, st>>>(gt, x, w, e, p.rows, ctas, xmap, r1_vec,
+                                                                                   r1_out);
   SPARF_CHECK_LAUNCH("wg_gemm_staged_kernel");
   return SPARF_OK;
 }
@@ -1524,18 +1613,30 @@
 }
 
 int tc_dgrad_chain(TcPrec dg, TcPrec wg, int M, int W, int top, TcImage in, const TcImage* wimg, const uint32_t* const* bits,
-                   float* const* db, const TcImage* tr, const TcImage* row, cudaStream_t st) {
-  SPARF_REQUIRE(!dg.f16 && !wg.f16 && M >= 1 && W == CH_W && top >= 1 && top < SPARF_MAX_TRUNK && in.p && in.ks == CH_KS,
-                "tc_dgrad_chain: bf16 images, M=%d W=%d top=%d, input row image of %d k-steps", M, W, top, CH_KS);
+                   float* const* db, const TcImage* tr, const TcImage* row, cudaStream_t st, const TcChainHead* head) {
+  SPARF_REQUIRE(!dg.f16 && !wg.f16 && M >= 1 && W == CH_W && top >= 1 && top < SPARF_MAX_TRUNK && in.p &&
+                    (head ? in.ks >= 1 && in.ks <= CH_KS : in.ks == CH_KS),
+                "tc_dgrad_chain: bf16 images, M=%d W=%d top=%d, input row image of %d k-steps", M, W, top, in.ks);
   DgChain c{};
-  c.M = M; c.top = top; c.tr_ks = ceil_div(M, TK); c.in = in.p;
+  c.M = M; c.top = top; c.tr_ks = ceil_div(M, TK); c.in = in.p; c.in_ks = in.ks;
+  if (head) {
+    SPARF_REQUIRE(head->w.p && head->w.ks == in.ks && head->bits && !(reinterpret_cast<uintptr_t>(head->bits) & 15) && head->db &&
+                      head->tr.p && head->tr.ks == c.tr_ks && head->mask && !(reinterpret_cast<uintptr_t>(head->mask) & 7) &&
+                      head->r1_vec && head->r1_row,
+                  "tc_dgrad_chain: head layer: weight image of %d k-steps, 16-byte aligned mask bits, column sums, transposed "
+                  "image of %d k-steps; layer %d: 8-byte aligned fp32 mask, rank-1 vectors",
+                  in.ks, c.tr_ks, top);
+    c.hw = head->w.p; c.hbits = head->bits; c.hdb = head->db; c.htr = head->tr.p;
+    c.hmask = head->mask; c.r1_vec = head->r1_vec; c.r1_row = head->r1_row;
+  }
   for (int l = 1; l <= top; ++l) {
-    SPARF_REQUIRE(wimg[l].p && wimg[l].ks == CH_KS && bits[l] && !(reinterpret_cast<uintptr_t>(bits[l]) & 15) && db[l] &&
+    const bool fp32_mask = head && l == top;
+    SPARF_REQUIRE(wimg[l].p && wimg[l].ks == CH_KS && (fp32_mask || (bits[l] && !(reinterpret_cast<uintptr_t>(bits[l]) & 15))) && db[l] &&
                       tr[l].p && tr[l].ks == c.tr_ks && (!row[l].p || row[l].ks == CH_KS),
                   "tc_dgrad_chain: layer %d: weight image of %d k-steps, 16-byte aligned mask bits, column sums, transposed "
                   "image of %d k-steps, row image of %d",
                   l, CH_KS, c.tr_ks, CH_KS);
-    c.w[l] = wimg[l].p; c.bits[l] = bits[l]; c.db[l] = db[l]; c.tr[l] = tr[l].p; c.row[l] = row[l].p;
+    c.w[l] = wimg[l].p; c.bits[l] = fp32_mask ? nullptr : bits[l]; c.db[l] = db[l]; c.tr[l] = tr[l].p; c.row[l] = row[l].p;
   }
   const int ctas = gemm_ctas(dg);
   if (dg.passes == 3 && wg.passes == 3) return launch_dgrad_chain<3, 3>(c, ctas, dg.rows, st);
@@ -1591,15 +1692,18 @@
 }
 
 int tc_gemm_tn(TcPrec p, int M, int N, int K, int Kv, TcImage gt, const float* X, int ldx, int div, float* dW, int ldw,
-               int wcol, uint32_t* bits, cudaStream_t st) {
+               int wcol, uint32_t* bits, cudaStream_t st, const float* r1_vec, float* r1_out) {
   SPARF_REQUIRE((p.passes == 1 || p.passes == 3) && gt.ks == ceil_div(M, TK), "tc_gemm_tn: passes=%d ks=%d", p.passes, gt.ks);
+  SPARF_REQUIRE(!r1_out || (r1_vec && div == 1 && Kv == K), "tc_gemm_tn: r1_out needs r1_vec, div = 1 and Kv = K");
   Epi e{};
   e.kind = 2; e.M = N; e.N = K; e.out = dW; e.ldo = ldw; e.col_off = wcol; e.Kv = Kv;
   if (!(reinterpret_cast<uintptr_t>(X) & 15) && ldx % 4 == 0 && K % 4 == 0) {
     SPARF_REQUIRE(!p.f16, "tc_gemm_tn: bf16 halves only");
     const Staged x{X, ldx, div, M, K, bits, ceil_div(K, 32)};
-    return p.passes == 3 ? run_staged<3>(p, opnd(gt), N, x, gt.ks, e, st) : run_staged<1>(p, opnd(gt), N, x, gt.ks, e, st);
-  }
+    return p.passes == 3 ? run_staged<3>(p, opnd(gt), N, x, gt.ks, e, r1_vec, r1_out, st)
+                         : run_staged<1>(p, opnd(gt), N, x, gt.ks, e, r1_vec, r1_out, st);
+  }
+  SPARF_REQUIRE(!r1_out, "tc_gemm_tn: r1_out needs X 16-byte aligned with ldx and K multiples of 4");
   SPARF_REQUIRE(!p.rows.rows, "tc_gemm_tn: a device row count needs X 16-byte aligned with ldx and K multiples of 4");
   return SPARF_WG_RUN(false, p, opnd(gt), N, TnB{X, ldx, div, M, K, bits, ceil_div(K, 32)}, K, gt.ks, true, e, 0, 0, st);
 }
@@ -1728,7 +1832,8 @@
 }
 
 static int selftest_wgrad(const float* G, const float* X, int M, int N, int K, int Kv, int ldx, int div, int passes,
-                          int max_ctas, const int64_t* rows, float* dW, uint32_t* bits, cudaStream_t st) {
+                          int max_ctas, const int64_t* rows, float* dW, uint32_t* bits, cudaStream_t st,
+                          const float* r1_vec = nullptr, float* r1_out = nullptr) {
   SPARF_REQUIRE(M >= 1 && M <= (1 << 20) && N >= 1 && N <= 512 && K >= 1 && K <= 512 && Kv >= 0 && Kv <= K && ldx >= K &&
                     div >= 1 && (passes == 1 || passes == 3),
                 "tc_selftest_wgrad: M=%d N=%d K=%d Kv=%d ldx=%d div=%d passes=%d", M, N, K, Kv, ldx, div, passes);
@@ -1740,9 +1845,18 @@
   const TcImage gt{p.pack_a, ceil_div(M, TK)};
   int rc = tc_pack_cols(p, M, N, G, N, gt, st);
   p.rows = RowCount{rows, 0};
-  if (!rc) rc = tc_gemm_tn(p, M, N, K, Kv, gt, X, ldx, div, dW, K, 0, bits, st);
+  if (!rc) rc = tc_gemm_tn(p, M, N, K, Kv, gt, X, ldx, div, dW, K, 0, bits, st, r1_vec, r1_out);
   free_images(p, st);
   return rc;
+}
+
+extern "C" int sparf_tc_selftest_wgrad_r1(const float* G, const float* X, int32_t M, int32_t N, int32_t K, int32_t ldx,
+                                          int32_t passes, int32_t max_ctas, const int64_t* rows, const float* r1_vec, float* dW,
+                                          float* r1_out, sparf_stream_t stream) {
+  SPARF_REQUIRE(r1_vec && r1_out && K >= 1 && K <= 512, "tc_selftest_wgrad_r1: K=%d, r1 vectors", K);
+  cudaStream_t st = (cudaStream_t)stream;
+  SPARF_CHECK_CUDA(cudaMemsetAsync(r1_out, 0, (size_t)K * sizeof(float), st));
+  return selftest_wgrad(G, X, M, N, K, K, ldx, 1, passes, max_ctas, rows, dW, nullptr, st, r1_vec, r1_out);
 }
 
 extern "C" int sparf_tc_selftest_wgrad(const float* G, const float* X, int32_t M, int32_t N, int32_t K, int32_t Kv, int32_t ldx,
@@ -1933,3 +2047,67 @@
   free_images(dg, st);
   return rc;
 }
+
+extern "C" int sparf_tc_selftest_dgrad_chain_head(const float* Ghid, int32_t M, int32_t HW, int32_t E3, int32_t nt, int32_t skip,
+                                                  const float* Wh, const float* W, const float* wr1, const uint32_t* fbits,
+                                                  const float* H, const float* graw, const uint32_t* bits, int32_t dg_passes,
+                                                  int32_t wg_passes, int32_t max_ctas, int32_t chain, const int64_t* rows,
+                                                  uint16_t* tr, uint16_t* row, float* db, sparf_stream_t stream) {
+  SPARF_REQUIRE(Ghid && Wh && W && wr1 && fbits && H && graw && bits && tr && db && M >= 1 && M <= (1 << 20) && HW >= 1 &&
+                    HW <= CH_W && E3 >= 1 && nt >= 3 && nt <= SPARF_MAX_TRUNK && skip > 0 && skip <= nt - 3,
+                "tc_selftest_dgrad_chain_head: M=%d HW=%d E3=%d nt=%d skip=%d", M, HW, E3, nt, skip);
+  cudaStream_t st = (cudaStream_t)stream;
+  TcPrec dg{false, dg_passes}, wg{false, wg_passes};
+  dg.max_ctas = wg.max_ctas = max_ctas;
+  dg.rows = wg.rows = RowCount{rows, 0};
+  const int top = nt - 1, hks = ceil_div(HW, TK);
+  const size_t ngh = tc_image_elems(M, HW), nh = tc_image_elems(M, CH_W), ntr = tc_image_elems(CH_W, M),
+               nw = tc_image_elems(CH_W, CH_W);
+  SPARF_TRY(alloc_images(std::max(ngh + 2 * nh, (size_t)(nt + 1) * nw), st, dg));
+  SPARF_CHECK_CUDA(cudaMemsetAsync(db, 0, (size_t)nt * CH_W * sizeof(float), st));
+  const TcImage gin{dg.pack_a, hks}, grow[2] = {{dg.pack_a + ngh, CH_KS}, {dg.pack_a + ngh + nh, CH_KS}};
+  const float* Wl[SPARF_MAX_TRUNK];
+  int ldw[SPARF_MAX_TRUNK];
+  size_t wo = 0;
+  for (int l = 0; l < nt; ++l) {
+    Wl[l] = W + wo;
+    ldw[l] = (l == 0 ? E3 : CH_W) + (l == skip ? E3 : 0);
+    wo += (size_t)CH_W * ldw[l];
+  }
+  TcImage trl[SPARF_MAX_TRUNK], rowl[SPARF_MAX_TRUNK], wimg[SPARF_MAX_TRUNK];
+  const uint32_t* bl[SPARF_MAX_TRUNK] = {};
+  float* dbl[SPARF_MAX_TRUNK] = {};
+  for (int l = 1; l <= top; ++l) {
+    trl[l] = TcImage{tr + (size_t)(l - 1) * ntr, ceil_div(M, TK)};
+    if (row && (l == 1 || l - 1 == skip)) rowl[l] = TcImage{row + (l == 1 ? 0 : nh), CH_KS};
+    if (l < top) bl[l] = bits + (size_t)(l - 1) * M * (CH_W / 32);
+    dbl[l] = db + (size_t)(l - 1) * CH_W;
+    wimg[l] = TcImage{dg.pack_b + (size_t)l * nw, CH_KS};
+  }
+  const TcImage htr{tr + (size_t)top * ntr, ceil_div(M, TK)}, himg{dg.pack_b, hks};
+  float* hdb = db + (size_t)top * CH_W;
+  int rc = tc_pack_rows(dg, M, HW, Ghid, HW, 1, gin, st);
+  if (chain) {
+    for (int l = 1; l <= top && !rc; ++l) rc = tc_pack_nn(dg, CH_W, CH_W, CH_W, Wl[l], ldw[l], 0, wimg[l], st);
+    if (!rc) rc = tc_pack_nn(dg, CH_W, HW, CH_W, Wh, CH_W, 0, himg, st);
+    TcChainHead h;
+    h.w = himg; h.tr = htr; h.bits = fbits; h.db = hdb; h.mask = H; h.r1_vec = graw; h.r1_row = wr1;
+    if (!rc) rc = tc_dgrad_chain(dg, wg, M, CH_W, top, gin, wimg, bl, dbl, trl, rowl, st, &h);
+  } else {
+    TcOut oh, ol;
+    oh.row = grow[0]; oh.tr = htr;
+    ol.row = grow[1]; ol.tr = trl[top];
+    oh.row_passes = ol.row_passes = dg_passes;
+    oh.tr_passes = ol.tr_passes = wg_passes;
+    if (!rc)
+      rc = tc_gemm_nn(dg, M, HW, CH_W, CH_W, gin, Wh, CH_W, 0, nullptr, 0, fbits, nullptr, nullptr, nullptr, 0, 0, oh, hdb,
+                      nullptr, st);
+    if (!rc)
+      rc = tc_gemm_nn(dg, M, CH_W, CH_W, CH_W, grow[0], Wl[top], ldw[top], 0, H, CH_W, nullptr, graw, wr1, nullptr, 0, 0, ol,
+                      dbl[top], nullptr, st);
+    for (int l = 1; l < top && !rc; ++l) rc = tc_pack_nn(dg, CH_W, CH_W, CH_W, Wl[l], ldw[l], 0, wimg[l], st);
+    if (!rc) rc = tc_dgrad_chain(dg, wg, M, CH_W, top - 1, grow[1], wimg, bl, dbl, trl, rowl, st);
+  }
+  free_images(dg, st);
+  return rc;
+}
diff --git a/sparf_b200/csrc/gemm_wgmma.cuh b/sparf_b200/csrc/gemm_wgmma.cuh
--- a/sparf_b200/csrc/gemm_wgmma.cuh
+++ b/sparf_b200/csrc/gemm_wgmma.cuh
@@ -38,13 +38,20 @@
 int tc_trunk_chain(TcPrec p, int M, int W, int nt, int skip, TcImage enc, const TcImage* wimg, const float* const* bias,
                    float* const* H, uint32_t* const* bits, const TcOut& last, cudaStream_t st);
 int tc_pack_nn(TcPrec p, int Kout, int N, int Kv, const float* W, int ldw, int wcol, TcImage img, cudaStream_t st);
+struct TcChainHead {
+  TcImage w, tr;
+  const uint32_t* bits;
+  float* db;
+  const float *mask, *r1_vec, *r1_row;
+};
 int tc_dgrad_chain(TcPrec dg, TcPrec wg, int M, int W, int top, TcImage in, const TcImage* wimg, const uint32_t* const* bits,
-                   float* const* db, const TcImage* tr, const TcImage* row, cudaStream_t st);
+                   float* const* db, const TcImage* tr, const TcImage* row, cudaStream_t st,
+                   const TcChainHead* head = nullptr);
 int tc_gemm_nn(TcPrec p, int M, int N, int Kout, int Kv, TcImage g, const float* W, int ldw, int wcol, const float* mask_src,
                int ldmask, const uint32_t* mask_bits, const float* r1_vec, const float* r1_row, float* D, int ldd,
                int accumulate, const TcOut& out, float* db, float* r1_wgrad, cudaStream_t st);
 int tc_gemm_tn(TcPrec p, int M, int N, int K, int Kv, TcImage gt, const float* X, int ldx, int div, float* dW, int ldw,
-               int wcol, uint32_t* bits, cudaStream_t st);
+               int wcol, uint32_t* bits, cudaStream_t st, const float* r1_vec = nullptr, float* r1_out = nullptr);
 
 int tc_head_backward(TcPrec dg, TcPrec wg, int M, int HW, const float* d_rgb, const float* rgb, const float* d_sigma,
                      const float* raw, const float* hid, const float* W9, float* graw, TcImage row, TcImage tr, float* dW9,
diff --git a/sparf_b200/csrc/mlp.cu b/sparf_b200/csrc/mlp.cu
--- a/sparf_b200/csrc/mlp.cu
+++ b/sparf_b200/csrc/mlp.cu
@@ -548,6 +548,7 @@
 };
 
 static bool trunk_chained(const MlpDims& d, bool tc) { return tc && tc_chain_supported(d.W, d.E3p, d.nt, d.skip); }
+static bool head_chained(const MlpDims& d, bool tc) { return trunk_chained(d, tc) && d.HW <= d.W; }
 
 static size_t tape_layout(const MlpDims& d, bool tc, int R, int S, char* base, Tape* tp) {
   const size_t M = (size_t)R * S;
@@ -583,9 +584,9 @@
   float *wts, *rgbv, *G0, *G1, *Genc, *Ghid, *gpre, *graw, *Gdtmp, *Gdenc;
   float *ones, *colsum_sink;
   Tape act;
-  TcImage encimg, dencimg, Himg[2], Grow[2], Gtr[SPARF_MAX_TRUNK - 1], ghid_row, ghid_tr;
+  TcImage encimg, dencimg, Himg[2], Grow[2], Gtr[SPARF_MAX_TRUNK], ghid_row, ghid_tr;
   TcImage wimg[SPARF_MAX_TRUNK];
-  TcImage nnimg[SPARF_MAX_TRUNK];
+  TcImage nnimg[SPARF_MAX_TRUNK], headimg;
   uint32_t* mask_bits;
   uint16_t* pack_b;
   size_t pack_elems;
@@ -597,6 +598,7 @@
   const bool fwd_here = pass == Pass::kForward || pass == Pass::kRecomputeBackward || grad_only;
   const bool bwd = pass == Pass::kRecomputeBackward || pass == Pass::kTapedBackward || grad_only;
   const bool chain = trunk_chained(d, tc);
+  const bool hchain = head && head_chained(d, tc);
   Carver cv{base, 0};
   Ws w{};
   w.wts = cv.take(32);
@@ -647,10 +649,11 @@
   }
   if (tc && bwd) {
     for (TcImage& g : w.Grow) g = cv.image((int)Mc, d.W);
-    const int ntr = chain ? d.nt - 1 : 2;
+    const int ntr = hchain ? d.nt : chain ? d.nt - 1 : 2;
     for (int i = 0; i < (grad_only ? 1 : ntr); ++i) w.Gtr[i] = cv.image(d.W, (int)Mc);
     for (int i = 1; grad_only && i < ntr; ++i) w.Gtr[i] = w.Gtr[0];
-    for (int l = 1; chain && l <= d.nt - 2; ++l) w.nnimg[l] = cv.image(d.W, d.W);
+    for (int l = 1; chain && l <= (hchain ? d.nt - 1 : d.nt - 2); ++l) w.nnimg[l] = cv.image(d.W, d.W);
+    if (hchain) w.headimg = cv.image(d.W, d.HW);
     if (head) {
       w.ghid_row = cv.image((int)Mc, d.HW);
       w.ghid_tr = cv.image(d.HW, (int)Mc);
@@ -913,8 +916,9 @@
                              ghid_t, grad->head_w[1], grad->head_b[1], grad->head_b[0], grad->trunk_b[d.nt - 1], st));
   SPARF_TRY(tc_gemm_tn(ep.wgrad, (int)Mc, d.HW, d.W, d.W, ghid_t, feat, d.W, 1, grad->head_w[0], ldw8, 0, w.mask_bits, st));
   SPARF_TRY(tc_gemm_tn(ep.wgrad, (int)Mc, d.HW, d.Evp, d.Ev, ghid_t, v.denc, d.Evp, S, grad->head_w[0], ldw8, d.W, nullptr, st));
-  SPARF_TRY(tc_gemm_nn(ep.dgrad, (int)Mc, d.HW, d.W, d.W, ghid, mlp->head_w[0], ldw8, 0, nullptr, 0, w.mask_bits, nullptr,
-                       nullptr, nullptr, 0, 0, grad_images(c, 0, Mc), grad->trunk_b[d.nt - 1] + 1, nullptr, st));
+  if (!head_chained(d, true))
+    SPARF_TRY(tc_gemm_nn(ep.dgrad, (int)Mc, d.HW, d.W, d.W, ghid, mlp->head_w[0], ldw8, 0, nullptr, 0, w.mask_bits, nullptr,
+                         nullptr, nullptr, 0, 0, grad_images(c, 0, Mc), grad->trunk_b[d.nt - 1] + 1, nullptr, st));
   if (dir_grad)
     SPARF_TRY(tc_gemm_nn(ep.dgrad, (int)Mc, d.HW, d.Evp, d.Ev, ghid, mlp->head_w[0], ldw8, d.W, nullptr, 0, nullptr, nullptr,
                          nullptr, w.Gdtmp, d.Evp, 0, TcOut{}, nullptr, nullptr, st));
@@ -960,34 +964,51 @@
   return SPARF_OK;
 }
 
-static int grad_tr_buf(const MlpDims& d, bool chained, int l) { return chained ? (l ? d.nt - 1 - l : 0) : (d.nt - 1 - l) & 1; }
+static int grad_tr_buf(const MlpDims& d, bool chained, int l, bool from_head = false) {
+  return chained ? (l || from_head ? d.nt - 1 - l : 0) : (d.nt - 1 - l) & 1;
+}
 static int grad_row(const MlpDims& d, bool chained, int l) {
   return chained ? (l == 0 || l == d.nt - 1 ? 0 : 1) : (d.nt - 1 - l) & 1;
 }
 
-static int chunk_dgrad_chain(const SparfMLP* mlp, const Call& c, long long Mc, uint32_t* const* bits, const SparfMLPGrad* grad,
-                             bool enc_grad, cudaStream_t st) {
+static int chunk_dgrad_chain(const SparfMLP* mlp, const Call& c, long long Mc, float* const* H, uint32_t* const* bits,
+                             const float* graw, const SparfMLPGrad* grad, bool enc_grad, bool from_head, cudaStream_t st) {
   const MlpDims& d = c.d;
-  const int top = d.nt - 2;
+  const int top = from_head ? d.nt - 1 : d.nt - 2;
   const uint32_t* mask[SPARF_MAX_TRUNK] = {};
   float* db[SPARF_MAX_TRUNK] = {};
   TcImage tr[SPARF_MAX_TRUNK], row[SPARF_MAX_TRUNK];
   for (int l = top; l >= 1; --l) {
-    SPARF_TRY(tc_pack_nn(c.ep.dgrad, d.W, d.W, d.W, mlp->trunk_w[l], trunk_ldw(d, l), 0, c.w.nnimg[l], st));
-    mask[l] = bits[l - 1];
+    const int ldw = trunk_ldw(d, l);
+    SPARF_TRY(tc_pack_nn(c.ep.dgrad, d.W, d.W, d.W, mlp->trunk_w[l] + (l == d.nt - 1 ? ldw : 0), ldw, 0, c.w.nnimg[l], st));
+    mask[l] = l < d.nt - 1 ? bits[l - 1] : nullptr;
     db[l] = grad ? grad->trunk_b[l - 1] : c.w.colsum_sink;
-    tr[l] = grad_tr(c.w, grad_tr_buf(d, true, l - 1), Mc);
+    tr[l] = grad_tr(c.w, grad_tr_buf(d, true, l - 1, from_head), Mc);
     if (enc_grad && (l - 1 == 0 || l - 1 == d.skip)) row[l] = c.w.Grow[grad_row(d, true, l - 1)];
   }
-  return tc_dgrad_chain(c.ep.dgrad, c.ep.wgrad, (int)Mc, d.W, top, c.w.Grow[grad_row(d, true, top)], c.w.nnimg, mask, db, tr,
-                        row, st);
+  if (!from_head)
+    return tc_dgrad_chain(c.ep.dgrad, c.ep.wgrad, (int)Mc, d.W, top, c.w.Grow[grad_row(d, true, top)], c.w.nnimg, mask, db,
+                          tr, row, st);
+  SPARF_TRY(tc_pack_nn(c.ep.dgrad, d.W, d.HW, d.W, mlp->head_w[0], d.W + d.Ev, 0, c.w.headimg, st));
+  TcChainHead h;
+  h.w = c.w.headimg;
+  h.tr = grad_tr(c.w, grad_tr_buf(d, true, d.nt - 1, true), Mc);
+  h.bits = c.w.mask_bits;
+  h.db = grad->trunk_b[d.nt - 1] + 1;
+  h.mask = H[d.nt - 2];
+  h.r1_vec = graw;
+  h.r1_row = mlp->trunk_w[d.nt - 1];
+  return tc_dgrad_chain(c.ep.dgrad, c.ep.wgrad, (int)Mc, d.W, top, c.w.ghid_row, c.w.nnimg, mask, db, tr, row, st, &h);
 }
 
 static int trunk_backward_tc(const SparfMLP* mlp, const Call& c, long long Mc, const float* enc, float* const* H,
-                             uint32_t* const* bits, const float* graw, const SparfMLPGrad* grad, bool enc_grad, cudaStream_t st) {
+                             uint32_t* const* bits, const float* graw, const SparfMLPGrad* grad, bool enc_grad, bool from_head,
+                             cudaStream_t st) {
   const MlpDims& d = c.d;
   const EnginePrec& ep = c.ep;
   const bool chained = trunk_chained(d, true);
+  SPARF_REQUIRE(!from_head || (chained && grad && graw), "trunk_backward_tc: a chain from the head needs weight gradients");
+  if (from_head) SPARF_TRY(chunk_dgrad_chain(mlp, c, Mc, H, bits, graw, grad, enc_grad, true, st));
   bool genc_written = false;
   for (int l = d.nt - 1; l >= 0; --l) {
     const bool last = l == d.nt - 1;
@@ -998,12 +1019,14 @@
     const int rowoff = last ? 1 : 0;
     const float* Wl = mlp->trunk_w[l] + (size_t)rowoff * ldw;
     const int gi = (d.nt - 1 - l) & 1;
-    const bool nn = l > 0 && (!chained || last);
+    const bool nn = l > 0 && (!chained || (last && !from_head));
     uint32_t* wbits = grad && nn && !r1 ? c.w.mask_bits : nullptr;
     if (grad) {
       float* dWl = grad->trunk_w[l] + (size_t)rowoff * ldw;
-      const TcImage gt = grad_tr(c.w, grad_tr_buf(d, chained, l), Mc);
-      SPARF_TRY(tc_gemm_tn(ep.wgrad, (int)Mc, d.W, Kin, Kinv, gt, in, Kin, 1, dWl, ldw, 0, wbits, st));
+      const TcImage gt = grad_tr(c.w, grad_tr_buf(d, chained, l, from_head), Mc);
+      const bool r1_here = from_head && r1;
+      SPARF_TRY(tc_gemm_tn(ep.wgrad, (int)Mc, d.W, Kin, Kinv, gt, in, Kin, 1, dWl, ldw, 0, wbits, st, r1_here ? graw : nullptr,
+                           r1_here ? grad->trunk_w[l] : nullptr));
       if (l == d.skip) SPARF_TRY(tc_gemm_tn(ep.wgrad, (int)Mc, d.W, d.E3p, d.E3, gt, enc, d.E3p, 1, dWl, ldw, d.W, nullptr, st));
     }
     if (nn)
@@ -1016,7 +1039,7 @@
                            nullptr, st));
       genc_written = true;
     }
-    if (chained && last) SPARF_TRY(chunk_dgrad_chain(mlp, c, Mc, bits, grad, enc_grad, st));
+    if (chained && last && !from_head) SPARF_TRY(chunk_dgrad_chain(mlp, c, Mc, H, bits, graw, grad, enc_grad, false, st));
   }
   return SPARF_OK;
 }
@@ -1060,7 +1083,7 @@
       }
       SPARF_CHECK_LAUNCH("direnc_bwd_kernel");
     }
-    SPARF_TRY(c.tc ? trunk_backward_tc(mlp, c, Mc, v.enc, v.H, v.bits, w.graw, grad, need_rays, st)
+    SPARF_TRY(c.tc ? trunk_backward_tc(mlp, c, Mc, v.enc, v.H, v.bits, w.graw, grad, need_rays, head_chained(d, true), st)
                    : trunk_backward_simt(mlp, c, Mc, v.enc, v.H, w.graw, grad, need_rays, st));
     if (need_rays) {
       float* d_o = d_origins ? d_origins + (size_t)r0 * 3 : nullptr;
@@ -1260,7 +1283,7 @@
     } else {
       SPARF_CHECK_CUDA(cudaMemsetAsync(c.w.G0, 0, (size_t)n * d.W * sizeof(float), st));
     }
-    SPARF_TRY(c.tc ? trunk_backward_tc(mlp, c, n, v.enc, v.H, v.bits, dr, grad, d_points != nullptr, st)
+    SPARF_TRY(c.tc ? trunk_backward_tc(mlp, c, n, v.enc, v.H, v.bits, dr, grad, d_points != nullptr, false, st)
                    : trunk_backward_simt(mlp, c, n, v.enc, v.H, dr, grad, d_points != nullptr, st));
     if (d_points) {
       posenc_bwd_kernel<<<ceil_div(n, 4), 128, 0, st>>>(n, 1, mlp->L_xyz, d.E3p, v.enc, c.w.Genc, nullptr,
@@ -1294,7 +1317,7 @@
       SPARF_CHECK_CUDA(cudaMemsetAsync(c.w.Grow[0].p, 0, tc_image_elems(n, d.W) * sizeof(uint16_t), st));
     else
       SPARF_CHECK_CUDA(cudaMemsetAsync(c.w.G0, 0, (size_t)n * d.W * sizeof(float), st));
-    SPARF_TRY(c.tc ? trunk_backward_tc(mlp, c, n, v.enc, v.H, v.bits, c.w.ones, nullptr, true, st)
+    SPARF_TRY(c.tc ? trunk_backward_tc(mlp, c, n, v.enc, v.H, v.bits, c.w.ones, nullptr, true, false, st)
                    : trunk_backward_simt(mlp, c, n, v.enc, v.H, c.w.ones, nullptr, true, st));
     posenc_bwd_kernel<<<ceil_div(n, 4), 128, 0, st>>>(n, 1, mlp->L_xyz, d.E3p, v.enc, c.w.Genc, nullptr, gp, nullptr, c.rc);
     SPARF_CHECK_LAUNCH("posenc_bwd_kernel");
```
